# AlphacatPlus/VmambaIR

Hardware: AMD Instinct MI355X
Metric: images/sec, x4 SR 64->256 training step (fwd+bwd+Adam+EMA), full VmambaIR UNet (higher is better)
Workload: dtype bf16; 1 GPU; BASELINE.json configs[1]: x4 SR 64x64 LQ, MambaSISR6 dim48 [15,1,1,1]+15, bf16 autocast (scan arithmetic f32), batch 8 per GPU; global_batch=8, per_gpu_batch=8, parallelism=dp1, step_launch=hipGraph replay, vendor_conv_solver_search=True, vendor_conv_solver_records=bench_data/miopen, optimizer=Adam 2e-4 (0.9,0.99) + EMA 0.999, loss=L1, rccl_ranks=1, allreduce_overlapped=False, allreduce_buckets=1, allreduce_bytes=0

## Files before the change

### include/vmambair_oss.h

```cpp
#ifndef VMAMBAIR_OSS_H
#define VMAMBAIR_OSS_H

#include <stddef.h>
#include <stdint.h>

#ifdef __cplusplus
extern "C" {
#endif

#define OSS_OK 0
#define OSS_ERR_NULL (-1)
#define OSS_ERR_SHAPE (-2)
#define OSS_ERR_DSTATE (-3)
#define OSS_ERR_WORKSPACE (-4)

#define OSS_MAX_DSTATE 256

typedef enum {
    OSS_F32 = 0, OSS_F16 = 1, OSS_BF16 = 2,
    OSS_F32_BF16X3 = 3
} oss_dtype;

typedef void *oss_stream_t;

typedef struct {
    int batch, dim, seqlen, dstate, n_groups;
    int delta_softplus;
    int rev_group_start, u_row_mod;
    int a_log_form, reserved0_;
    int64_t u_batch_stride, u_d_stride;
    int64_t delta_batch_stride, delta_d_stride;
    int64_t out_batch_stride, out_d_stride;
    int64_t A_d_stride;
    int64_t B_batch_stride, B_group_stride, B_dstate_stride;
    int64_t C_batch_stride, C_group_stride, C_dstate_stride;
    const void *u, *delta;
    const float *A;
    const void *B, *C;
    const float *D;
    const float *delta_bias;
    void *out;
    float *x;
    const float *dt_weight;
    int dt_rank, reserved1_;
    int64_t dt_group_stride, dt_rank_stride;
    void *workspace;
    size_t workspace_bytes;
    float *hs;
    int tune_variant, tune_segments, tune_carry_split, reserved2_;
} oss_scan_fwd_params;

typedef struct {
    oss_scan_fwd_params f;
    int64_t dout_batch_stride, dout_d_stride;
    int64_t du_batch_stride, du_d_stride;
    int64_t ddelta_batch_stride, ddelta_d_stride;
    const void *dout;
    void *du, *ddelta;
    float *dA;
    void *dB, *dC;
    float *dD;
    float *ddelta_bias;
    void *workspace;
    size_t workspace_bytes;
    int dout_row_mod;
    int reserved_;
    int64_t dBC_group_stride;
    void *ddt;
    float *ddt_weight;
    int64_t ddt_batch_stride, ddt_group_stride, ddt_rank_stride;
    int tune_variant, tune_segments;
    int tune_partials, reserved3_;
    const float *finish_dt_weight;
    int finish_dt_rank, reserved4_;
} oss_scan_bwd_params;

int oss_scan_chunk(void);
int oss_scan_num_chunks(int seqlen);

size_t oss_scan_fwd_workspace_bytes(int batch, int dim, int seqlen, int dstate, int n_groups);
size_t oss_scan_lane_state_floats(int batch, int dim, int seqlen, int dstate);
int oss_scan_fwd(const oss_scan_fwd_params *p, oss_dtype io, oss_stream_t stream);

size_t oss_scan_bwd_workspace_bytes(int batch, int dim, int seqlen, int dstate, int n_groups);
int oss_scan_bwd(const oss_scan_bwd_params *p, oss_dtype io, oss_stream_t stream);

int oss_scan_bwd_finish_dt_ok(int seqlen, int dt_rank);

int oss_scan_fused_dt_ok(oss_dtype io, int batch, int D, int C, int R, int dstate, int seqlen);

void oss_scan_set_variant(int fwd_variant, int bwd_variant);
int oss_scan_last_variant(int which );
void oss_scan_set_segments(int fwd_segments, int bwd_segments);
int oss_scan_last_segments(int which );
void oss_scan_set_carry_split(int split);
int oss_scan_last_lane_states(void);

int oss_dwconv3x3_fwd(oss_dtype io, const void *x, const float *weight, const float *bias, void *y, void *pre_silu, int batch,
                      int channels, int height, int width, int64_t x_batch_stride, int64_t x_channel_stride,
                      int64_t y_batch_stride, int64_t y_channel_stride, int flip, oss_stream_t stream);
int oss_dwconv3x3_wgrad(oss_dtype io, const void *x, const void *dy, float *dweight, float *dbias, float *partials,
                        const void *pre_silu, void *dpre, int batch, int channels, int height, int width,
                        int64_t x_batch_stride, int64_t x_channel_stride, int64_t dy_batch_stride, int64_t dy_channel_stride,
                        oss_stream_t stream);

int oss_dwconv3x3_fused_ok(oss_dtype io, int height, int width, int channels_per_workgroup);
int oss_dwconv3x3_silu_fwd(oss_dtype io, const void *x, const float *weight, const float *bias, void *y, int batch, int channels,
                           int height, int width, int64_t x_batch_stride, int64_t x_channel_stride, int64_t y_batch_stride,
                           int64_t y_channel_stride, oss_stream_t stream);
int oss_dwconv3x3_silu_bwd(oss_dtype io, const void *x, const float *weight, const float *bias, const void *dy, void *dx,
                           float *dweight, float *dbias, float *partials, int batch, int channels, int height, int width,
                           int64_t x_batch_stride, int64_t x_channel_stride, int64_t dy_batch_stride, int64_t dy_channel_stride,
                           int64_t dx_batch_stride, int64_t dx_channel_stride, oss_stream_t stream);
int oss_dwgate_fwd_ok(oss_dtype io, int height, int width);

int oss_effn_fwd_ok(oss_dtype io, int channels, int hidden, int height, int width);
int oss_effn_round_weights(oss_dtype io, const float *project_in, const float *dwconv, const float *project_out, void *w_in, float *w_dw,
                           void *w_out, int channels, int hidden, oss_stream_t stream);
int oss_effn_fwd(oss_dtype io, const void *x, const float *norm_weight, const float *norm_bias, const void *w_in, const float *w_dw,
                 const void *w_out, void *out, int batch, int channels, int hidden, int height, int width, int64_t x_batch_stride,
                 int64_t x_channel_stride, int64_t out_batch_stride, int64_t out_channel_stride, float eps, oss_stream_t stream);
int oss_dwgate_fwd(oss_dtype io, const void *t, const float *weight, const float *bias, void *out, int batch, int hidden,
                   int height, int width, int64_t t_batch_stride, int64_t t_channel_stride, int64_t out_batch_stride,
                   int64_t out_channel_stride, oss_stream_t stream);
int oss_dwgate_bwd(oss_dtype io, const void *t, const float *weight, const float *bias, const void *dout, void *dt,
                   float *dweight, float *dbias, float *partials, int batch, int hidden, int height, int width,
                   int64_t t_batch_stride, int64_t t_channel_stride, int64_t dout_batch_stride, int64_t dout_channel_stride,
                   int64_t dt_batch_stride, int64_t dt_channel_stride, oss_stream_t stream);

int oss_dwconv3x3_flat2_ok(oss_dtype io, int height, int width);
int oss_dwconv3x3_silu_flat2_fwd(oss_dtype io, const void *x, const float *weight, const float *bias, void *x2, int batch, int channels,
                                 int height, int width, int64_t x_batch_stride, int64_t x_channel_stride, oss_stream_t stream);
int oss_dwconv3x3_silu_flat2_bwd(oss_dtype io, const void *x, const float *weight, const float *bias, const void *g2, void *dx,
                                 float *dweight, float *dbias, float *partials, int batch, int channels, int height, int width,
                                 int64_t x_batch_stride, int64_t x_channel_stride, int64_t dx_batch_stride, int64_t dx_channel_stride,
                                 oss_stream_t stream);

int oss_conv1x1_fwd(oss_dtype io, const void *x, const float *weight, const float *bias, const void *residual, void *y,
                    int batch, int cout, int cin, int pixels, int64_t x_batch_stride, int64_t x_channel_stride,
                    oss_stream_t stream);
int oss_conv1x1_dgrad(oss_dtype io, const void *dy, const float *weight, void *dx, int batch, int cout, int cin, int pixels,
                      int64_t dy_batch_stride, int64_t dy_channel_stride, oss_stream_t stream);
size_t oss_conv1x1_wgrad_partial_floats(int batch, int cout, int cin, int pixels);
size_t oss_conv1x1_fwd_image_bytes(int cout, int cin);
size_t oss_conv1x1_dgrad_image_bytes(int cout, int cin);
size_t oss_conv1x1_pack_row_bytes(void);
int oss_conv1x1_pack_rows(int cout, int cin);
int oss_conv1x1_pack_fill(void *rows, const float *weight, void *fwd_image, void *dgrad_image, int cout, int cin);
int oss_conv1x1_pack_weights(oss_dtype io, const void *table, int n_rows, oss_stream_t stream);
int oss_conv1x1_fwd_packed(oss_dtype io, const void *x, const float *weight, const void *fwd_image, const float *bias,
                           const void *residual, void *y, int batch, int cout, int cin, int pixels, int64_t x_batch_stride,
                           int64_t x_channel_stride, oss_stream_t stream);
int oss_conv1x1_dgrad_packed(oss_dtype io, const void *dy, const float *weight, const void *dgrad_image, void *dx, int batch,
                             int cout, int cin, int pixels, int64_t dy_batch_stride, int64_t dy_channel_stride,
                             oss_stream_t stream);
int oss_ln_conv1x1_fwd_packed(oss_dtype io, const void *x, const float *ln_weight, const float *ln_bias, float eps, void *n, float *mean,
                              float *rstd, const float *weight, const void *fwd_image, const float *bias, void *y, int batch, int cout,
                              int cin, int pixels, int64_t x_batch_stride, int64_t x_channel_stride, oss_stream_t stream);
int oss_conv1x1_wg(oss_dtype io, const void *x, const float *weight, const float *bias, void *y, int batch, int cout, int cin,
                   int pixels, int64_t x_batch_stride, int64_t x_channel_stride, int transposed_weight, oss_stream_t stream);
int oss_ln_conv1x1_ok(oss_dtype io, int cout, int cin, int pixels);
int oss_ln_conv1x1_fwd(oss_dtype io, const void *x, const float *ln_weight, const float *ln_bias, float eps, void *n, float *mean,
                       float *rstd, const float *weight, const float *bias, void *y, int batch, int cout, int cin, int pixels,
                       int64_t x_batch_stride, int64_t x_channel_stride, oss_stream_t stream);
int oss_conv1x1_dgrad_ln_bwd_ok(oss_dtype io, int cout, int cin, int pixels, int batch);
size_t oss_conv1x1_dgrad_ln_bwd_partial_floats(int batch, int cin, int pixels);
int oss_conv1x1_dgrad_ln_bwd(oss_dtype io, const void *dy, const float *weight, const void *x, const float *ln_weight, int ln_has_bias,
                             const float *mean, const float *rstd, const void *skip_grad, void *dx, float *dln_weight, float *dln_bias,
                             float *partials, int batch, int cout, int cin, int pixels, int64_t dy_batch_stride,
                             int64_t dy_channel_stride, oss_stream_t stream);
void oss_conv1x1_set_wg(int on, int pixels);
void oss_conv1x1_wgrad_set_tile(int mode);
void oss_conv1x1_wgrad_set_span(int mult);
int oss_conv1x1_wgrad(oss_dtype io, const void *dy, const void *x, float *dweight, float *dbias, float *partials, int batch,
                      int cout, int cin, int pixels, int64_t dy_batch_stride, int64_t dy_channel_stride,
                      int64_t x_batch_stride, int64_t x_channel_stride, oss_stream_t stream);

int oss_cross_scan2(oss_dtype in_type, oss_dtype out_type, const void *x, void *x2, int batch, int D, int height, int width,
                    int64_t x_batch_stride, int64_t x_channel_stride, oss_stream_t stream);
int oss_cross_merge2(oss_dtype io, const void *g2, void *dx, int batch, int D, int height, int width, oss_stream_t stream);
int oss_proj_fwd(oss_dtype io, const void *x2, const float *x_proj_weight, const float *dt_projs_weight, void *xdbl, void *dts,
                 int batch, int D, int C, int R, int seqlen, oss_stream_t stream);
int oss_proj_dgrad(oss_dtype io, const void *ddts, void *dxdbl, const void *du, const float *x_proj_weight,
                   const float *dt_projs_weight, void *dx2, int batch, int D, int C, int R, int seqlen, oss_stream_t stream);
size_t oss_proj_wgrad_partial_floats(int batch, int D, int C, int R, int seqlen);
void oss_proj_set_path(int force_vector_alu);
int oss_proj_rows_optional_ok(oss_dtype io, int batch, int D, int C, int R, int seqlen);
int oss_proj_wgrad(oss_dtype io, const void *x2, const void *xdbl, const void *dxdbl, const void *ddts, float *dx_proj_weight,
                   float *ddt_projs_weight, float *partials, int batch, int D, int C, int R, int seqlen, oss_stream_t stream);

typedef struct {
    int B, L, dc, Rc, Cc, reserved_;
    const float *pooled;
    const float *cin_w, *cin_b;
    const float *Wxc;
    const float *Wdtc;
    const float *dt_bias;
    const float *A_logs;
    const float *Dsc;
    const float *cout_w, *cout_b;
    const float *cn_w, *cn_b;
    float *zt;
    float *dts;
    float *hs;
    float *y;
    float *yc;
    float *stat;
    float *c;
    const float *pool_part;
    int n_part;
    float pool_scale;
} oss_chan_params;
int oss_chan_fwd(const oss_chan_params *p, oss_stream_t stream);
size_t oss_chan_grad_floats(int L, int dc, int Rc, int Cc);
size_t oss_chan_bwd_scratch_floats(int B, int L, int dc, int Rc, int Cc);
int oss_chan_bwd(const oss_chan_params *p, const float *gc, float *dpooled, float *grads, float *scratch, oss_stream_t stream);
int oss_rowsum(oss_dtype io, const void *a, const void *bmul, float *out, int batch, int channels, int pixels,
               int64_t a_batch_stride, int64_t a_channel_stride, int64_t b_batch_stride, int64_t b_channel_stride, float alpha,
               oss_stream_t stream);
int oss_row_affine(oss_dtype io, const void *x, const float *mul, const float *add, void *y, int batch, int channels,
                   int pixels, int64_t x_batch_stride, int64_t x_channel_stride, float alpha, oss_stream_t stream);

int oss_gelu_gate_fwd(oss_dtype io, const void *h, void *out, int batch, size_t half_elems, int64_t h_batch_stride,
                      oss_stream_t stream);
int oss_gelu_gate_bwd(oss_dtype io, const void *h, const void *dout, void *dh, int batch, size_t half_elems,
                      int64_t h_batch_stride, int64_t dout_batch_stride, oss_stream_t stream);

typedef struct {
    const void *src;
    void *dst;
    int64_t stride;
    int j0, n, K, reserved_;
} oss_sum_chunk;
void oss_set_defer_finish(int on);
size_t oss_deferred_chunks(void);
int oss_flush_finishes(void *host_table, void *device_table, size_t capacity_chunks, oss_stream_t stream);
int oss_flush_finishes_n(void *host_table, void *device_table, size_t capacity_chunks, size_t max_chunks, oss_stream_t stream);

void oss_set_defer_wgrad(int on);
size_t oss_deferred_wgrads(void);
size_t oss_deferred_wgrad_table_bytes(void);
int oss_flush_wgrads(void *host_table, void *device_table, size_t capacity_bytes, oss_stream_t stream);
int oss_flush_wgrads_n(void *host_table, void *device_table, size_t capacity_bytes, size_t max_products, oss_stream_t stream);

#define OSS_ADAM_CHUNK 2048
typedef struct {
    void *param;
    const void *grad;
    void *exp_avg, *exp_avg_sq, *ema;
    int n, reserved_;
} oss_adam_chunk;
int oss_adam_ema_step(const oss_adam_chunk *chunks, int n_chunks, float *state, float lr, float beta1, float beta2, float eps,
                      float ema_decay, oss_stream_t stream);
int oss_adamw_ema_step(const oss_adam_chunk *chunks, int n_chunks, float *state, float lr, float beta1, float beta2, float eps,
                       float weight_decay, float ema_decay, const float *grad_scale, oss_stream_t stream);

int oss_merge4(oss_dtype io, const void *out, float *y, int batch, int D, int height, int width, oss_stream_t stream);

size_t oss_ln_nchw_bwd_partial_floats(int batch, int channels, int pixels);
int oss_ln_nchw_fwd(oss_dtype x_type, oss_dtype y_type, const void *x, const float *weight, const float *bias,
                    const void *gate, void *y, float *mean, float *rstd, int batch, int channels, int pixels,
                    int64_t x_batch_stride, int64_t x_channel_stride, int64_t gate_batch_stride,
                    int64_t gate_channel_stride, float eps, oss_stream_t stream);
int oss_ln_nchw_fwd_pool_tiles(int channels, int pixels, int64_t x_batch_stride, int64_t x_channel_stride, int64_t gate_batch_stride,
                               int64_t gate_channel_stride);
int oss_ln_nchw_fwd_pool(oss_dtype x_type, oss_dtype y_type, const void *x, const float *weight, const float *bias,
                         const void *gate, void *y, float *mean, float *rstd, float *pool_part, int batch, int channels, int pixels,
                         int64_t x_batch_stride, int64_t x_channel_stride, int64_t gate_batch_stride,
                         int64_t gate_channel_stride, float eps, oss_stream_t stream);
int oss_ln_nchw_bwd(oss_dtype x_type, oss_dtype y_type, const void *x, const float *weight, const float *bias,
                    const void *gate, const void *dy, const float *mean, const float *rstd, void *dx, void *dgate,
                    float *dweight, float *dbias, float *partials, const void *skip_grad, int batch, int channels, int pixels,
                    int64_t x_batch_stride, int64_t x_channel_stride, int64_t gate_batch_stride,
                    int64_t gate_channel_stride, int64_t dgate_batch_stride, oss_stream_t stream);
int oss_ln_nchw_bwd_affine(oss_dtype x_type, oss_dtype y_type, const void *x, const float *weight, const float *bias,
                           const void *gate, const void *dy, const float *dy_mul, const float *dy_add, float add_scale,
                           const float *mean, const float *rstd, void *dx, void *dgate, float *dweight, float *dbias, float *partials,
                           const void *skip_grad, int batch, int channels, int pixels, int64_t x_batch_stride,
                           int64_t x_channel_stride, int64_t gate_batch_stride, int64_t gate_channel_stride,
                           int64_t dgate_batch_stride, oss_stream_t stream);

void oss_prof_enable(int on);
void oss_prof_reset(void);
int oss_prof_collect(int which, int variant, oss_dtype io, double *total_ms, long long *launches,
                     double *algorithmic_bytes);
int oss_prof_collect2(int which, int variant, oss_dtype io, double *total_ms, long long *launches, double *algorithmic_bytes,
                      double *own_bytes);

int oss_hbm_copy(const void *src, void *dst, size_t n_bytes, oss_stream_t stream);

int oss_prof_marker(int which, oss_stream_t stream);

const char *oss_scan_build_id(void);

const char *oss_version(void);

int oss_conv3x3_thin_ok(oss_dtype io, int cin, int cout, int height, int width);
int oss_conv3x3_thin_fwd(oss_dtype io, const void *x, const float *weight, const float *bias, void *y, int batch, int cin, int cout,
                         int height, int width, int64_t x_batch_stride, int64_t x_channel_stride, int64_t y_batch_stride,
                         int64_t y_channel_stride, oss_stream_t stream);
int oss_conv3x3_thin_dgrad(oss_dtype io, const void *dy, const float *weight, void *dx, int batch, int cin, int cout, int height,
                           int width, int64_t dy_batch_stride, int64_t dy_channel_stride, int64_t dx_batch_stride,
                           int64_t dx_channel_stride, oss_stream_t stream);
size_t oss_conv3x3_thin_wgrad_partial_floats(int batch, int cin, int cout);
int oss_conv3x3_thin_wgrad(oss_dtype io, const void *x, const void *dy, float *dweight, float *dbias, float *partial, int batch, int cin,
                           int cout, int height, int width, int64_t x_batch_stride, int64_t x_channel_stride, int64_t dy_batch_stride,
                           int64_t dy_channel_stride, oss_stream_t stream);

int oss_conv3x3_dense_ok(oss_dtype io, int cin, int cout, int height, int width);
int oss_conv3x3_dense_fwd(oss_dtype io, const void *x, const float *weight, const float *bias, void *y, int batch, int cin, int cout,
                          int height, int width, int64_t x_batch_stride, int64_t x_channel_stride, int64_t y_batch_stride,
                          int64_t y_channel_stride, oss_stream_t stream);
int oss_conv3x3_dense_dgrad(oss_dtype io, const void *dy, const float *weight, void *dx, int batch, int cin, int cout, int height,
                            int width, int64_t dy_batch_stride, int64_t dy_channel_stride, int64_t dx_batch_stride,
                            int64_t dx_channel_stride, oss_stream_t stream);
size_t oss_conv3x3_dense_wgrad_partial_floats(int batch, int cin, int cout, int height, int width);
int oss_conv3x3_dense_wgrad(oss_dtype io, const void *x, const void *dy, float *dweight, float *dbias, float *partial, int batch, int cin,
                            int cout, int height, int width, int64_t x_batch_stride, int64_t x_channel_stride, int64_t dy_batch_stride,
                            int64_t dy_channel_stride, oss_stream_t stream);

#define OSS_METRIC_QUANTISE 1
#define OSS_METRIC_Y 2
#define OSS_METRIC_REPLICATE 4
int oss_image_metrics_ok(oss_dtype io, int channels, int height, int width, int crop_border, int flags);
size_t oss_image_metrics_partial_doubles(int batch, int channels, int height, int width, int crop_border);
int oss_image_metrics(oss_dtype io, const void *a, const void *b, double *out, double *partials, int batch, int channels,
                      int height, int width, int64_t a_batch_stride, int64_t a_channel_stride, int64_t a_row_stride,
                      int64_t b_batch_stride, int64_t b_channel_stride, int64_t b_row_stride, int crop_border, int flags,
                      oss_stream_t stream);

#define OSS_PAIRS_HFLIP 1
#define OSS_PAIRS_ROT 2
int oss_pairs_philox(const uint32_t *counter, const uint32_t *key, uint32_t *out);
int oss_pairs_ok(int channels, int scale, int patch_h, int patch_w, int batch);
int oss_pairs_draw(const int64_t *table, int n_pairs, int64_t *counter, int *samples, int batch, int patch, int64_t seed, int rank,
                   int world, int flags, oss_stream_t stream);
int oss_pairs_gather(const void *pool, int64_t pool_bytes, const int64_t *table, int n_pairs, const int *samples, float *lq, float *gt,
                     int *clamped, int batch, int channels, int patch_h, int patch_w, int scale, int swap_rb, oss_stream_t stream);

void oss_prof_family_enable(int on);
int oss_prof_family_count(void);
int oss_prof_family(int family, const char **name, const char **kernel_patterns, double *algorithmic_bytes, long long *calls);

#define OSS_FEATURE_FUSED_DT 1
#define OSS_FEATURE_LANE_STATES 2
int oss_scan_features(void);

int oss_f32_matmul_modes(void);

#define OSS_ABI_VERSION 9
int oss_abi_version(void);
size_t oss_abi_struct_bytes(int which);

#ifdef __cplusplus
}
#endif
#endif
```

### vmambair_amd/csrc/oss_capi.hip

```cpp
#include <atomic>
#include <mutex>
#include <vector>
#include <cstring>
#include <algorithm>
#include "oss_device.h"
#include "oss_host.h"

namespace oss {

static std::atomic<int> g_force_fwd{-1}, g_force_bwd{-1};
static std::atomic<int> g_last_fwd{-1}, g_last_bwd{-1};
static std::atomic<int> g_force_fwd_seg{-1}, g_force_bwd_seg{-1};
std::atomic<int> g_last_fwd_segments{1}, g_last_bwd_segments{1}, g_last_bwd_lane_states{0};

int scan_pick_segments(long wgs, int n_chunks, int seg_req, double ovh) {
    if (seg_req == 0 || seg_req == 1 || n_chunks < 2 || wgs <= 0) return 1;
    if (seg_req > 1) return std::min(std::min(seg_req, n_chunks), kMaxSegments);
    if (wgs >= 256) return 1;
    int best = 1;
    double best_cost = (double)n_chunks;
    for (int s = 2; s <= std::min(n_chunks, 16); ++s) {
        const int cps = (n_chunks + s - 1) / s;
        if ((n_chunks + cps - 1) / cps != s) continue;
        const double rounds = (double)((wgs * s + 255) / 256);
        const double cost = rounds * cps * (1.0 + ovh);
        if (cost < 0.95 * best_cost) { best = s; best_cost = cost; }
    }
    return best;
}

static std::atomic<int> g_carry_split{0};
int scan_carry_split(long wgs, int n_seg, int cps, int n_chunks, int per_call) {
    if (n_seg <= 1) return 1;
    const int forced = per_call > 0 ? per_call : g_carry_split.load();
    const int max_slots = std::min(n_chunks, kMaxSegments);
    int csub = 1;
    for (int c = 2; c <= cps; ++c) {
        const int ccps = (cps + c - 1) / c, pieces = (cps + ccps - 1) / ccps;
        if (n_seg * pieces > max_slots) break;
        if (forced > 0 ? pieces <= forced : wgs * (n_seg - 1) * pieces <= 512) csub = pieces;
    }
    return csub;
}

static std::atomic<int> g_defer_finish{0};
static std::mutex g_defer_mu;
static std::vector<oss_sum_chunk> g_defer_chunks;
bool defer_finish() { return g_defer_finish.load() != 0; }
void defer_sum(const float *src, int K, size_t stride, size_t V, float *dst0, size_t n0, float *dst1) {
    std::lock_guard<std::mutex> lk(g_defer_mu);
    for (size_t j = 0; j < V;) {
        const size_t lim = j < n0 ? n0 : V;
        const size_t n = std::min<size_t>(1024, lim - j);
        oss_sum_chunk c;
        c.src = src;
        c.dst = j < n0 ? dst0 + j : dst1 + (j - n0);
        c.stride = (int64_t)stride;
        c.j0 = (int)j; c.n = (int)n; c.K = K; c.reserved_ = 0;
        g_defer_chunks.push_back(c);
        j += n;
    }
}
static std::atomic<int> g_defer_wgrad{0};
static std::vector<unsigned char> g_wgrad_descs;
static std::vector<unsigned> g_wgrad_blocks;
bool defer_wgrad() { return g_defer_wgrad.load() != 0; }
void defer_wgrad_push(const void *desc, size_t bytes, unsigned blocks) {
    std::lock_guard<std::mutex> lk(g_defer_mu);
    const unsigned char *p = reinterpret_cast<const unsigned char *>(desc);
    g_wgrad_descs.insert(g_wgrad_descs.end(), p, p + bytes);
    g_wgrad_blocks.push_back(blocks);
}

int scan_fwd_pick_variant(int batch, int dim, int seqlen, int dstate, int n_groups, int elem_bytes) {
    (void)dstate; (void)elem_bytes;
    const int rows_per_group = dim / n_groups;
    const long rows = (long)batch * dim;
    if (seqlen <= 256 || rows_per_group < 8) return (rows_per_group >= 16 && rows >= 4096) ? 2 : 4;
    if (rows_per_group % 16 == 0 && rows / 4 >= 2048) return 2;
    if (rows_per_group % 16 == 0 && rows / 2 >= 2048) return 1;
    if (seqlen >= 4096 && rows_per_group % 12 == 0 && (long)batch * n_groups * (rows_per_group / 12) <= 128) return 6;
    if (seqlen >= 1024 && (long)batch * n_groups * ((rows_per_group + 7) / 8) <= 256) return 3;
    if (seqlen >= 1024 && rows_per_group >= 12 && (long)batch * n_groups * ((rows_per_group + 11) / 12) <= 256) return 6;
    return 0;
}

int scan_bwd_pick_variant(int batch, int dim, int seqlen, int dstate, int n_groups) {
    const int rows_per_group = dim / n_groups;
    if (seqlen <= 256 || rows_per_group < 8 || dstate > 64) return 1;
    const long wgs = (long)batch * n_groups * ((rows_per_group + 7) / 8);
    if (seqlen >= 2048 && rows_per_group % 12 == 0 && (long)batch * n_groups * (rows_per_group / 12) < 192) return 10;
    if (wgs <= 128 && rows_per_group % 4 == 0) return 13;
    if (wgs <= 256) return 11;
    return rows_per_group >= 12 ? 10 : 11;
}

constexpr int kProfVariants = 32;
struct ProfBucket {
    std::vector<std::pair<hipEvent_t, hipEvent_t>> pending;
    double ms = 0.0, bytes = 0.0, own = 0.0;
    long long launches = 0;
};
static std::mutex g_prof_mu;
static std::atomic<int> g_prof_on{0};
static ProfBucket g_prof[3][kProfVariants][3];
static std::vector<hipEvent_t> g_event_pool;

static hipEvent_t prof_event() {
    if (!g_event_pool.empty()) { hipEvent_t e = g_event_pool.back(); g_event_pool.pop_back(); return e; }
    hipEvent_t e; (void)hipEventCreate(&e); return e;
}

struct ProfTimer : LaunchTimer {
    bool on; int which, variant, io; double bytes, own; hipEvent_t e0{}, e1{};
    ProfTimer(int which_, int variant_, int io_, double bytes_, double own_ = 0.0)
        : on(g_prof_on.load() != 0 && variant_ >= 0 && variant_ < 16), which(which_), variant(variant_),
          io(io_), bytes(bytes_), own(own_) {}
    void segmented() override { if (variant < 16) variant += 16; }
    void begin(hipStream_t s) override {
        if (!on) return;
        {
            std::lock_guard<std::mutex> lk(g_prof_mu);
            e0 = prof_event(); e1 = prof_event();
        }
        (void)hipEventRecord(e0, s);
    }
    void end(hipStream_t s) override {
        if (!on) return;
        (void)hipEventRecord(e1, s);
        std::lock_guard<std::mutex> lk(g_prof_mu);
        ProfBucket &b = g_prof[which][variant][io];
        b.pending.emplace_back(e0, e1);
        b.bytes += bytes;
        b.own += own;
        b.launches += 1;
    }
};


enum Fam { FAM_CONV1X1 = 0, FAM_WGRAD, FAM_DWCONV, FAM_PROJ, FAM_LN, FAM_CHAN, FAM_MERGE, FAM_GATE, FAM_CONV3X3, FAM_FINISH, FAM_OPTIM, FAM_N };
static const char *const kFamName[FAM_N] = {"conv1x1 forward / input gradient (+ fused LayerNorm)", "1x1 / projection weight gradients",
                                            "depth-wise 3x3 (+ silu / gelu gate / flattenings)", "x_proj / dt_proj forward + input gradient",
                                            "LayerNorm (+ silu gate, pooled sums)", "channel branch (+ rowsum / row_affine)",
                                            "cross-scan / cross-merge / merge4", "gelu gate (unfused)", "thin 3x3 convolutions",
                                            "deferred partial-sum finishing", "Adam(W) + EMA"};
static const char *const kFamKernels[FAM_N] = {"oss_conv1x1_pair_kernel|oss_conv1x1_pairk_kernel|oss_conv1x1_pairw_kernel|oss_conv1x1_wg_kernel|"
                                               "oss_conv1x1_dgrad_lnbwd_kernel|oss_conv1x1_f32_kernel|oss_conv1x1_pack_kernel",
                                               "oss_conv1x1_wgrad|oss_rows_f32_wgrad|oss_proj_wgrad",
                                               "oss_dwconv3x3|oss_dwgate|oss_effn",
                                               "oss_proj_fwd|oss_proj_dgrad|oss_dt_fwd|oss_dt_dgrad|oss_proj_valu",
                                               "oss_ln_nchw",
                                               "oss_chan_|oss_rowsum|oss_row_affine",
                                               "oss_merge4|oss_cross_scan2|oss_cross_merge2",
                                               "oss_gelu_gate",
                                               "oss_conv3x3_",
                                               "oss_sum_partials",
                                               "oss_adam"};
static std::atomic<int> g_fam_on{0};
static double g_fam_bytes[FAM_N];
static long long g_fam_calls[FAM_N];
static inline bool is_f32_split(oss_dtype io) { return io == OSS_F32_BF16X3; }
static inline int take_f32_split(oss_dtype &io) {
    if (!is_f32_split(io)) return 0;
    io = OSS_F32;
    return 1;
}
static inline void fam_count(int fam, double bytes) {
    if (!g_fam_on.load(std::memory_order_relaxed)) return;
    std::lock_guard<std::mutex> lk(g_prof_mu);
    g_fam_bytes[fam] += bytes;
    g_fam_calls[fam] += 1;
}

static double fwd_alg_bytes(const oss_scan_fwd_params &p, int s) {
    const double BKL = (double)p.batch * p.dim * p.seqlen, BGNL = (double)p.batch * p.n_groups * p.dstate * p.seqlen;
    const double xb = 4.0 * p.batch * p.dim * oss_scan_num_chunks(p.seqlen) * 2 * p.dstate;
    return s * (3.0 * BKL + 2.0 * BGNL) + 4.0 * ((double)p.dim * p.dstate + 2.0 * p.dim) + xb;
}
static double bwd_alg_bytes(const oss_scan_fwd_params &p, int s) {
    const double BKL = (double)p.batch * p.dim * p.seqlen, BGNL = (double)p.batch * p.n_groups * p.dstate * p.seqlen;
    const double xb = 4.0 * p.batch * p.dim * oss_scan_num_chunks(p.seqlen) * 2 * p.dstate;
    return s * (5.0 * BKL + 4.0 * BGNL) + 4.0 * (2.0 * p.dim * p.dstate + 4.0 * p.dim) + xb;
}

static double fwd_own_bytes(const oss_scan_fwd_params &p, int s) {
    const double full = fwd_alg_bytes(p, s);
    if (p.u_row_mod <= 0) return full;
    return full - (double)s * p.batch * (p.dim - p.u_row_mod) * p.seqlen;
}
static double bwd_own_bytes(const oss_scan_bwd_params &q, int s) {
    const oss_scan_fwd_params &p = q.f;
    double v = bwd_alg_bytes(p, s);
    if (p.u_row_mod > 0) v -= (double)s * p.batch * (p.dim - p.u_row_mod) * p.seqlen;
    if (q.dout_row_mod > 0) v -= (double)s * p.batch * (p.dim - q.dout_row_mod) * p.seqlen;
    return v;
}

static int check_fwd(const oss_scan_fwd_params *p) {
    if (!p || !p->u || !p->delta || !p->A || !p->B || !p->C) return OSS_ERR_NULL;
    if (p->dt_weight && (p->dt_rank < 1 || p->dt_rank > kMaxDtRank)) return OSS_ERR_SHAPE;
    if (p->batch < 0 || p->dim <= 0 || p->seqlen < 0 || p->dstate <= 0 || p->n_groups <= 0) return OSS_ERR_SHAPE;
    if (p->dim % p->n_groups != 0) return OSS_ERR_SHAPE;
    if (p->dstate > OSS_MAX_DSTATE) return OSS_ERR_DSTATE;
    if (p->rev_group_start < 0 || p->u_row_mod < 0 || (p->u_row_mod > 0 && p->dim % p->u_row_mod != 0)) return OSS_ERR_SHAPE;
    return OSS_OK;
}

}

using namespace oss;

extern "C" {

int oss_scan_chunk(void) { return kScanChunk; }
int oss_scan_num_chunks(int seqlen) { return seqlen <= 0 ? 0 : (seqlen + kScanChunk - 1) / kScanChunk; }

int oss_scan_fwd(const oss_scan_fwd_params *p, oss_dtype io, oss_stream_t stream) {
    const int eb = io_bytes(io);
    if (!eb) return OSS_ERR_SHAPE;
    int rc = check_fwd(p);
    if (rc != OSS_OK) return rc;
    if (!p->out || !p->x) return OSS_ERR_NULL;
    if (p->batch == 0 || p->seqlen == 0) return OSS_OK;
    int v = p->tune_variant > 0 ? p->tune_variant - 1 : g_force_fwd.load();
    if (v < 0) v = scan_fwd_pick_variant(p->batch, p->dim, p->seqlen, p->dstate, p->n_groups, eb);
    g_last_fwd.store(v);
    g_last_fwd_segments.store(1);
    const int sr = p->tune_segments > 0 ? p->tune_segments : g_force_fwd_seg.load();
    hipStream_t s = reinterpret_cast<hipStream_t>(stream);
    ProfTimer prof(0, v, (int)io, fwd_alg_bytes(*p, eb), fwd_own_bytes(*p, eb));
    prof.begin(s);
    rc = io_dispatch(io, [&](auto tag) { return scan_fwd_dispatch<typename decltype(tag)::type>(*p, v, sr, s); });
    if (g_last_fwd_segments.load() > 1) prof.segmented();
    prof.end(s);
    return rc;
}

static int bwd_variant_for(int batch, int dim, int seqlen, int dstate, int n_groups, int per_call = 0) {
    int v = per_call > 0 ? per_call - 1 : g_force_bwd.load();
    if (v < 0) v = scan_bwd_pick_variant(batch, dim, seqlen, dstate, n_groups);
    return v;
}

size_t oss_scan_bwd_workspace_bytes(int batch, int dim, int seqlen, int dstate, int n_groups) {
    if (batch <= 0 || dim <= 0 || seqlen <= 0 || dstate <= 0 || n_groups <= 0 || dim % n_groups) return 0;
    const int rows_per_group = dim / n_groups;
    const int rows = scan_bwd_rows_per_wg(1);
    const size_t tiles = (size_t)(rows_per_group + rows - 1) / rows;
    const size_t segs = (size_t)std::min(kMaxSegments, std::max(1, (seqlen + 511) / 512));
    const size_t floats = (size_t)batch * n_groups * tiles * (2 * dstate + kMaxDtRank) * seqlen +
                          (size_t)batch * segs * dim * (dstate + 2 + kMaxDtRank) +
                          (segs > 1 ? 2 * (size_t)batch * dim * dstate * segs : 0);
    return floats * sizeof(float);
}

size_t oss_scan_lane_state_floats(int batch, int dim, int seqlen, int dstate) {
    if (batch <= 0 || dim <= 0 || seqlen <= 0 || dstate <= 0) return 0;
    return (size_t)batch * dim * dstate * lane_state_stride(seqlen);
}

size_t oss_scan_fwd_workspace_bytes(int batch, int dim, int seqlen, int dstate, int n_groups) {
    if (batch <= 0 || dim <= 0 || seqlen <= 0 || dstate <= 0 || n_groups <= 0 || dim % n_groups) return 0;
    const int segs = std::min(kMaxSegments, (seqlen + kScanChunk - 1) / kScanChunk);
    return segs > 1 ? scan_carry_bytes(batch, dim, dstate, segs) : 0;
}

int oss_scan_bwd_finish_dt_ok(int seqlen, int dt_rank) { return scan_finish_dt_ok(seqlen, dt_rank) ? 1 : 0; }

int oss_scan_bwd(const oss_scan_bwd_params *p, oss_dtype io, oss_stream_t stream) {
    const int eb = io_bytes(io);
    if (!eb) return OSS_ERR_SHAPE;
    if (!p) return OSS_ERR_NULL;
    int rc = check_fwd(&p->f);
    if (rc != OSS_OK) return rc;
    if (!p->dout || !p->du || !p->dA || !p->dB || !p->dC) return OSS_ERR_NULL;
    if (!p->f.dt_weight && !p->ddelta) return OSS_ERR_NULL;
    if (p->f.dt_weight && (!p->ddt || !p->ddt_weight)) return OSS_ERR_NULL;
    const oss_scan_fwd_params &f = p->f;
    if (f.batch == 0 || f.seqlen == 0) return OSS_OK;
    if (!f.x && oss_scan_num_chunks(f.seqlen) > 1) return OSS_ERR_NULL;
    if (p->dout_row_mod < 0 || (p->dout_row_mod > 0 && f.dim % p->dout_row_mod != 0)) return OSS_ERR_SHAPE;
    const int v = bwd_variant_for(f.batch, f.dim, f.seqlen, f.dstate, f.n_groups, p->tune_variant);
    g_last_bwd.store(v);
    hipStream_t s = reinterpret_cast<hipStream_t>(stream);
    ProfTimer prof(1, v, (int)io, bwd_alg_bytes(f, eb), bwd_own_bytes(*p, eb));
    ProfTimer fprof(2, v, (int)io, 0.0);
    const int sr = p->tune_segments > 0 ? p->tune_segments : g_force_bwd_seg.load();
    g_last_bwd_lane_states.store(0);
    return io_dispatch(io, [&](auto tag) { return scan_bwd_dispatch<typename decltype(tag)::type>(*p, v, sr, s, &prof, &fprof); });
}

int oss_dwconv3x3_fwd(oss_dtype io, const void *x, const float *weight, const float *bias, void *y, void *pre_silu, int batch,
                      int channels, int height, int width, int64_t xsb, int64_t xsc, int64_t ysb, int64_t ysc, int flip,
                      oss_stream_t stream) {
    if (is_f32_split(io)) return OSS_ERR_SHAPE;
    fam_count(FAM_DWCONV, (double)batch * channels * height * width * io_bytes(io) * (pre_silu ? 3.0 : 2.0) + 40.0 * channels);
    if (!x || !weight || !y) return OSS_ERR_NULL;
    if (batch <= 0 || channels <= 0 || height <= 0 || width <= 0 || channels > 65535 || batch > 65535) return OSS_ERR_SHAPE;
    return dwconv3x3(io, x, weight, bias, y, batch, channels, height, width, xsb, xsc, ysb, ysc, flip,
                     reinterpret_cast<hipStream_t>(stream), pre_silu, pre_silu != nullptr);
}

int oss_dwconv3x3_fused_ok(oss_dtype io, int height, int width, int channels_per_workgroup) {
    return dwconv3x3_fused_ok(io, height, width, channels_per_workgroup);
}

int oss_dwconv3x3_silu_fwd(oss_dtype io, const void *x, const float *weight, const float *bias, void *y, int batch, int channels,
                           int height, int width, int64_t xsb, int64_t xsc, int64_t ysb, int64_t ysc, oss_stream_t stream) {
    if (is_f32_split(io)) return OSS_ERR_SHAPE;
    fam_count(FAM_DWCONV, (double)batch * channels * height * width * io_bytes(io) * 2.0 + 40.0 * channels);
    if (!x || !weight || !y) return OSS_ERR_NULL;
    if (batch <= 0 || channels <= 0 || height <= 0 || width <= 0 || channels > 65535 || batch > 65535) return OSS_ERR_SHAPE;
    return dwconv3x3(io, x, weight, bias, y, batch, channels, height, width, xsb, xsc, ysb, ysc, 0,
                     reinterpret_cast<hipStream_t>(stream), nullptr, 1);
}

int oss_dwconv3x3_silu_bwd(oss_dtype io, const void *x, const float *weight, const float *bias, const void *dy, void *dx,
                           float *dweight, float *dbias, float *partials, int batch, int channels, int height, int width,
                           int64_t xsb, int64_t xsc, int64_t gsb, int64_t gsc, int64_t dsb, int64_t dsc, oss_stream_t stream) {
    if (is_f32_split(io)) return OSS_ERR_SHAPE;
    fam_count(FAM_DWCONV, (double)batch * channels * height * width * io_bytes(io) * 3.0 + 80.0 * channels);
    if (!x || !weight || !dy || !dx || !dweight || !partials) return OSS_ERR_NULL;
    if (batch <= 0 || channels <= 0 || height <= 0 || width <= 0 || channels > 65535 || batch > 65535) return OSS_ERR_SHAPE;
    return dwconv3x3_bwd_fused(io, 0, x, weight, bias, dy, dx, dweight, dbias, partials, batch, channels, height, width, xsb, xsc,
                               gsb, gsc, dsb, dsc, reinterpret_cast<hipStream_t>(stream));
}

int oss_dwconv3x3_flat2_ok(oss_dtype io, int height, int width) {
    return dwconv3x3_flat2_ok(io, height, width);
}

int oss_dwconv3x3_silu_flat2_fwd(oss_dtype io, const void *x, const float *weight, const float *bias, void *x2, int batch, int channels,
                                 int height, int width, int64_t xsb, int64_t xsc, oss_stream_t stream) {
    if (is_f32_split(io)) return OSS_ERR_SHAPE;
    fam_count(FAM_DWCONV, (double)batch * channels * height * width * io_bytes(io) * 3.0 + 40.0 * channels);
    if (!x || !weight || !x2) return OSS_ERR_NULL;
    if (batch <= 0 || channels <= 0 || height <= 0 || width <= 0 || channels > 65535 || batch > 65535) return OSS_ERR_SHAPE;
    return dwconv3x3_silu_flat2_fwd(io, x, weight, bias, x2, batch, channels, height, width, xsb, xsc, reinterpret_cast<hipStream_t>(stream));
}

int oss_dwconv3x3_silu_flat2_bwd(oss_dtype io, const void *x, const float *weight, const float *bias, const void *g2, void *dx,
                                 float *dweight, float *dbias, float *partials, int batch, int channels, int height, int width,
                                 int64_t xsb, int64_t xsc, int64_t dsb, int64_t dsc, oss_stream_t stream) {
    if (is_f32_split(io)) return OSS_ERR_SHAPE;
    fam_count(FAM_DWCONV, (double)batch * channels * height * width * io_bytes(io) * 4.0 + 80.0 * channels);
    if (!x || !weight || !g2 || !dx || !dweight || !partials) return OSS_ERR_NULL;
    if (batch <= 0 || channels <= 0 || height <= 0 || width <= 0 || channels > 65535 || batch > 65535) return OSS_ERR_SHAPE;
    return dwconv3x3_silu_flat2_bwd(io, x, weight, bias, g2, dx, dweight, dbias, partials, batch, channels, height, width, xsb, xsc, dsb,
                                    dsc, reinterpret_cast<hipStream_t>(stream));
}

int oss_effn_fwd_ok(oss_dtype io, int channels, int hidden, int height, int width) {
    return effn_fwd_ok(io, channels, hidden, height, width);
}

int oss_effn_round_weights(oss_dtype io, const float *project_in, const float *dwconv, const float *project_out, void *w_in, float *w_dw,
                           void *w_out, int channels, int hidden, oss_stream_t stream) {
    if (is_f32_split(io)) return OSS_ERR_SHAPE;
    if (!project_in || !dwconv || !project_out || !w_in || !w_dw || !w_out) return OSS_ERR_NULL;
    return effn_round_weights(io, project_in, dwconv, project_out, w_in, w_dw, w_out, channels, hidden, reinterpret_cast<hipStream_t>(stream));
}

int oss_effn_fwd(oss_dtype io, const void *x, const float *norm_weight, const float *norm_bias, const void *w_in, const float *w_dw,
                 const void *w_out, void *out, int batch, int channels, int hidden, int height, int width, int64_t xsb, int64_t xsc,
                 int64_t osb, int64_t osc, float eps, oss_stream_t stream) {
    if (is_f32_split(io)) return OSS_ERR_SHAPE;
    fam_count(FAM_DWCONV, (double)batch * channels * height * width * io_bytes(io) * 3.0 + (double)hidden * (3.0 * channels * io_bytes(io) + 72.0));
    if (!x || !norm_weight || !w_in || !w_dw || !w_out || !out) return OSS_ERR_NULL;
    if (batch <= 0 || channels <= 0 || hidden <= 0 || height <= 0 || width <= 0) return OSS_ERR_SHAPE;
    return effn_fwd(io, x, norm_weight, norm_bias, w_in, w_dw, w_out, out, batch, channels, hidden, height, width, xsb, xsc, osb, osc, eps,
                    reinterpret_cast<hipStream_t>(stream));
}

int oss_dwgate_fwd_ok(oss_dtype io, int height, int width) {
    return dwgate_fwd_ok(io, height, width);
}

int oss_dwgate_fwd(oss_dtype io, const void *t, const float *weight, const float *bias, void *out, int batch, int hidden,
                   int height, int width, int64_t tsb, int64_t tsc, int64_t osb, int64_t osc, oss_stream_t stream) {
    if (is_f32_split(io)) return OSS_ERR_SHAPE;
    fam_count(FAM_DWCONV, (double)batch * hidden * height * width * io_bytes(io) * 3.0 + 80.0 * hidden);
    if (!t || !weight || !out) return OSS_ERR_NULL;
    if (batch <= 0 || hidden <= 0 || height <= 0 || width <= 0 || hidden > 32767 || batch > 65535) return OSS_ERR_SHAPE;
    return dwgate_fwd(io, t, weight, bias, out, batch, hidden, height, width, tsb, tsc, osb, osc, reinterpret_cast<hipStream_t>(stream));
}

int oss_dwgate_bwd(oss_dtype io, const void *t, const float *weight, const float *bias, const void *dout, void *dt,
                   float *dweight, float *dbias, float *partials, int batch, int hidden, int height, int width, int64_t tsb,
                   int64_t tsc, int64_t gsb, int64_t gsc, int64_t dsb, int64_t dsc, oss_stream_t stream) {
    if (is_f32_split(io)) return OSS_ERR_SHAPE;
    fam_count(FAM_DWCONV, (double)batch * hidden * height * width * io_bytes(io) * 5.0 + 160.0 * hidden);
    if (!t || !weight || !dout || !dt || !dweight || !partials) return OSS_ERR_NULL;
    if (batch <= 0 || hidden <= 0 || height <= 0 || width <= 0 || hidden > 32767 || batch > 65535) return OSS_ERR_SHAPE;
    return dwconv3x3_bwd_fused(io, 1, t, weight, bias, dout, dt, dweight, dbias, partials, batch, 2 * hidden, height, width, tsb,
                               tsc, gsb, gsc, dsb, dsc, reinterpret_cast<hipStream_t>(stream));
}

int oss_dwconv3x3_wgrad(oss_dtype io, const void *x, const void *dy, float *dweight, float *dbias, float *partials,
                        const void *pre_silu, void *dpre, int batch, int channels, int height, int width, int64_t xsb,
                        int64_t xsc, int64_t gsb, int64_t gsc, oss_stream_t stream) {
    if (is_f32_split(io)) return OSS_ERR_SHAPE;
    fam_count(FAM_DWCONV, (double)batch * channels * height * width * io_bytes(io) * (pre_silu ? 4.0 : 2.0));
    if (!x || !dy || !dweight || !partials) return OSS_ERR_NULL;
    if (batch <= 0 || channels <= 0 || height <= 0 || width <= 0 || batch > 65535) return OSS_ERR_SHAPE;
    return dwconv3x3_wgrad(io, x, dy, dweight, dbias, partials, batch, channels, height, width, xsb, xsc, gsb, gsc,
                           reinterpret_cast<hipStream_t>(stream), pre_silu, dpre);
}

int oss_conv1x1_fwd(oss_dtype io, const void *x, const float *weight, const float *bias, const void *residual, void *y,
                    int batch, int cout, int cin, int pixels, int64_t xsb, int64_t xsc, oss_stream_t stream) {
    const int x3 = take_f32_split(io);
    fam_count(FAM_CONV1X1, (double)batch * pixels * io_bytes(io) * ((double)cin + cout + (residual ? cout : 0)) + 4.0 * cin * cout);
    if (!x || !weight || !y) return OSS_ERR_NULL;
    if (batch <= 0 || cout <= 0 || cin <= 0 || pixels <= 0 || batch > 65535 || cout > 32 * 65535) return OSS_ERR_SHAPE;
    return conv1x1(io, x, weight, bias, y, batch, cout, cin, pixels, xsb, xsc, cin, 1, reinterpret_cast<hipStream_t>(stream),
                   residual, x3);
}

int oss_conv1x1_dgrad(oss_dtype io, const void *dy, const float *weight, void *dx, int batch, int cout, int cin, int pixels,
                      int64_t gsb, int64_t gsc, oss_stream_t stream) {
    const int x3 = take_f32_split(io);
    fam_count(FAM_CONV1X1, (double)batch * pixels * io_bytes(io) * ((double)cin + cout) + 4.0 * cin * cout);
    if (!dy || !weight || !dx) return OSS_ERR_NULL;
    if (batch <= 0 || cout <= 0 || cin <= 0 || pixels <= 0 || batch > 65535) return OSS_ERR_SHAPE;
    return conv1x1(io, dy, weight, nullptr, dx, batch, cin, cout, pixels, gsb, gsc, 1, cin, reinterpret_cast<hipStream_t>(stream), nullptr, x3);
}

size_t oss_conv1x1_fwd_image_bytes(int cout, int cin) { return cout > 0 && cin > 0 ? conv1x1_image_bytes(cout, cin) : 0; }
size_t oss_conv1x1_dgrad_image_bytes(int cout, int cin) { return cout > 0 && cin > 0 ? conv1x1_image_bytes(cin, cout) : 0; }
size_t oss_conv1x1_pack_row_bytes(void) { return conv1x1_pack_row_bytes(); }
int oss_conv1x1_pack_rows(int cout, int cin) { return cout > 0 && cin > 0 ? conv1x1_pack_rows(cout, cin) : 0; }
int oss_conv1x1_pack_fill(void *rows, const float *weight, void *fwd_image, void *dgrad_image, int cout, int cin) {
    if (!rows || !weight || !fwd_image || !dgrad_image) return OSS_ERR_NULL;
    if (cout <= 0 || cin <= 0 || (size_t)cout * cin >= (1u << 30)) return OSS_ERR_SHAPE;
    if ((reinterpret_cast<uintptr_t>(fwd_image) | reinterpret_cast<uintptr_t>(dgrad_image)) & 15u) return OSS_ERR_SHAPE;
    return conv1x1_pack_fill(rows, weight, fwd_image, dgrad_image, cout, cin);
}
int oss_conv1x1_pack_weights(oss_dtype io, const void *table, int n_rows, oss_stream_t stream) {
    if (is_f32_split(io)) return OSS_ERR_SHAPE;
    fam_count(FAM_CONV1X1, (double)n_rows * 256.0 * 16.0 * 3.0);
    if (!table) return OSS_ERR_NULL;
    if (n_rows <= 0) return OSS_ERR_SHAPE;
    return conv1x1_pack(io, table, n_rows, reinterpret_cast<hipStream_t>(stream));
}
int oss_conv1x1_fwd_packed(oss_dtype io, const void *x, const float *weight, const void *fwd_image, const float *bias,
                           const void *residual, void *y, int batch, int cout, int cin, int pixels, int64_t xsb, int64_t xsc,
                           oss_stream_t stream) {
    if (!fwd_image || !io_ok<IO_16>(io)) return oss_conv1x1_fwd(io, x, weight, bias, residual, y, batch, cout, cin, pixels, xsb, xsc, stream);
    fam_count(FAM_CONV1X1, (double)batch * pixels * io_bytes(io) * ((double)cin + cout + (residual ? cout : 0)) + 2.0 * cin * cout);
    if (!x || !weight || !y) return OSS_ERR_NULL;
    if (batch <= 0 || cout <= 0 || cin <= 0 || pixels <= 0 || batch > 65535 || cout > 32 * 65535) return OSS_ERR_SHAPE;
    if (reinterpret_cast<uintptr_t>(fwd_image) & 15u) return OSS_ERR_SHAPE;
    return conv1x1(io, x, weight, bias, y, batch, cout, cin, pixels, xsb, xsc, cin, 1, reinterpret_cast<hipStream_t>(stream),
                   residual, 0, fwd_image);
}
int oss_conv1x1_dgrad_packed(oss_dtype io, const void *dy, const float *weight, const void *dgrad_image, void *dx, int batch,
                             int cout, int cin, int pixels, int64_t gsb, int64_t gsc, oss_stream_t stream) {
    if (!dgrad_image || !io_ok<IO_16>(io)) return oss_conv1x1_dgrad(io, dy, weight, dx, batch, cout, cin, pixels, gsb, gsc, stream);
    fam_count(FAM_CONV1X1, (double)batch * pixels * io_bytes(io) * ((double)cin + cout) + 2.0 * cin * cout);
    if (!dy || !weight || !dx) return OSS_ERR_NULL;
    if (batch <= 0 || cout <= 0 || cin <= 0 || pixels <= 0 || batch > 65535) return OSS_ERR_SHAPE;
    if (reinterpret_cast<uintptr_t>(dgrad_image) & 15u) return OSS_ERR_SHAPE;
    return conv1x1(io, dy, weight, nullptr, dx, batch, cin, cout, pixels, gsb, gsc, 1, cin, reinterpret_cast<hipStream_t>(stream), nullptr, 0,
                   dgrad_image);
}

size_t oss_conv1x1_wgrad_partial_floats(int batch, int cout, int cin, int pixels) {
    if (batch <= 0 || cout <= 0 || cin <= 0 || pixels <= 0) return 0;
    return (size_t)batch * conv1x1_wgrad_slabs(pixels) * cout * (cin + 1);
}

int oss_conv1x1_wgrad(oss_dtype io, const void *dy, const void *x, float *dweight, float *dbias, float *partials, int batch,
                      int cout, int cin, int pixels, int64_t gsb, int64_t gsc, int64_t xsb, int64_t xsc, oss_stream_t stream) {
    const int x3 = take_f32_split(io);
    fam_count(FAM_WGRAD, (double)batch * pixels * io_bytes(io) * ((double)cin + cout) + 4.0 * cin * cout);
    if (!dy || !x || !dweight || !partials) return OSS_ERR_NULL;
    if (batch <= 0 || cout <= 0 || cin <= 0 || pixels <= 0 || batch > 65535) return OSS_ERR_SHAPE;
    return conv1x1_wgrad(io, dy, x, dweight, partials, batch, cout, cin, pixels, gsb, gsc, xsb, xsc,
                         reinterpret_cast<hipStream_t>(stream), 1, 0, 0, 0, 0, dbias, x3);
}

size_t oss_proj_wgrad_partial_floats(int batch, int D, int C, int R, int seqlen) {
    if (batch <= 0 || D <= 0 || C <= 0 || R <= 0 || seqlen <= 0) return 0;
    const size_t slabs = (size_t)batch * conv1x1_wgrad_slabs(seqlen);
    const size_t a = slabs * 2 * (2 * (size_t)C) * D, b = slabs * 4 * (size_t)D * R;
    return a + b;
}

int oss_proj_fwd(oss_dtype io, const void *x2, const float *x_proj_weight, const float *dt_projs_weight, void *xdbl, void *dts,
                 int batch, int D, int C, int R, int seqlen, oss_stream_t stream) {
    const int x3 = take_f32_split(io);
    fam_count(FAM_PROJ, (double)batch * seqlen * io_bytes(io) * (2.0 * D + 4.0 * C + (dts ? 4.0 * R + 4.0 * D : 0.0)) + 16.0 * C * D + 16.0 * D * R);
    if (!x2 || !x_proj_weight || !dt_projs_weight || !xdbl) return OSS_ERR_NULL;
    if (batch <= 0 || D <= 0 || seqlen <= 0 || R <= 0 || C <= R) return OSS_ERR_SHAPE;
    return proj_fwd(io, x2, x_proj_weight, dt_projs_weight, xdbl, dts, batch, D, C, R, seqlen, reinterpret_cast<hipStream_t>(stream), x3);
}

int oss_proj_dgrad(oss_dtype io, const void *ddts, void *dxdbl, const void *du, const float *x_proj_weight,
                   const float *dt_projs_weight, void *dx2, int batch, int D, int C, int R, int seqlen, oss_stream_t stream) {
    const int x3 = take_f32_split(io);
    fam_count(FAM_PROJ, (double)batch * seqlen * io_bytes(io) * ((ddts ? 4.0 * D + 4.0 * R : 0.0) + 4.0 * C + (du ? 4.0 * D : 0.0) + 2.0 * D) + 16.0 * C * D);
    if (!dxdbl || !x_proj_weight || !dt_projs_weight || !dx2) return OSS_ERR_NULL;
    if (batch <= 0 || D <= 0 || seqlen <= 0 || R <= 0 || C <= R) return OSS_ERR_SHAPE;
    return proj_dgrad(io, ddts, dxdbl, du, x_proj_weight, dt_projs_weight, dx2, batch, D, C, R, seqlen,
                      reinterpret_cast<hipStream_t>(stream), x3);
}

void oss_proj_set_path(int force_vector_alu) { proj_force_valu(force_vector_alu); }
int oss_proj_rows_optional_ok(oss_dtype io, int batch, int D, int C, int R, int seqlen) {
    return proj_mfma_ok(io, batch, D, C, R, seqlen) ? 1 : 0;
}
int oss_scan_fused_dt_ok(oss_dtype io, int batch, int D, int C, int R, int dstate, int seqlen) {
    return proj_mfma_ok(io, batch, D, C, R, seqlen) && R >= 1 && R <= kMaxDtRank && dstate <= 64 && seqlen >= 512;
}
int oss_conv1x1_wg(oss_dtype io, const void *x, const float *weight, const float *bias, void *y, int batch, int cout, int cin,
                   int pixels, int64_t xsb, int64_t xsc, int transposed_weight, oss_stream_t stream) {
    if (is_f32_split(io)) return OSS_ERR_SHAPE;
    fam_count(FAM_CONV1X1, (double)batch * pixels * io_bytes(io) * ((double)cin + cout) + 4.0 * cin * cout);
    if (!x || !weight || !y) return OSS_ERR_NULL;
    if (batch <= 0 || batch > 65535) return OSS_ERR_SHAPE;
    return conv1x1_wg(io, x, weight, bias, y, batch, cout, cin, pixels, xsb, xsc, transposed_weight, reinterpret_cast<hipStream_t>(stream));
}

int oss_ln_conv1x1_ok(oss_dtype io, int cout, int cin, int pixels) {
    const void *a = reinterpret_cast<const void *>(uintptr_t(256));
    return conv1x1_wg_ok(io, cout, cin, pixels, (int64_t)cin * pixels, pixels, a, a, reinterpret_cast<const float *>(a), nullptr);
}

int oss_ln_conv1x1_fwd(oss_dtype io, const void *x, const float *ln_weight, const float *ln_bias, float eps, void *n, float *mean,
                       float *rstd, const float *weight, const float *bias, void *y, int batch, int cout, int cin, int pixels,
                       int64_t xsb, int64_t xsc, oss_stream_t stream) {
    if (is_f32_split(io)) return OSS_ERR_SHAPE;
    fam_count(FAM_CONV1X1, (double)batch * pixels * (io_bytes(io) * (2.0 * cin + cout) + 8.0) + 4.0 * cin * cout);
    if (!x || !ln_weight || !n || !mean || !rstd || !weight || !y) return OSS_ERR_NULL;
    if (batch <= 0 || batch > 65535) return OSS_ERR_SHAPE;
    return ln_conv1x1_wg(io, x, ln_weight, ln_bias, eps, n, mean, rstd, weight, bias, y, batch, cout, cin, pixels, xsb, xsc,
                         reinterpret_cast<hipStream_t>(stream));
}

int oss_ln_conv1x1_fwd_packed(oss_dtype io, const void *x, const float *ln_weight, const float *ln_bias, float eps, void *n, float *mean,
                              float *rstd, const float *weight, const void *fwd_image, const float *bias, void *y, int batch, int cout,
                              int cin, int pixels, int64_t xsb, int64_t xsc, oss_stream_t stream) {
    if (!fwd_image)
        return oss_ln_conv1x1_fwd(io, x, ln_weight, ln_bias, eps, n, mean, rstd, weight, bias, y, batch, cout, cin, pixels, xsb, xsc, stream);
    if (is_f32_split(io)) return OSS_ERR_SHAPE;
    fam_count(FAM_CONV1X1, (double)batch * pixels * (io_bytes(io) * (2.0 * cin + cout) + 8.0) + 2.0 * cin * cout);
    if (!x || !ln_weight || !n || !mean || !rstd || !weight || !y) return OSS_ERR_NULL;
    if (batch <= 0 || batch > 65535) return OSS_ERR_SHAPE;
    return ln_conv1x1_wg(io, x, ln_weight, ln_bias, eps, n, mean, rstd, weight, bias, y, batch, cout, cin, pixels, xsb, xsc,
                         reinterpret_cast<hipStream_t>(stream), fwd_image);
}

int oss_conv1x1_dgrad_ln_bwd_ok(oss_dtype io, int cout, int cin, int pixels, int batch) {
    return conv1x1_dgrad_lnbwd_ok(io, cin, cout, pixels, batch);
}
size_t oss_conv1x1_dgrad_ln_bwd_partial_floats(int batch, int cin, int pixels) {
    if (batch <= 0 || cin <= 0 || pixels <= 0) return 0;
    return conv1x1_dgrad_lnbwd_partial_floats(batch, cin, pixels);
}
int oss_conv1x1_dgrad_ln_bwd(oss_dtype io, const void *dy, const float *weight, const void *x, const float *ln_weight, int ln_has_bias,
                             const float *mean, const float *rstd, const void *skip_grad, void *dx, float *dln_weight, float *dln_bias,
                             float *partials, int batch, int cout, int cin, int pixels, int64_t gsb, int64_t gsc, oss_stream_t stream) {
    if (is_f32_split(io)) return OSS_ERR_SHAPE;
    fam_count(FAM_CONV1X1, (double)batch * pixels * (io_bytes(io) * ((double)cout + 2.0 * cin + (skip_grad ? cin : 0)) + 8.0) + 4.0 * cin * cout);
    if (!dy || !weight || !x || !ln_weight || !mean || !rstd || !dx || !dln_weight || !partials) return OSS_ERR_NULL;
    if (batch <= 0 || batch > 65535) return OSS_ERR_SHAPE;
    return conv1x1_dgrad_lnbwd(io, dy, weight, x, ln_weight, ln_has_bias, mean, rstd, skip_grad, dx, dln_weight, dln_bias, partials, batch,
                               cin, cout, pixels, gsb, gsc, reinterpret_cast<hipStream_t>(stream));
}

void oss_conv1x1_set_wg(int on, int pixels) { conv1x1_set_wg(on); conv1x1_wg_set_pixels(pixels); }
void oss_conv1x1_wgrad_set_tile(int mode) { conv1x1_wgrad_set_tile(mode); }
void oss_conv1x1_wgrad_set_span(int mult) { conv1x1_wgrad_set_span(mult); }

int oss_proj_wgrad(oss_dtype io, const void *x2, const void *xdbl, const void *dxdbl, const void *ddts, float *dx_proj_weight,
                   float *ddt_projs_weight, float *partials, int batch, int D, int C, int R, int seqlen, oss_stream_t stream) {
    const int x3 = take_f32_split(io);
    fam_count(FAM_WGRAD, (double)batch * seqlen * io_bytes(io) * (2.0 * D + 8.0 * C + (ddts ? 4.0 * D : 0.0)));
    if (!x2 || !xdbl || !dxdbl || !dx_proj_weight || !partials) return OSS_ERR_NULL;
    if (ddts && !ddt_projs_weight) return OSS_ERR_NULL;
    if (batch <= 0 || D <= 0 || seqlen <= 0 || R <= 0 || C <= R) return OSS_ERR_SHAPE;
    hipStream_t s = reinterpret_cast<hipStream_t>(stream);
    const int64_t L = seqlen;
    if (io == OSS_F32) {
        int e = rows_f32_wgrad(reinterpret_cast<const float *>(dxdbl), reinterpret_cast<const float *>(x2), dx_proj_weight, partials, batch,
                               4, 2, C, D, seqlen, 4 * C * L, C * L, L, 2 * D * L, D * L, L, s, nullptr, x3);
        if (e || !ddts) return e;
        float *part2 = partials + (size_t)batch * conv1x1_wgrad_slabs(seqlen) * 2 * (2 * (size_t)C) * D;
        return rows_f32_wgrad(reinterpret_cast<const float *>(ddts), reinterpret_cast<const float *>(xdbl), ddt_projs_weight, part2, batch, 4,
                              4, D, R, seqlen, 4 * D * L, D * L, L, 4 * C * L, C * L, L, s, nullptr, x3);
    }
    int e = conv1x1_wgrad(io, dxdbl, x2, dx_proj_weight, partials, batch, 2 * C, D, seqlen, 4 * C * L, L, 2 * D * L, L, s,
                           2,  C * L,  D * L,  C,  2 * C * L);
    if (e || !ddts) return e;
    float *part2 = partials + (size_t)batch * conv1x1_wgrad_slabs(seqlen) * 2 * (2 * (size_t)C) * D;
    return conv1x1_wgrad(io, ddts, xdbl, ddt_projs_weight, part2, batch, D, R, seqlen, 4 * D * L, L, 4 * C * L, L, s,
                          4,  D * L,  C * L,  D, 0);
}

int oss_cross_scan2(oss_dtype in_type, oss_dtype out_type, const void *x, void *x2, int batch, int D, int height, int width,
                    int64_t x_batch_stride, int64_t x_channel_stride, oss_stream_t stream) {
    if (is_f32_split(in_type) || is_f32_split(out_type)) return OSS_ERR_SHAPE;
    fam_count(FAM_MERGE, (double)batch * D * height * width * (io_bytes(in_type) + 2.0 * io_bytes(out_type)));
    if (!x || !x2) return OSS_ERR_NULL;
    if (batch <= 0 || D <= 0 || height <= 0 || width <= 0) return OSS_ERR_SHAPE;
    return cross_scan2(in_type, out_type, x, x2, batch, D, height, width, x_batch_stride, x_channel_stride,
                       reinterpret_cast<hipStream_t>(stream));
}

int oss_cross_merge2(oss_dtype io, const void *g2, void *dx, int batch, int D, int height, int width, oss_stream_t stream) {
    if (is_f32_split(io)) return OSS_ERR_SHAPE;
    fam_count(FAM_MERGE, (double)batch * D * height * width * io_bytes(io) * 3.0);
    if (!g2 || !dx) return OSS_ERR_NULL;
    if (batch <= 0 || D <= 0 || height <= 0 || width <= 0) return OSS_ERR_SHAPE;
    return cross_merge2(io, g2, dx, batch, D, height, width, reinterpret_cast<hipStream_t>(stream));
}

int oss_chan_fwd(const oss_chan_params *p, oss_stream_t stream) {
    fam_count(FAM_CHAN, p ? 4.0 * p->B * ((double)p->L * (2.0 * p->Cc + 2.0 * p->dc * 18.0 + 3.0) + (p->pool_part ? (double)p->n_part * p->L : p->L)) : 0.0);
    if (!p) return OSS_ERR_NULL;
    return chan_fwd(*p, reinterpret_cast<hipStream_t>(stream));
}

size_t oss_chan_grad_floats(int L, int dc, int Rc, int Cc) { return chan_grad_floats(L, dc, Rc, Cc); }
size_t oss_chan_bwd_scratch_floats(int B, int L, int dc, int Rc, int Cc) { return chan_bwd_scratch_floats(B, L, dc, Rc, Cc); }

int oss_chan_bwd(const oss_chan_params *p, const float *gc, float *dpooled, float *grads, float *scratch, oss_stream_t stream) {
    fam_count(FAM_CHAN, p ? 4.0 * p->B * ((double)p->L * (2.0 * p->Cc + 2.0 * p->dc * 18.0 + 5.0)) : 0.0);
    if (!p) return OSS_ERR_NULL;
    return chan_bwd(*p, gc, dpooled, grads, scratch, reinterpret_cast<hipStream_t>(stream));
}

int oss_rowsum(oss_dtype io, const void *a, const void *bmul, float *out, int batch, int channels, int pixels, int64_t asb,
               int64_t asc, int64_t bsb, int64_t bsc, float alpha, oss_stream_t stream) {
    if (is_f32_split(io)) return OSS_ERR_SHAPE;
    fam_count(FAM_CHAN, (double)batch * channels * pixels * io_bytes(io) * (bmul ? 2.0 : 1.0));
    if (!a || !out) return OSS_ERR_NULL;
    if (batch <= 0 || channels <= 0 || pixels <= 0) return OSS_ERR_SHAPE;
    return rowsum(io, a, bmul, out, batch, channels, pixels, asb, asc, bsb, bsc, alpha, reinterpret_cast<hipStream_t>(stream));
}

int oss_row_affine(oss_dtype io, const void *x, const float *mul, const float *add, void *y, int batch, int channels, int pixels,
                   int64_t xsb, int64_t xsc, float alpha, oss_stream_t stream) {
    if (is_f32_split(io)) return OSS_ERR_SHAPE;
    fam_count(FAM_CHAN, (double)batch * channels * pixels * io_bytes(io) * 2.0);
    if (!x || !y) return OSS_ERR_NULL;
    if (batch <= 0 || channels <= 0 || pixels <= 0) return OSS_ERR_SHAPE;
    return row_affine(io, x, mul, add, y, batch, channels, pixels, xsb, xsc, alpha, reinterpret_cast<hipStream_t>(stream));
}

int oss_gelu_gate_fwd(oss_dtype io, const void *h, void *out, int batch, size_t half_elems, int64_t h_batch_stride,
                      oss_stream_t stream) {
    if (is_f32_split(io)) return OSS_ERR_SHAPE;
    fam_count(FAM_GATE, (double)batch * half_elems * io_bytes(io) * 3.0);
    if (!h || !out) return OSS_ERR_NULL;
    if (batch <= 0 || half_elems == 0) return OSS_ERR_SHAPE;
    return gelu_gate_fwd(io, h, out, batch, half_elems, h_batch_stride, reinterpret_cast<hipStream_t>(stream));
}

int oss_gelu_gate_bwd(oss_dtype io, const void *h, const void *dout, void *dh, int batch, size_t half_elems,
                      int64_t h_batch_stride, int64_t dout_batch_stride, oss_stream_t stream) {
    if (is_f32_split(io)) return OSS_ERR_SHAPE;
    fam_count(FAM_GATE, (double)batch * half_elems * io_bytes(io) * 5.0);
    if (!h || !dout || !dh) return OSS_ERR_NULL;
    if (batch <= 0 || half_elems == 0) return OSS_ERR_SHAPE;
    return gelu_gate_bwd(io, h, dout, dh, batch, half_elems, h_batch_stride, dout_batch_stride, reinterpret_cast<hipStream_t>(stream));
}

int oss_conv3x3_thin_ok(oss_dtype io, int cin, int cout, int height, int width) {
    return conv3x3_thin_ok(io, cin, cout, height, width);
}
int oss_conv3x3_thin_fwd(oss_dtype io, const void *x, const float *weight, const float *bias, void *y, int batch, int cin, int cout,
                         int height, int width, int64_t xsb, int64_t xsc, int64_t ysb, int64_t ysc, oss_stream_t stream) {
    if (is_f32_split(io)) return OSS_ERR_SHAPE;
    fam_count(FAM_CONV3X3, (double)batch * height * width * io_bytes(io) * ((double)cin + cout));
    if (!x || !weight || !y) return OSS_ERR_NULL;
    return conv3x3_thin_fwd(io, x, weight, bias, y, batch, cin, cout, height, width, xsb, xsc, ysb, ysc, reinterpret_cast<hipStream_t>(stream));
}
int oss_conv3x3_thin_dgrad(oss_dtype io, const void *dy, const float *weight, void *dx, int batch, int cin, int cout, int height,
                           int width, int64_t gsb, int64_t gsc, int64_t dsb, int64_t dsc, oss_stream_t stream) {
    if (is_f32_split(io)) return OSS_ERR_SHAPE;
    fam_count(FAM_CONV3X3, (double)batch * height * width * io_bytes(io) * ((double)cin + cout));
    if (!dy || !weight || !dx) return OSS_ERR_NULL;
    return conv3x3_thin_dgrad(io, dy, weight, dx, batch, cin, cout, height, width, gsb, gsc, dsb, dsc, reinterpret_cast<hipStream_t>(stream));
}
size_t oss_conv3x3_thin_wgrad_partial_floats(int batch, int cin, int cout) {
    return (batch <= 0 || cin <= 0 || cout <= 0) ? 0 : conv3x3_thin_wgrad_partial_floats(batch, cin, cout);
}
int oss_conv3x3_thin_wgrad(oss_dtype io, const void *x, const void *dy, float *dweight, float *dbias, float *partial, int batch, int cin,
                           int cout, int height, int width, int64_t xsb, int64_t xsc, int64_t gsb, int64_t gsc, oss_stream_t stream) {
    if (is_f32_split(io)) return OSS_ERR_SHAPE;
    fam_count(FAM_CONV3X3, (double)batch * height * width * io_bytes(io) * ((double)cin + cout));
    if (!x || !dy || !dweight || !partial) return OSS_ERR_NULL;
    return conv3x3_thin_wgrad(io, x, dy, dweight, dbias, partial, batch, cin, cout, height, width, xsb, xsc, gsb, gsc,
                              reinterpret_cast<hipStream_t>(stream));
}

int oss_conv3x3_dense_ok(oss_dtype io, int cin, int cout, int height, int width) {
    return conv3x3_dense_ok(io, cin, cout, height, width);
}
static double dense_bytes(oss_dtype io, int batch, int cin, int cout, int height, int width) {
    return (double)batch * height * width * io_bytes(io) * ((double)cin + cout) + 36.0 * cin * cout;
}
int oss_conv3x3_dense_fwd(oss_dtype io, const void *x, const float *weight, const float *bias, void *y, int batch, int cin, int cout,
                          int height, int width, int64_t xsb, int64_t xsc, int64_t ysb, int64_t ysc, oss_stream_t stream) {
    if (is_f32_split(io)) return OSS_ERR_SHAPE;
    fam_count(FAM_CONV3X3, dense_bytes(io, batch, cin, cout, height, width));
    if (!x || !weight || !y) return OSS_ERR_NULL;
    return conv3x3_dense_fwd(io, x, weight, bias, y, batch, cin, cout, height, width, xsb, xsc, ysb, ysc, reinterpret_cast<hipStream_t>(stream));
}
int oss_conv3x3_dense_dgrad(oss_dtype io, const void *dy, const float *weight, void *dx, int batch, int cin, int cout, int height,
                            int width, int64_t gsb, int64_t gsc, int64_t dsb, int64_t dsc, oss_stream_t stream) {
    if (is_f32_split(io)) return OSS_ERR_SHAPE;
    fam_count(FAM_CONV3X3, dense_bytes(io, batch, cin, cout, height, width));
    if (!dy || !weight || !dx) return OSS_ERR_NULL;
    return conv3x3_dense_dgrad(io, dy, weight, dx, batch, cin, cout, height, width, gsb, gsc, dsb, dsc, reinterpret_cast<hipStream_t>(stream));
}
size_t oss_conv3x3_dense_wgrad_partial_floats(int batch, int cin, int cout, int height, int width) {
    if (batch <= 0 || batch > 65535 || cin < 16 || cin % 16 != 0 || cin > 16384 || cout < 5 || cout > 16384 || height < 1 ||
        height > 32768 || width < 1 || width > 32768)
        return 0;
    return conv3x3_dense_wgrad_partial_floats(batch, cin, cout, height, width);
}
int oss_conv3x3_dense_wgrad(oss_dtype io, const void *x, const void *dy, float *dweight, float *dbias, float *partial, int batch, int cin,
                            int cout, int height, int width, int64_t xsb, int64_t xsc, int64_t gsb, int64_t gsc, oss_stream_t stream) {
    if (is_f32_split(io)) return OSS_ERR_SHAPE;
    fam_count(FAM_CONV3X3, dense_bytes(io, batch, cin, cout, height, width));
    if (!x || !dy || !dweight || !partial) return OSS_ERR_NULL;
    return conv3x3_dense_wgrad(io, x, dy, dweight, dbias, partial, batch, cin, cout, height, width, xsb, xsc, gsb, gsc,
                               reinterpret_cast<hipStream_t>(stream));
}

int oss_image_metrics_ok(oss_dtype io, int channels, int height, int width, int crop_border, int flags) {
    return image_metrics_ok(io, channels, height, width, crop_border, flags);
}
size_t oss_image_metrics_partial_doubles(int batch, int channels, int height, int width, int crop_border) {
    return image_metrics_partial_doubles(batch, channels, height, width, crop_border);
}
int oss_image_metrics(oss_dtype io, const void *a, const void *b, double *out, double *partials, int batch, int channels, int height,
                      int width, int64_t asb, int64_t asc, int64_t ars, int64_t bsb, int64_t bsc, int64_t brs, int crop_border, int flags,
                      oss_stream_t stream) {
    if (is_f32_split(io)) return OSS_ERR_SHAPE;
    if (!a || !b || !out || !partials) return OSS_ERR_NULL;
    return image_metrics(io, a, b, out, partials, batch, channels, height, width, asb, asc, ars, bsb, bsc, brs, crop_border, flags,
                         reinterpret_cast<hipStream_t>(stream));
}

void oss_set_defer_wgrad(int on) {
    std::lock_guard<std::mutex> lk(g_defer_mu);
    g_defer_wgrad.store(on ? 1 : 0);
    g_wgrad_descs.clear();
    g_wgrad_blocks.clear();
}
size_t oss_deferred_wgrads(void) {
    std::lock_guard<std::mutex> lk(g_defer_mu);
    return g_wgrad_blocks.size();
}
size_t oss_deferred_wgrad_table_bytes(void) {
    std::lock_guard<std::mutex> lk(g_defer_mu);
    size_t blocks = 0;
    for (unsigned b : g_wgrad_blocks) blocks += b;
    return ((g_wgrad_descs.size() + 255) & ~(size_t)255) + 2 * blocks;
}
int oss_flush_wgrads_n(void *host_table, void *device_table, size_t capacity_bytes, size_t max_products, oss_stream_t stream) {
    std::lock_guard<std::mutex> lk(g_defer_mu);
    const size_t n_all = g_wgrad_blocks.size();
    const size_t n = max_products > 0 ? std::min(n_all, max_products) : n_all;
    if (n == 0) return 0;
    if (!host_table || !device_table) return OSS_ERR_NULL;
    if (n > 65535) return OSS_ERR_SHAPE;
    const size_t db = wgrad_desc_bytes();
    const size_t desc_bytes = (n * db + 255) & ~(size_t)255;
    size_t total = 0;
    for (size_t i = 0; i < n; ++i) total += g_wgrad_blocks[i];
    if (desc_bytes + 2 * total > capacity_bytes) return OSS_ERR_WORKSPACE;
    if (total > 0x7fffffffu) return OSS_ERR_SHAPE;
    const int io = wgrad_desc_io(g_wgrad_descs.data());
    unsigned first = 0;
    uint16_t *map = reinterpret_cast<uint16_t *>(reinterpret_cast<unsigned char *>(host_table) + desc_bytes);
    for (size_t i = 0; i < n; ++i) {
        if (wgrad_desc_io(g_wgrad_descs.data() + i * db) != io) return OSS_ERR_SHAPE;
        wgrad_desc_set_first_block(g_wgrad_descs.data() + i * db, first);
        for (unsigned k = 0; k < g_wgrad_blocks[i]; ++k) map[first + k] = (uint16_t)i;
        first += g_wgrad_blocks[i];
    }
    std::memcpy(host_table, g_wgrad_descs.data(), n * db);
    hipStream_t s = reinterpret_cast<hipStream_t>(stream);
    const hipError_t e = hipMemcpyAsync(device_table, host_table, desc_bytes + 2 * total, hipMemcpyHostToDevice, s);
    if (e != hipSuccess) return (int)e;
    g_wgrad_descs.erase(g_wgrad_descs.begin(), g_wgrad_descs.begin() + n * db);
    g_wgrad_blocks.erase(g_wgrad_blocks.begin(), g_wgrad_blocks.begin() + n);
    return wgrad_grouped_launch(io, device_table, reinterpret_cast<unsigned char *>(device_table) + desc_bytes, (unsigned)total, s);
}
int oss_flush_wgrads(void *host_table, void *device_table, size_t capacity_bytes, oss_stream_t stream) {
    return oss_flush_wgrads_n(host_table, device_table, capacity_bytes, 0, stream);
}

void oss_set_defer_finish(int on) {
    std::lock_guard<std::mutex> lk(g_defer_mu);
    g_defer_finish.store(on ? 1 : 0);
    g_defer_chunks.clear();
}
size_t oss_deferred_chunks(void) {
    std::lock_guard<std::mutex> lk(g_defer_mu);
    return g_defer_chunks.size();
}
int oss_flush_finishes_n(void *host_table, void *device_table, size_t capacity_chunks, size_t max_chunks, oss_stream_t stream) {
    std::lock_guard<std::mutex> lk(g_defer_mu);
    const size_t n_all = g_defer_chunks.size();
    const size_t n = max_chunks > 0 ? std::min(n_all, max_chunks) : n_all;
    if (n == 0) return 0;
    if (!host_table || !device_table) return OSS_ERR_NULL;
    if (n > capacity_chunks) return OSS_ERR_WORKSPACE;
    hipStream_t s = reinterpret_cast<hipStream_t>(stream);
    if (g_fam_on.load(std::memory_order_relaxed)) {
        double by = 0.0;
        for (size_t i = 0; i < n; ++i) by += 4.0 * g_defer_chunks[i].n * (g_defer_chunks[i].K + 1.0);
        fam_count(FAM_FINISH, by);
    }
    std::memcpy(host_table, g_defer_chunks.data(), n * sizeof(oss_sum_chunk));
    hipError_t e = hipMemcpyAsync(device_table, host_table, n * sizeof(oss_sum_chunk), hipMemcpyHostToDevice, s);
    if (e != hipSuccess) return (int)e;
    g_defer_chunks.erase(g_defer_chunks.begin(), g_defer_chunks.begin() + n);
    return sum_partials_multi(reinterpret_cast<const oss_sum_chunk *>(device_table), (int)n, s);
}
int oss_flush_finishes(void *host_table, void *device_table, size_t capacity_chunks, oss_stream_t stream) {
    return oss_flush_finishes_n(host_table, device_table, capacity_chunks, 0, stream);
}

int oss_adam_ema_step(const oss_adam_chunk *chunks, int n_chunks, float *state, float lr, float beta1, float beta2, float eps,
                      float ema_decay, oss_stream_t stream) {
    fam_count(FAM_OPTIM, 36.0 * n_chunks * 2048.0);
    if (!chunks || !state) return OSS_ERR_NULL;
    if (n_chunks <= 0) return OSS_ERR_SHAPE;
    return adam_ema_step(chunks, n_chunks, state, lr, beta1, beta2, eps, ema_decay, reinterpret_cast<hipStream_t>(stream));
}

int oss_adamw_ema_step(const oss_adam_chunk *chunks, int n_chunks, float *state, float lr, float beta1, float beta2, float eps,
                       float weight_decay, float ema_decay, const float *grad_scale, oss_stream_t stream) {
    fam_count(FAM_OPTIM, 36.0 * n_chunks * 2048.0);
    if (!chunks || !state) return OSS_ERR_NULL;
    if (n_chunks <= 0 || weight_decay < 0.f) return OSS_ERR_SHAPE;
    return adam_ema_step(chunks, n_chunks, state, lr, beta1, beta2, eps, ema_decay, reinterpret_cast<hipStream_t>(stream),
                         weight_decay, grad_scale);
}

int oss_merge4(oss_dtype io, const void *out, float *y, int batch, int D, int height, int width, oss_stream_t stream) {
    if (is_f32_split(io)) return OSS_ERR_SHAPE;
    fam_count(FAM_MERGE, (double)batch * D * height * width * (4.0 * io_bytes(io) + 4.0));
    if (!out || !y) return OSS_ERR_NULL;
    if (batch <= 0 || D <= 0 || height <= 0 || width <= 0 || (long)batch * D > 65535) return OSS_ERR_SHAPE;
    return merge4(io, out, y, batch, D, height, width, reinterpret_cast<hipStream_t>(stream));
}

int oss_ln_nchw_fwd(oss_dtype xt, oss_dtype yt, const void *x, const float *weight, const float *bias, const void *gate,
                    void *y, float *mean, float *rstd, int batch, int channels, int pixels, int64_t xsb, int64_t xsc,
                    int64_t gsb, int64_t gsc, float eps, oss_stream_t stream) {
    if (is_f32_split(xt) || is_f32_split(yt)) return OSS_ERR_SHAPE;
    fam_count(FAM_LN, (double)batch * channels * pixels * (io_bytes(xt) + io_bytes(yt) * (gate ? 2.0 : 1.0)) + 8.0 * batch * pixels);
    if (!x || !weight || !y || !mean || !rstd) return OSS_ERR_NULL;
    if (batch <= 0 || channels <= 0 || pixels <= 0 || batch > 65535) return OSS_ERR_SHAPE;
    return ln_nchw_fwd(xt, yt, x, weight, bias, gate, y, mean, rstd, batch, channels, pixels, xsb, xsc, gsb, gsc, eps,
                       reinterpret_cast<hipStream_t>(stream));
}

int oss_ln_nchw_fwd_pool_tiles(int channels, int pixels, int64_t xsb, int64_t xsc, int64_t gsb, int64_t gsc) {
    if (channels <= 0 || pixels <= 0) return 0;
    return ln_nchw_fwd_pool_tiles(channels, pixels, xsb, xsc, gsb, gsc);
}

int oss_ln_nchw_fwd_pool(oss_dtype xt, oss_dtype yt, const void *x, const float *weight, const float *bias, const void *gate, void *y,
                         float *mean, float *rstd, float *pool_part, int batch, int channels, int pixels, int64_t xsb, int64_t xsc,
                         int64_t gsb, int64_t gsc, float eps, oss_stream_t stream) {
    if (is_f32_split(xt) || is_f32_split(yt)) return OSS_ERR_SHAPE;
    fam_count(FAM_LN, (double)batch * channels * pixels * (io_bytes(xt) + io_bytes(yt) * (gate ? 2.0 : 1.0)) + 8.0 * batch * pixels);
    if (!x || !weight || !y || !mean || !rstd || !pool_part) return OSS_ERR_NULL;
    if (batch <= 0 || channels <= 0 || pixels <= 0 || batch > 65535 || channels > 4096) return OSS_ERR_SHAPE;
    return ln_nchw_fwd(xt, yt, x, weight, bias, gate, y, mean, rstd, batch, channels, pixels, xsb, xsc, gsb, gsc, eps,
                       reinterpret_cast<hipStream_t>(stream), pool_part);
}

int oss_ln_nchw_bwd(oss_dtype xt, oss_dtype yt, const void *x, const float *weight, const float *bias, const void *gate,
                    const void *dy, const float *mean, const float *rstd, void *dx, void *dgate, float *dweight,
                    float *dbias, float *partials, const void *skip_grad, int batch, int channels, int pixels, int64_t xsb,
                    int64_t xsc, int64_t gsb, int64_t gsc, int64_t dgate_batch_stride, oss_stream_t stream) {
    if (is_f32_split(xt) || is_f32_split(yt)) return OSS_ERR_SHAPE;
    fam_count(FAM_LN, (double)batch * channels * pixels * (2.0 * io_bytes(xt) + io_bytes(yt) * (1.0 + (gate ? 2.0 : 0.0) + (skip_grad ? 1.0 : 0.0))) + 8.0 * batch * pixels);
    if (!x || !weight || !dy || !mean || !rstd || !dx || !dweight || !partials) return OSS_ERR_NULL;
    if (gate && !dgate) return OSS_ERR_NULL;
    if (batch <= 0 || channels <= 0 || pixels <= 0 || batch > 65535 || channels > 4096) return OSS_ERR_SHAPE;
    return ln_nchw_bwd(xt, yt, x, weight, bias, gate, dy, mean, rstd, dx, dgate, dweight, dbias, partials, batch, channels,
                       pixels, xsb, xsc, gsb, gsc, reinterpret_cast<hipStream_t>(stream), skip_grad, dgate_batch_stride);
}

int oss_ln_nchw_bwd_affine(oss_dtype xt, oss_dtype yt, const void *x, const float *weight, const float *bias, const void *gate,
                           const void *dy, const float *dy_mul, const float *dy_add, float add_scale, const float *mean,
                           const float *rstd, void *dx,
                           void *dgate, float *dweight, float *dbias, float *partials, const void *skip_grad, int batch,
                           int channels, int pixels, int64_t xsb, int64_t xsc, int64_t gsb, int64_t gsc,
                           int64_t dgate_batch_stride, oss_stream_t stream) {
    if (is_f32_split(xt) || is_f32_split(yt)) return OSS_ERR_SHAPE;
    fam_count(FAM_LN, (double)batch * channels * pixels * (2.0 * io_bytes(xt) + io_bytes(yt) * (1.0 + (gate ? 2.0 : 0.0) + (skip_grad ? 1.0 : 0.0))) + 8.0 * batch * pixels);
    if (!x || !weight || !dy || !mean || !rstd || !dx || !dweight || !partials || !dy_add) return OSS_ERR_NULL;
    if (gate && !dgate) return OSS_ERR_NULL;
    if (batch <= 0 || channels <= 0 || pixels <= 0 || batch > 65535 || channels > 4096) return OSS_ERR_SHAPE;
    return ln_nchw_bwd(xt, yt, x, weight, bias, gate, dy, mean, rstd, dx, dgate, dweight, dbias, partials, batch, channels,
                       pixels, xsb, xsc, gsb, gsc, reinterpret_cast<hipStream_t>(stream), skip_grad, dgate_batch_stride, dy_mul,
                       dy_add, add_scale);
}

size_t oss_ln_nchw_bwd_partial_floats(int batch, int channels, int pixels) {
    if (batch <= 0 || channels <= 0 || pixels <= 0) return 0;
    return ln_nchw_bwd_partial_floats(batch, channels, pixels);
}

void oss_prof_enable(int on) { g_prof_on.store(on ? 1 : 0); }

void oss_prof_family_enable(int on) {
    std::lock_guard<std::mutex> lk(g_prof_mu);
    if (on) for (int f = 0; f < FAM_N; ++f) { g_fam_bytes[f] = 0.0; g_fam_calls[f] = 0; }
    g_fam_on.store(on ? 1 : 0);
}
int oss_prof_family_count(void) { return FAM_N; }
int oss_prof_family(int family, const char **name, const char **kernel_patterns, double *algorithmic_bytes, long long *calls) {
    if (family < 0 || family >= FAM_N) return OSS_ERR_SHAPE;
    std::lock_guard<std::mutex> lk(g_prof_mu);
    if (name) *name = kFamName[family];
    if (kernel_patterns) *kernel_patterns = kFamKernels[family];
    if (algorithmic_bytes) *algorithmic_bytes = g_fam_bytes[family];
    if (calls) *calls = g_fam_calls[family];
    return OSS_OK;
}

void oss_prof_reset(void) {
    std::lock_guard<std::mutex> lk(g_prof_mu);
    for (auto &k : g_prof) for (auto &v : k) for (auto &b : v) {
        for (auto &pr : b.pending) { (void)hipEventSynchronize(pr.second); g_event_pool.push_back(pr.first); g_event_pool.push_back(pr.second); }
        b.pending.clear(); b.ms = 0.0; b.bytes = 0.0; b.own = 0.0; b.launches = 0;
    }
}

int oss_prof_collect2(int which, int variant, oss_dtype io, double *total_ms, long long *launches, double *algorithmic_bytes,
                      double *own_bytes) {
    const int rc = oss_prof_collect(which, variant, io, total_ms, launches, algorithmic_bytes);
    if (rc == OSS_OK && own_bytes) {
        std::lock_guard<std::mutex> lk(g_prof_mu);
        *own_bytes = g_prof[which][variant][(int)io].own;
    }
    return rc;
}

int oss_prof_collect(int which, int variant, oss_dtype io, double *total_ms, long long *launches, double *algorithmic_bytes) {
    if (which < 0 || which > 2 || variant < 0 || variant >= kProfVariants || !io_ok(io)) return OSS_ERR_SHAPE;
    std::lock_guard<std::mutex> lk(g_prof_mu);
    ProfBucket &b = g_prof[which][variant][(int)io];
    for (auto &pr : b.pending) {
        (void)hipEventSynchronize(pr.second);
        float ms = 0.f;
        if (hipEventElapsedTime(&ms, pr.first, pr.second) == hipSuccess) b.ms += ms;
        g_event_pool.push_back(pr.first); g_event_pool.push_back(pr.second);
    }
    b.pending.clear();
    if (total_ms) *total_ms = b.ms;
    if (launches) *launches = b.launches;
    if (algorithmic_bytes) *algorithmic_bytes = b.bytes;
    return OSS_OK;
}

void oss_scan_set_variant(int fwd_variant, int bwd_variant) {
    g_force_fwd.store(fwd_variant);
    g_force_bwd.store(bwd_variant);
}
int oss_scan_last_variant(int which) { return which == 0 ? g_last_fwd.load() : g_last_bwd.load(); }
void oss_scan_set_segments(int fwd_segments, int bwd_segments) {
    g_force_fwd_seg.store(fwd_segments);
    g_force_bwd_seg.store(bwd_segments);
}
int oss_scan_last_segments(int which) { return which == 0 ? g_last_fwd_segments.load() : g_last_bwd_segments.load(); }
void oss_scan_set_carry_split(int split) { g_carry_split.store(split < 0 ? 0 : split); }
int oss_scan_last_lane_states(void) { return g_last_bwd_lane_states.load(); }
int oss_f32_matmul_modes(void) { return 1 | 2; }
int oss_scan_features(void) { return OSS_FEATURE_FUSED_DT | OSS_FEATURE_LANE_STATES; }

__global__ void __launch_bounds__(256) oss_copy_flat_kernel(const f32x4 *src, f32x4 *dst, size_t n) {
    const size_t i = (size_t)blockIdx.x * 256 + threadIdx.x;
    if (i < n) dst[i] = src[i];
}

int oss_hbm_copy(const void *src, void *dst, size_t n_bytes, oss_stream_t stream) {
    if (!src || !dst) return OSS_ERR_NULL;
    const size_t n = n_bytes / 16;
    if (n == 0) return OSS_OK;
    if ((n + 255) / 256 > 0x7fffffffu) return OSS_ERR_SHAPE;
    hipLaunchKernelGGL(oss_copy_flat_kernel, dim3((unsigned)((n + 255) / 256)), dim3(256), 0, reinterpret_cast<hipStream_t>(stream),
                       reinterpret_cast<const f32x4 *>(src), reinterpret_cast<f32x4 *>(dst), n);
    return (int)hipGetLastError();
}

__global__ void oss_prof_marker_begin() {}
__global__ void oss_prof_marker_end() {}
int oss_prof_marker(int which, oss_stream_t stream) {
    hipStream_t s = reinterpret_cast<hipStream_t>(stream);
    if (which == 1) hipLaunchKernelGGL(oss_prof_marker_begin, dim3(1), dim3(1), 0, s);
    else hipLaunchKernelGGL(oss_prof_marker_end, dim3(1), dim3(1), 0, s);
    return (int)hipGetLastError();
}

#ifndef OSS_SCAN_BUILD_ID
#define OSS_SCAN_BUILD_ID "unknown"
#endif
const char *oss_scan_build_id(void) { return OSS_SCAN_BUILD_ID; }

const char *oss_version(void) { return "vmambair_oss 0.4 (gfx950)"; }

int oss_abi_version(void) { return OSS_ABI_VERSION; }
size_t oss_abi_struct_bytes(int which) {
    switch (which) {
        case 0: return sizeof(oss_scan_fwd_params);
        case 1: return sizeof(oss_scan_bwd_params);
        case 2: return sizeof(oss_chan_params);
        default: return 0;
    }
}

}
```

### vmambair_amd/csrc/oss_channel.hip

```cpp
#include "oss_device.h"
#include "oss_host.h"

namespace oss {

constexpr int kChN = 16;
constexpr int kChU = 8;
constexpr int kChNT = 512;
constexpr int kChRed = 8;

template <int NT>
__device__ __forceinline__ float block_sum(float v, float *red , int tid) {
    static_assert(NT == 256 || NT == 512, "block_sum: 4 or 8 waves");
    const float w = segment_sum_to_last<64>(v);
    __syncthreads();
    if ((tid & 63) == 63) red[tid >> 6] = w;
    __syncthreads();
    float t = (red[0] + red[1]) + (red[2] + red[3]);
    if constexpr (NT == 512) t += (red[4] + red[5]) + (red[6] + red[7]);
    return t;
}

__device__ __forceinline__ float sum_over_rows(float v, int lane) {
    v += __int_as_float(__builtin_amdgcn_ds_bpermute((lane ^ 16) << 2, __float_as_int(v)));
    v += __int_as_float(__builtin_amdgcn_ds_bpermute((lane ^ 32) << 2, __float_as_int(v)));
    return v;
}

template <bool use_lds, int NT>
__global__ void __launch_bounds__(NT)
oss_chan_fwd_kernel(oss_chan_params p) {
    extern __shared__ float sm[];
    const int b = blockIdx.x, tid = threadIdx.x, L = p.L, dc = p.dc, Cc = p.Cc, Rc = p.Rc;
    const bool lift = p.cin_w != nullptr;
    float *seq = sm;
    float *ybuf = seq + dc * L;
    float *ycs = ybuf + 2 * dc * L;
    float *red = ycs + L;
    float *ypart = red + kChRed;
    const bool pool_runs = p.pool_part && p.n_part >= 64;
    if (pool_runs) {
        const int ns = max(1, min(8, NT / L)), per = (p.n_part + ns - 1) / ns;
        float *run = ypart;
        for (int idx = tid; idx < ns * L; idx += NT) {
            const int sub = idx / L, l = idx - sub * L;
            const int k0 = sub * per, k1 = min(p.n_part, k0 + per);
            const float *pp = p.pool_part + (size_t)b * p.n_part * L + l;
            float sum = 0.f;
            int k = k0;
            for (; k + 16 <= k1; k += 16) {
                float v[16];
#pragma unroll
                for (int q = 0; q < 16; ++q) v[q] = pp[(size_t)(k + q) * L];
#pragma unroll
                for (int q = 0; q < 16; ++q) sum += v[q];
            }
            for (; k < k1; ++k) sum += pp[(size_t)k * L];
            run[idx] = sum;
        }
        __syncthreads();
        for (int l = tid; l < L; l += NT) {
            float sum = run[l];
            for (int sub = 1; sub < ns; ++sub) sum += run[sub * L + l];
            ycs[l] = sum * p.pool_scale;
        }
        __syncthreads();
    }
    for (int l = tid; l < L; l += NT) {
        float pl;
        if (pool_runs) {
            pl = ycs[l];
            const_cast<float *>(p.pooled)[(size_t)b * L + l] = pl;
        } else if (p.pool_part) {
            const float *pp = p.pool_part + (size_t)b * p.n_part * L + l;
            float sum = 0.f;
            int k = 0;
            for (; k + 8 <= p.n_part; k += 8) {
                float v[8];
#pragma unroll
                for (int q = 0; q < 8; ++q) v[q] = pp[(size_t)(k + q) * L];
#pragma unroll
                for (int q = 0; q < 8; ++q) sum += v[q];
            }
            for (; k < p.n_part; ++k) sum += pp[(size_t)k * L];
            pl = sum * p.pool_scale;
            const_cast<float *>(p.pooled)[(size_t)b * L + l] = pl;
        } else {
            pl = p.pooled[(size_t)b * L + l];
        }
        for (int i = 0; i < dc; ++i) seq[i * L + l] = lift ? __builtin_fmaf(p.cin_w[i], pl, p.cin_b[i]) : pl;
    }
    __syncthreads();
    float *zg = p.zt + (size_t)b * 2 * L * Cc;
    float *dg = p.dts + (size_t)b * 2 * dc * L;
    float *zb, *db, *dlsF = nullptr;
    if constexpr (use_lds) { zb = ypart + 4 * 2 * dc * L; db = zb + 2 * L * Cc; dlsF = db + 2 * dc * L; } else { zb = zg; db = dg; }
    {
        const int ncol = 2 * Cc;
        const int tpc = ncol >= NT ? 1 : NT / ncol;
        for (int col = tid % (ncol < NT ? ncol : NT); col < ncol; col += NT) {
            const int sub = ncol < NT ? tid / ncol : 0;
            if (sub >= tpc) break;
            float wv[4];
#pragma unroll
            for (int i = 0; i < 4; ++i) wv[i] = i < dc ? p.Wxc[col * dc + i] : 0.f;
            const int k = col / Cc, c = col - k * Cc;
#pragma unroll 4
            for (int l = sub; l < L; l += tpc) {
                float s = 0.f;
#pragma unroll
                for (int i = 0; i < 4; ++i)
                    if (i < dc) s = __builtin_fmaf(wv[i], seq[i * L + l], s);
                zb[(k * L + l) * Cc + c] = s;
                if (use_lds) zg[(k * L + l) * Cc + c] = s;
            }
        }
    }
    __syncthreads();
    {
        const int nrow = 2 * dc, tpr = NT / nrow;
        const int row = tid / tpr, sub = tid - row * tpr;
        if (row < nrow) {
            const int k = row / dc;
            const float brow = p.dt_bias[row];
            float wr[8];
#pragma unroll
            for (int r = 0; r < 8; ++r) wr[r] = r < Rc ? p.Wdtc[row * Rc + r] : 0.f;
#pragma unroll 2
            for (int l = sub; l < L; l += tpr) {
                const float *zr = zb + (k * L + l) * Cc;
                float s = 0.f;
#pragma unroll
                for (int r = 0; r < 8; ++r)
                    if (r < Rc) s = __builtin_fmaf(wr[r], zr[r], s);
                for (int r = 8; r < Rc; ++r) s = __builtin_fmaf(p.Wdtc[row * Rc + r], zr[r], s);
                db[row * L + l] = s;
                if constexpr (use_lds) {
                    dg[row * L + l] = s;
                    float e;
                    dlsF[row * L + l] = softplus_thr(s + brow, e);
                }
            }
        }
    }
    __syncthreads();
    static_assert(NT == 512, "wave = (direction, one of four state groups)");
    constexpr int GPD = NT / 128, NPG = kChN / GPD;
    const int wave = __builtin_amdgcn_readfirstlane(tid >> 6), lane = tid & 63;
    {
        const int k = wave / GPD, ng = wave - k * GPD, n0 = ng * NPG;
        float A2[4][NPG], carry[4][NPG], Dv[4];
#pragma unroll
        for (int i = 0; i < 4; ++i) {
            const int row = k * dc + min(i, dc - 1);
            Dv[i] = p.Dsc[row];
#pragma unroll
            for (int nn = 0; nn < NPG; ++nn) { A2[i][nn] = -__expf(p.A_logs[row * kChN + n0 + nn]) * kLog2e; carry[i][nn] = 0.f; }
        }
        const int nchunk = (L + 127) >> 7;
        for (int c = 0; c < nchunk; ++c) {
            const int t0 = c * 128 + 2 * lane;
            const bool v0 = t0 < L, v1 = t0 + 1 < L;
            const int tc0 = min(t0, L - 1), tc1 = min(t0 + 1, L - 1);
            const int l0 = k ? L - 1 - tc0 : tc0, l1 = k ? L - 1 - tc1 : tc1;
            const float *z0 = zb + (k * L + l0) * Cc + Rc + n0, *z1 = zb + (k * L + l1) * Cc + Rc + n0;
            float B0[NPG], B1[NPG], C0[NPG], C1[NPG];
#pragma unroll
            for (int nn = 0; nn < NPG; ++nn) { B0[nn] = z0[nn]; B1[nn] = z1[nn]; C0[nn] = z0[kChN + nn]; C1[nn] = z1[kChN + nn]; }
            float yv0[4], yv1[4];
#pragma unroll
            for (int i = 0; i < 4; ++i) {
                yv0[i] = 0.f; yv1[i] = 0.f;
                if (i < dc) {
                    const int row = k * dc + i;
                    float dl0, dl1;
                    if constexpr (use_lds) { dl0 = dlsF[row * L + l0]; dl1 = dlsF[row * L + l1]; }
                    else {
                        float e;
                        const float bias = p.dt_bias[row];
                        dl0 = softplus_thr(db[row * L + l0] + bias, e);
                        dl1 = softplus_thr(db[row * L + l1] + bias, e);
                    }
                    dl0 = v0 ? dl0 : 0.f;
                    dl1 = v1 ? dl1 : 0.f;
                    const float u0 = seq[i * L + l0], u1 = seq[i * L + l1];
                    float hv0[NPG], hv1[NPG], a0[NPG], a1[NPG], b0[NPG], b1[NPG], P[NPG], h[NPG];
#pragma unroll
                    for (int nn = 0; nn < NPG; ++nn) {
                        a0[nn] = exp2_hw(dl0 * A2[i][nn]); a1[nn] = exp2_hw(dl1 * A2[i][nn]);
                        b0[nn] = dl0 * B0[nn] * u0; b1[nn] = dl1 * B1[nn] * u1;
                        P[nn] = a0[nn] * a1[nn]; h[nn] = __builtin_fmaf(a1[nn], b0[nn], b1[nn]);
                    }
                    segment_scan4_64(P, h);
#pragma unroll
                    for (int nn = 0; nn < NPG; ++nn) {
                        const float hp = shift_from_prev_lane(h[nn], 0.f, false), Pp = shift_from_prev_lane(P[nn], 1.f, false);
                        const float hin = __builtin_fmaf(Pp, carry[i][nn], hp);
                        const float h0 = __builtin_fmaf(a0[nn], hin, b0[nn]), h1 = __builtin_fmaf(a1[nn], h0, b1[nn]);
                        hv0[nn] = h0; hv1[nn] = h1;
                        yv0[i] = __builtin_fmaf(C0[nn], h0, yv0[i]);
                        yv1[i] = __builtin_fmaf(C1[nn], h1, yv1[i]);
                        carry[i][nn] = __int_as_float(__builtin_amdgcn_readlane(__float_as_int(h1), 63));
                    }
                    float *hr = p.hs + (((size_t)b * 2 * dc + row) * L) * kChN + n0;
                    static_assert(NPG == 4, "one 16-byte store per (row, step)");
                    if (v0) *reinterpret_cast<f32x4 *>(hr + (size_t)l0 * kChN) = f32x4{hv0[0], hv0[1], hv0[2], hv0[3]};
                    if (v1) *reinterpret_cast<f32x4 *>(hr + (size_t)l1 * kChN) = f32x4{hv1[0], hv1[1], hv1[2], hv1[3]};
                    if (ng == 0) { yv0[i] = __builtin_fmaf(Dv[i], u0, yv0[i]); yv1[i] = __builtin_fmaf(Dv[i], u1, yv1[i]); }
                }
            }
#pragma unroll
            for (int i = 0; i < 4; ++i) {
                if (i < dc) {
                    float *yr = ypart + (ng * 2 * dc + k * dc + i) * L;
                    if (v0) yr[l0] = yv0[i];
                    if (v1) yr[l1] = yv1[i];
                }
            }
        }
    }
    __syncthreads();
    for (int idx = tid; idx < 2 * dc * L; idx += NT)
        ybuf[idx] = ((ypart[idx] + ypart[2 * dc * L + idx]) + ypart[2 * 2 * dc * L + idx]) + ypart[3 * 2 * dc * L + idx];
    __syncthreads();
    float part = 0.f;
    for (int l = tid; l < L; l += NT) {
        float s = lift ? p.cout_b[0] : 0.f;
        for (int i = 0; i < dc; ++i) s = __builtin_fmaf(lift ? p.cout_w[i] : 1.f, ybuf[i * L + l] + ybuf[(dc + i) * L + l], s);
        ycs[l] = s;
        part += s;
    }
    for (int idx = tid; idx < 2 * dc * L; idx += NT) p.y[(size_t)b * 2 * dc * L + idx] = ybuf[idx];
    const float mu = block_sum<NT>(part, red, tid) / (float)L;
    float q = 0.f;
    for (int l = tid; l < L; l += NT) { const float d = ycs[l] - mu; q = __builtin_fmaf(d, d, q); }
    const float rstd = 1.0f / sqrtf(block_sum<NT>(q, red, tid) / (float)L + 1e-5f);
    for (int l = tid; l < L; l += NT) {
        p.yc[(size_t)b * L + l] = ycs[l];
        p.c[(size_t)b * L + l] = __builtin_fmaf((ycs[l] - mu) * rstd, p.cn_w[l], p.cn_b[l]);
    }
    if (tid == 0) { p.stat[b * 2] = mu; p.stat[b * 2 + 1] = rstd; }
}

struct ChanSlots {
    int cnw, cnb, coutw, coutb, dA, dD, dbias, wdtc, wxc, cinw, cinb, total;
    __host__ __device__ ChanSlots(int L, int dc, int Rc, int Cc) {
        cnw = 0; cnb = L; coutw = 2 * L; coutb = coutw + dc; dA = coutb + 1; dD = dA + 2 * dc * kChN; dbias = dD + 2 * dc;
        wdtc = dbias + 2 * dc; wxc = wdtc + 2 * dc * Rc; cinw = wxc + 2 * Cc * dc; cinb = cinw + dc; total = cinb + dc;
    }
};

template <bool use_lds , int NT>
__global__ void __launch_bounds__(NT)
oss_chan_bwd_kernel(oss_chan_params p, const float *__restrict__ gc , float *__restrict__ dpool,
                    float *__restrict__ gpart, float *__restrict__ dzt, float *__restrict__ ddts, float *__restrict__ dug,
                    int stage_zdt ) {
    extern __shared__ float sm[];
    const int b = blockIdx.x, tid = threadIdx.x, L = p.L, dc = p.dc, Cc = p.Cc, Rc = p.Rc;
    const bool lift = p.cin_w != nullptr;
    const ChanSlots sl(L, dc, Rc, Cc);
    static_assert(NT == 512, "wave = (direction, one of four state groups)");
    constexpr int GPD = NT / 128, NPG = kChN / GPD;
    static_assert(NPG == 4, "16-byte accesses of a group's states");
    const int wave = __builtin_amdgcn_readfirstlane(tid >> 6), lane = tid & 63;
    const int sk = wave / GPD, sng = wave - sk * GPD, sn0 = sng * NPG;
    struct ScanOps { float B0[NPG], B1[NPG], C0[NPG], C1[NPG]; f32x4 hq0[4], hq1[4], hq2[4]; };
    auto fetch_ops = [&](int c, ScanOps &o) {
        const int u0 = c * 128 + 2 * lane;
        const int c0 = min(u0, L - 1), c1 = min(u0 + 1, L - 1), c2 = min(u0 + 2, L - 1);
        const int l0 = sk ? c0 : L - 1 - c0, l1 = sk ? c1 : L - 1 - c1, l2 = sk ? c2 : L - 1 - c2;
        const float *zsrc = p.zt + (size_t)b * 2 * L * Cc;
        const float *z0 = zsrc + (sk * L + l0) * Cc + Rc + sn0, *z1 = zsrc + (sk * L + l1) * Cc + Rc + sn0;
#pragma unroll
        for (int nn = 0; nn < NPG; ++nn) { o.B0[nn] = z0[nn]; o.B1[nn] = z1[nn]; o.C0[nn] = z0[kChN + nn]; o.C1[nn] = z1[kChN + nn]; }
#pragma unroll
        for (int i = 0; i < 4; ++i) {
            const float *hr = p.hs + (((size_t)b * 2 * dc + sk * dc + min(i, dc - 1)) * L) * kChN + sn0;
            o.hq0[i] = *reinterpret_cast<const f32x4 *>(hr + (size_t)l0 * kChN);
            o.hq1[i] = *reinterpret_cast<const f32x4 *>(hr + (size_t)l1 * kChN);
            o.hq2[i] = *reinterpret_cast<const f32x4 *>(hr + (size_t)l2 * kChN);
        }
    };
    ScanOps cur;
    fetch_ops(0, cur);
    float *seq = sm;
    float *dys = seq + dc * L;
    float *dsq = dys + L;
    float *red = dsq + dc * L;
    float *dpl = red + kChRed;
    float *dpu = dpl + 4 * 2 * dc * L;
    float *sWx = dpu + 4 * 2 * dc * L;
    float *zdt = sWx + 2 * Cc * dc;
    float *lds_end = zdt + (stage_zdt ? 2 * L * Rc : 0);
    float *gp = gpart + (size_t)b * sl.total;
    for (int idx = tid; idx < 2 * Cc * dc; idx += NT) sWx[idx] = p.Wxc[idx];
    if (stage_zdt) {
        const float *zsrc = p.zt + (size_t)b * 2 * L * Cc;
        for (int kl = tid; kl < 2 * L; kl += NT)
            for (int r = 0; r < Rc; ++r) zdt[kl * Rc + r] = zsrc[kl * Cc + r];
    }
    const float *db = p.dts + (size_t)b * 2 * dc * L;
    float *dzb, *ddb, *dub, *dlsL = nullptr, *sgsL = nullptr;
    if constexpr (use_lds) {
        dzb = lds_end; ddb = dzb + 2 * L * Cc; dub = ddb + 2 * dc * L;
        dlsL = dub + 2 * dc * L; sgsL = dlsL + 2 * dc * L;
#pragma unroll 4
        for (int idx = tid; idx < 2 * dc * L; idx += NT) {
            const float x = db[idx] + p.dt_bias[idx / L];
            float e;
            dlsL[idx] = softplus_thr(x, e);
            sgsL[idx] = (x <= 20.f) ? e * __builtin_amdgcn_rcpf(1.f + e) : 1.f;
        }
    } else {
        dzb = dzt + (size_t)b * 2 * L * Cc; ddb = ddts + (size_t)b * 2 * dc * L; dub = dug + (size_t)b * 2 * dc * L;
    }
    const float mu = p.stat[b * 2], rstd = p.stat[b * 2 + 1];
    float s1 = 0.f, s2 = 0.f;
    for (int l = tid; l < L; l += NT) {
        const float pl = p.pooled[(size_t)b * L + l];
        for (int i = 0; i < dc; ++i) seq[i * L + l] = lift ? __builtin_fmaf(p.cin_w[i], pl, p.cin_b[i]) : pl;
        const float g0 = gc[(size_t)b * L + l], xh = (p.yc[(size_t)b * L + l] - mu) * rstd, g = g0 * p.cn_w[l];
        gp[sl.cnw + l] = g0 * xh;
        gp[sl.cnb + l] = g0;
        s1 += g;
        s2 = __builtin_fmaf(g, xh, s2);
    }
    const float m1 = block_sum<NT>(s1, red, tid) / (float)L;
    const float m2 = block_sum<NT>(s2, red, tid) / (float)L;
    for (int l = tid; l < L; l += NT) {
        const float xh = (p.yc[(size_t)b * L + l] - mu) * rstd, g = gc[(size_t)b * L + l] * p.cn_w[l];
        dys[l] = rstd * (g - m1 - xh * m2);
    }
    __syncthreads();
    const float *yb = p.y + (size_t)b * 2 * dc * L;
    const float *zb = p.zt + (size_t)b * 2 * L * Cc;
    {
        const int k = sk, ng = sng, n0 = sn0;
        float Av[4][NPG], carry[4][NPG], carry_a[4][NPG], accA[4][NPG], cwv[4];
#pragma unroll
        for (int i = 0; i < 4; ++i) {
            const int row = k * dc + min(i, dc - 1);
            cwv[i] = i < dc ? (lift ? p.cout_w[i] : 1.f) : 0.f;
#pragma unroll
            for (int nn = 0; nn < NPG; ++nn) {
                Av[i][nn] = -__expf(p.A_logs[row * kChN + n0 + nn]);
                carry[i][nn] = 0.f; carry_a[i][nn] = 1.f; accA[i][nn] = 0.f;
            }
        }
        const int nchunk = (L + 127) >> 7;
        for (int c = 0; c < nchunk; ++c) {
            const int u0 = c * 128 + 2 * lane;
            const bool v0 = u0 < L, v1 = u0 + 1 < L, v2 = u0 + 2 < L;
            const int c0 = min(u0, L - 1), c1 = min(u0 + 1, L - 1), c2 = min(u0 + 2, L - 1);
            const int l0 = k ? c0 : L - 1 - c0, l1 = k ? c1 : L - 1 - c1, l2 = k ? c2 : L - 1 - c2;
            ScanOps nxt;
            if (c + 1 < nchunk) fetch_ops(c + 1, nxt);
            float (&B0)[NPG] = cur.B0, (&B1)[NPG] = cur.B1, (&C0)[NPG] = cur.C0, (&C1)[NPG] = cur.C1;
            f32x4 (&hq0)[4] = cur.hq0, (&hq1)[4] = cur.hq1, (&hq2)[4] = cur.hq2;
            const float dys0 = v0 ? dys[l0] : 0.f, dys1 = v1 ? dys[l1] : 0.f;
            float dB0[NPG], dB1[NPG], dC0[NPG], dC1[NPG], ddl0[4], ddl1[4], du0[4], du1[4];
#pragma unroll
            for (int nn = 0; nn < NPG; ++nn) { dB0[nn] = 0.f; dB1[nn] = 0.f; dC0[nn] = 0.f; dC1[nn] = 0.f; }
#pragma unroll
            for (int i = 0; i < 4; ++i) {
                ddl0[i] = 0.f; ddl1[i] = 0.f; du0[i] = 0.f; du1[i] = 0.f;
                if (i < dc) {
                    const int row = k * dc + i;
                    float dl0, dl1;
                    if constexpr (use_lds) { dl0 = dlsL[row * L + l0]; dl1 = dlsL[row * L + l1]; }
                    else {
                        float e;
                        const float bias = p.dt_bias[row];
                        dl0 = softplus_thr(db[row * L + l0] + bias, e);
                        dl1 = softplus_thr(db[row * L + l1] + bias, e);
                    }
                    dl0 = v0 ? dl0 : 0.f;
                    dl1 = v1 ? dl1 : 0.f;
                    const float us0 = seq[i * L + l0], us1 = seq[i * L + l1];
                    const float dy0 = cwv[i] * dys0, dy1 = cwv[i] * dys1;
                    float a0[NPG], a1[NPG], al0[NPG], g0[NPG], g1[NPG], P[NPG], h[NPG];
#pragma unroll
                    for (int nn = 0; nn < NPG; ++nn) {
                        a0[nn] = exp2_hw(dl0 * Av[i][nn] * kLog2e); a1[nn] = exp2_hw(dl1 * Av[i][nn] * kLog2e);
                        al0[nn] = shift_from_prev_lane(a1[nn], carry_a[i][nn], false);
                        g0[nn] = dy0 * C0[nn]; g1[nn] = dy1 * C1[nn];
                        P[nn] = al0[nn] * a0[nn]; h[nn] = __builtin_fmaf(a0[nn], g0[nn], g1[nn]);
                    }
                    segment_scan4_64(P, h);
#pragma unroll
                    for (int nn = 0; nn < NPG; ++nn) {
                        const float A = Av[i][nn];
                        const float hp = shift_from_prev_lane(h[nn], 0.f, false), Pp = shift_from_prev_lane(P[nn], 1.f, false);
                        const float din = __builtin_fmaf(Pp, carry[i][nn], hp);
                        const float dh0 = __builtin_fmaf(al0[nn], din, g0[nn]), dh1 = __builtin_fmaf(a0[nn], dh0, g1[nn]);
                        carry[i][nn] = __int_as_float(__builtin_amdgcn_readlane(__float_as_int(dh1), 63));
                        carry_a[i][nn] = __int_as_float(__builtin_amdgcn_readlane(__float_as_int(a1[nn]), 63));
                        const float h0 = hq0[i][nn], h1 = hq1[i][nn];
                        const float hp0 = v1 ? h1 : 0.f, hp1 = v2 ? hq2[i][nn] : 0.f;
                        dC0[nn] = __builtin_fmaf(dy0, h0, dC0[nn]);
                        dC1[nn] = __builtin_fmaf(dy1, h1, dC1[nn]);
                        dB0[nn] = __builtin_fmaf(dh0 * dl0, us0, dB0[nn]);
                        dB1[nn] = __builtin_fmaf(dh1 * dl1, us1, dB1[nn]);
                        ddl0[i] = __builtin_fmaf(dh0, __builtin_fmaf(A * a0[nn], hp0, B0[nn] * us0), ddl0[i]);
                        ddl1[i] = __builtin_fmaf(dh1, __builtin_fmaf(A * a1[nn], hp1, B1[nn] * us1), ddl1[i]);
                        du0[i] = __builtin_fmaf(dh0 * dl0, B0[nn], du0[i]);
                        du1[i] = __builtin_fmaf(dh1 * dl1, B1[nn], du1[i]);
                        accA[i][nn] = __builtin_fmaf(dh0 * dl0 * a0[nn], hp0, __builtin_fmaf(dh1 * dl1 * a1[nn], hp1, accA[i][nn]));
                    }
                }
            }
            {
                float *dz0 = dzb + (k * L + l0) * Cc + Rc + n0, *dz1 = dzb + (k * L + l1) * Cc + Rc + n0;
#pragma unroll
                for (int nn = 0; nn < NPG; ++nn) {
                    if (v0) { dz0[nn] = dB0[nn]; dz0[kChN + nn] = dC0[nn]; }
                    if (v1) { dz1[nn] = dB1[nn]; dz1[kChN + nn] = dC1[nn]; }
                }
            }
#pragma unroll
            for (int i = 0; i < 4; ++i) {
                if (i < dc) {
                    const int o = (ng * 2 * dc + k * dc + i) * L;
                    if (v0) { dpl[o + l0] = ddl0[i]; dpu[o + l0] = du0[i]; }
                    if (v1) { dpl[o + l1] = ddl1[i]; dpu[o + l1] = du1[i]; }
                }
            }
            if (c + 1 < nchunk) cur = nxt;
        }
#pragma unroll
        for (int i = 0; i < 4; ++i) {
            if (i < dc) {
#pragma unroll
                for (int nn = 0; nn < NPG; ++nn) {
                    const float tA = segment_sum_to_last<64>(accA[i][nn]);
                    if (lane == 63) gp[sl.dA + (k * dc + i) * kChN + n0 + nn] = tA * Av[i][nn];
                }
            }
        }
        __syncthreads();
        if (wave < 2 * dc) {
            const int row = wave, i = row % dc;
            const float Dr = p.Dsc[row], cw = lift ? p.cout_w[i] : 1.f, bias = p.dt_bias[row];
            float sB = 0.f, sD = 0.f;
            for (int l = lane; l < L; l += 64) {
                const int o = row * L + l, st = 2 * dc * L;
                const float tl = ((dpl[o] + dpl[st + o]) + dpl[2 * st + o]) + dpl[3 * st + o];
                const float tu = ((dpu[o] + dpu[st + o]) + dpu[2 * st + o]) + dpu[3 * st + o];
                float sg;
                if constexpr (use_lds) { sg = sgsL[o]; }
                else {
                    const float x = db[o] + bias, e = exp2_hw(x * kLog2e);
                    sg = (x <= 20.f) ? e * __builtin_amdgcn_rcpf(1.f + e) : 1.f;
                }
                const float dy = cw * dys[l], ddt = tl * sg;
                ddb[o] = ddt;
                dub[o] = __builtin_fmaf(dy, Dr, tu);
                sB += ddt;
                sD = __builtin_fmaf(dy, seq[i * L + l], sD);
            }
            const float tB = segment_sum_to_last<64>(sB), tD = segment_sum_to_last<64>(sD);
            if (lane == 63) { gp[sl.dbias + row] = tB; gp[sl.dD + row] = tD; }
        }
        if (wave <= dc) {
            const int o = wave;
            float a = 0.f;
            if (lift) {
                for (int l = lane; l < L; l += 64)
                    a = o < dc ? __builtin_fmaf(dys[l], yb[o * L + l] + yb[(dc + o) * L + l], a) : a + dys[l];
            }
            const float t = segment_sum_to_last<64>(a);
            if (lane == 63) gp[sl.coutw + o] = t;
        }
    }
    __syncthreads();
    {
        const int ncol = 2 * Rc;
        const int tpc = ncol >= NT ? 1 : NT / ncol;
        for (int col = tid % (ncol < NT ? ncol : NT); col < ncol; col += NT) {
            const int sub = ncol < NT ? tid / ncol : 0;
            if (sub >= tpc) break;
            const int k = col / Rc, r = col - k * Rc;
            float wv[4];
#pragma unroll
            for (int i = 0; i < 4; ++i) wv[i] = i < dc ? p.Wdtc[(k * dc + i) * Rc + r] : 0.f;
#pragma unroll 4
            for (int l = sub; l < L; l += tpc) {
                float s = 0.f;
#pragma unroll
                for (int i = 0; i < 4; ++i)
                    if (i < dc) s = __builtin_fmaf(wv[i], ddb[(k * dc + i) * L + l], s);
                dzb[(k * L + l) * Cc + r] = s;
            }
        }
    }
    __syncthreads();
    for (int idx = tid; idx < dc * L; idx += NT) {
        const int i = idx / L, l = idx - i * L;
        float s = dub[i * L + l] + dub[(dc + i) * L + l];
        for (int k = 0; k < 2; ++k) {
            const float *dz = dzb + (k * L + l) * Cc;
            const float *wx = sWx + k * Cc * dc + i;
#pragma unroll 8
            for (int c = 0; c < Cc; ++c) s = __builtin_fmaf(wx[c * dc], dz[c], s);
        }
        dsq[idx] = s;
    }
    __syncthreads();
    for (int l = tid; l < L; l += NT) {
        float s = 0.f;
        for (int i = 0; i < dc; ++i) s = lift ? __builtin_fmaf(p.cin_w[i], dsq[i * L + l], s) : s + dsq[i * L + l];
        dpool[(size_t)b * L + l] = s;
    }
    const int n_wdtc = 2 * dc * Rc, n_wxc = 2 * Cc * dc;
    for (int o = tid; o < n_wdtc + n_wxc + 2 * dc; o += NT) {
        float s = 0.f;
        if (o < n_wdtc) {
            const int row = o / Rc, r = o - row * Rc, k = row / dc;
            if (stage_zdt) {
#pragma unroll 8
                for (int l = 0; l < L; ++l) s = __builtin_fmaf(ddb[row * L + l], zdt[(k * L + l) * Rc + r], s);
            } else {
#pragma unroll 8
                for (int l = 0; l < L; ++l) s = __builtin_fmaf(ddb[row * L + l], zb[(k * L + l) * Cc + r], s);
            }
            gp[sl.wdtc + o] = s;
        } else if (o < n_wdtc + n_wxc) {
            const int q = o - n_wdtc, i = q % dc, kc = q / dc, k = kc / Cc, c = kc - k * Cc;
#pragma unroll 8
            for (int l = 0; l < L; ++l) s = __builtin_fmaf(dzb[(k * L + l) * Cc + c], seq[i * L + l], s);
            gp[sl.wxc + q] = s;
        } else {
            const int q = o - n_wdtc - n_wxc, i = q % dc;
            if (lift) {
                if (q < dc) { for (int l = 0; l < L; ++l) s = __builtin_fmaf(dsq[i * L + l], p.pooled[(size_t)b * L + l], s); }
                else        { for (int l = 0; l < L; ++l) s += dsq[i * L + l]; }
            }
            gp[sl.cinw + q] = s;
        }
    }
}

__global__ void __launch_bounds__(256)
oss_chan_grad_finish(const float *__restrict__ gpart, float *__restrict__ gsum, int B, int NP) {
    const int j = blockIdx.x * 256 + threadIdx.x;
    if (j >= NP) return;
    float s = 0.f;
    for (int b = 0; b < B; ++b) s += gpart[(size_t)b * NP + j];
    gsum[j] = s;
}

template <typename T>
__global__ void __launch_bounds__(256)
oss_rowsum_kernel(const T *__restrict__ a, const T *__restrict__ bmul, float *__restrict__ out, int C, int P, int64_t asb,
                  int64_t asc, int64_t bsb, int64_t bsc, float alpha) {
    __shared__ float red[4];
    const int row = blockIdx.x, b = row / C, c = row - b * C, tid = threadIdx.x;
    const T *ap = a + b * asb + c * asc;
    const T *bp = bmul ? bmul + b * bsb + c * bsc : nullptr;
    float s = 0.f;
    const bool vec = (P % 8 == 0) && ((reinterpret_cast<uintptr_t>(ap) | reinterpret_cast<uintptr_t>(bp)) & 15u) == 0;
    if (vec) {
        const T *bq = bp ? bp : ap;
        for (int p = tid * 8; p < P; p += 4096) {
            const bool two = p + 2048 < P;
            const int p2 = two ? p + 2048 : p;
            float a0[8], b0[8], a1[8], b1[8];
            load_items<8>(ap + p, 8, true, a0);
            load_items<8>(bq + p, 8, true, b0);
            load_items<8>(ap + p2, 8, true, a1);
            load_items<8>(bq + p2, 8, true, b1);
#pragma unroll
            for (int i = 0; i < 8; ++i) s = bp ? __builtin_fmaf(a0[i], b0[i], s) : s + a0[i];
            if (two) {
#pragma unroll
                for (int i = 0; i < 8; ++i) s = bp ? __builtin_fmaf(a1[i], b1[i], s) : s + a1[i];
            }
        }
    } else {
        for (int p = tid; p < P; p += 256) s = bp ? __builtin_fmaf(to_f32(ap[p]), to_f32(bp[p]), s) : s + to_f32(ap[p]);
    }
    const float t = block_sum<256>(s, red, tid);
    if (tid == 0) out[row] = t * alpha;
}

template <typename T>
__global__ void __launch_bounds__(256)
oss_row_affine_kernel(const T *__restrict__ x, const float *__restrict__ mul, const float *__restrict__ add, T *__restrict__ y,
                      int C, int P, int64_t xsb, int64_t xsc, float alpha) {
    const int row = blockIdx.y, b = row / C, c = row - b * C;
    const T *xp = x + b * xsb + c * xsc;
    T *yp = y + (size_t)row * P;
    const float *mp = mul ? mul + row : reinterpret_cast<const float *>(x), *ap = add ? add + row : mp;
    const float mv = *mp, av = *ap;
    const int p = (blockIdx.x * 256 + threadIdx.x) * 8;
    if (p >= P) return;
    const bool vec = (P % 8 == 0) && ((reinterpret_cast<uintptr_t>(xp) | reinterpret_cast<uintptr_t>(yp)) & 15u) == 0;
    float v[8];
    const int valid = min(8, P - p);
    load_items<8>(xp + p, valid, vec, v);
    const float sc = mul ? 1.f + mv : 1.f, sh = add ? alpha * av : 0.f;
#pragma unroll
    for (int i = 0; i < 8; ++i) v[i] = __builtin_fmaf(v[i], sc, sh);
    store_items<8>(yp + p, valid, vec, v);
}

size_t chan_grad_floats(int L, int dc, int Rc, int Cc) { return (size_t)ChanSlots(L, dc, Rc, Cc).total; }

constexpr size_t kChanLdsMax = 160 * 1024;
static int chan_enable_lds(const void *kern, size_t bytes) {
    if (bytes <= 48 * 1024) return 0;
    return (int)hipFuncSetAttribute(kern, hipFuncAttributeMaxDynamicSharedMemorySize, (int)kChanLdsMax);
}

static int chan_check(const oss_chan_params &p) {
    if (p.B <= 0 || p.L <= 0 || p.dc < 1 || p.dc > 4 || p.Rc < 1 || p.Cc != p.Rc + 2 * kChN) return OSS_ERR_SHAPE;
    if (!p.pooled || !p.Wxc || !p.Wdtc || !p.dt_bias || !p.A_logs || !p.Dsc || !p.cn_w || !p.cn_b || !p.zt || !p.dts || !p.hs ||
        !p.y || !p.yc || !p.stat || !p.c)
        return OSS_ERR_NULL;
    if ((p.cin_w != nullptr) != (p.cout_w != nullptr)) return OSS_ERR_NULL;
    if (p.cin_w && (!p.cin_b || !p.cout_b)) return OSS_ERR_NULL;
    return 0;
}

int chan_fwd(const oss_chan_params &p, hipStream_t s) {
    if (int e = chan_check(p)) return e;
    size_t smem = sizeof(float) * ((size_t)(3 * p.dc + 1) * p.L + kChRed + 4 * 2 * (size_t)p.dc * p.L);
    if (smem > kChanLdsMax) return OSS_ERR_SHAPE;
    const size_t extra = sizeof(float) * (2 * (size_t)p.L * p.Cc + 4 * (size_t)p.dc * p.L);
    const int use_lds = smem + extra <= kChanLdsMax ? 1 : 0;
    if (use_lds) smem += extra;
    if (use_lds) {
        if (int e = chan_enable_lds(reinterpret_cast<const void *>(oss_chan_fwd_kernel<true, kChNT>), smem)) return e;
        hipLaunchKernelGGL((oss_chan_fwd_kernel<true, kChNT>), dim3(p.B), dim3(kChNT), smem, s, p);
    } else {
        if (int e = chan_enable_lds(reinterpret_cast<const void *>(oss_chan_fwd_kernel<false, kChNT>), smem)) return e;
        hipLaunchKernelGGL((oss_chan_fwd_kernel<false, kChNT>), dim3(p.B), dim3(kChNT), smem, s, p);
    }
    return (int)hipGetLastError();
}

int chan_bwd(const oss_chan_params &p, const float *gc, float *dpool, float *gsum, float *scratch, hipStream_t s) {
    if (int e = chan_check(p)) return e;
    if (!gc || !dpool || !gsum || !scratch) return OSS_ERR_NULL;
    size_t smem = sizeof(float) * ((size_t)(2 * p.dc + 1) * p.L + kChRed + 2 * 4 * 2 * (size_t)p.dc * p.L + 2 * (size_t)p.Cc * p.dc);
    if (smem > kChanLdsMax) return OSS_ERR_SHAPE;
    const size_t zdt_bytes = sizeof(float) * 2 * (size_t)p.L * p.Rc;
    const int stage_zdt = smem + zdt_bytes <= kChanLdsMax ? 1 : 0;
    if (stage_zdt) smem += zdt_bytes;
    const size_t extra = sizeof(float) * (2 * (size_t)p.L * p.Cc + 8 * (size_t)p.dc * p.L);
    const int use_lds = smem + extra <= kChanLdsMax ? 1 : 0;
    if (use_lds) smem += extra;
    if (use_lds) {
        if (int e = chan_enable_lds(reinterpret_cast<const void *>(oss_chan_bwd_kernel<true, kChNT>), smem)) return e;
    } else {
        if (int e = chan_enable_lds(reinterpret_cast<const void *>(oss_chan_bwd_kernel<false, kChNT>), smem)) return e;
    }
    const size_t np = chan_grad_floats(p.L, p.dc, p.Rc, p.Cc);
    float *gpart = scratch;
    float *dzt = gpart + (size_t)p.B * np;
    float *ddts = dzt + (size_t)p.B * 2 * p.L * p.Cc;
    float *dug = ddts + (size_t)p.B * 2 * p.dc * p.L;
    if (use_lds) hipLaunchKernelGGL((oss_chan_bwd_kernel<true, kChNT>), dim3(p.B), dim3(kChNT), smem, s, p, gc, dpool, gpart, dzt, ddts, dug, stage_zdt);
    else         hipLaunchKernelGGL((oss_chan_bwd_kernel<false, kChNT>), dim3(p.B), dim3(kChNT), smem, s, p, gc, dpool, gpart, dzt, ddts, dug, stage_zdt);
    if (defer_finish())
        defer_sum(gpart, p.B, np, np, gsum, np, nullptr);
    else
        hipLaunchKernelGGL(oss_chan_grad_finish, dim3((unsigned)((np + 255) / 256)), dim3(256), 0, s, gpart, gsum, p.B, (int)np);
    return (int)hipGetLastError();
}

size_t chan_bwd_scratch_floats(int B, int L, int dc, int Rc, int Cc) {
    return (size_t)B * (chan_grad_floats(L, dc, Rc, Cc) + 2 * (size_t)L * Cc + 4 * (size_t)dc * L);
}

int rowsum(oss_dtype io, const void *a, const void *bmul, float *out, int B, int C, int P, int64_t asb, int64_t asc, int64_t bsb,
           int64_t bsc, float alpha, hipStream_t s) {
    return io_dispatch(io, [&](auto tag) {
        using T = typename decltype(tag)::type;
        hipLaunchKernelGGL(oss_rowsum_kernel<T>, dim3(B * C), dim3(256), 0, s, reinterpret_cast<const T *>(a), reinterpret_cast<const T *>(bmul),
                           out, C, P, asb, asc, bsb, bsc, alpha);
        return (int)hipGetLastError();
    });
}

int row_affine(oss_dtype io, const void *x, const float *mul, const float *add, void *y, int B, int C, int P, int64_t xsb,
               int64_t xsc, float alpha, hipStream_t s) {
    return io_dispatch(io, [&](auto tag) {
        using T = typename decltype(tag)::type;
        if ((long)B * C > 65535) return OSS_ERR_SHAPE;
        hipLaunchKernelGGL(oss_row_affine_kernel<T>, dim3((P + 2047) / 2048, B * C), dim3(256), 0, s, reinterpret_cast<const T *>(x), mul, add,
                           reinterpret_cast<T *>(y), C, P, xsb, xsc, alpha);
        return (int)hipGetLastError();
    });
}

}
```

### vmambair_amd/ops/channel.py

```python
from __future__ import annotations

import contextlib
import os
from typing import List, Optional

import torch

from .. import _capi
from ._common import (_DT, _LIB, _check, _f32c, _fork_for_wgrad, _keep, _keep_views, _planes, _ptr)


def chan_supported(dc: int, n_state: int, d_inner: int) -> bool:
    lds_bwd = 4 * ((18 * dc + 1) * d_inner + 2 * dc * (dc + 32 + 8) + 8)
    return n_state == 16 and 1 <= dc <= 4 and lds_bwd <= 160 * 1024


def _chan_params(B, L, pooled, prm, saved, c):
    cin_w, cin_b, Wxc, Wdtc, dt_bias, A_logs, Dsc, cout_w, cout_b, cn_w, cn_b = prm
    zt, dts, hs, y, yc, stat = saved
    P = _capi.ChanParams()
    P.B, P.L, P.dc, P.Rc, P.Cc = B, L, Wdtc.shape[1], Wdtc.shape[2], Wxc.shape[1]
    for name, t in (("pooled", pooled), ("cin_w", cin_w), ("cin_b", cin_b), ("Wxc", Wxc), ("Wdtc", Wdtc), ("dt_bias", dt_bias),
                    ("A_logs", A_logs), ("Dsc", Dsc), ("cout_w", cout_w), ("cout_b", cout_b), ("cn_w", cn_w), ("cn_b", cn_b),
                    ("zt", zt), ("dts", dts), ("hs", hs), ("y", y), ("yc", yc), ("stat", stat), ("c", c)):
        setattr(P, name, _ptr(t))
    P.pool_part, P.n_part, P.pool_scale = None, 0, 0.0
    return P


def chan_gate_fwd(y2: torch.Tensor, cin_w: Optional[torch.Tensor], cin_b: Optional[torch.Tensor], Wxc: torch.Tensor,
                  Wdtc: torch.Tensor, dt_bias: torch.Tensor, A_logs: torch.Tensor, Dsc: torch.Tensor,
                  cout_w: Optional[torch.Tensor], cout_b: Optional[torch.Tensor], cn_w: torch.Tensor, cn_b: torch.Tensor,
                  mul_mode: bool, pool_part: Optional[torch.Tensor] = None) -> List[torch.Tensor]:
    _check(y2.is_cuda and y2.dim() == 4 and y2.dtype in _DT, "chan_gate: y2 must be a (B, d, H, W) GPU tensor")
    B, d, H, W = y2.shape
    y2 = _planes(y2)
    prm = tuple(_f32c(t) for t in (cin_w, cin_b, Wxc, Wdtc, dt_bias, A_logs, Dsc, cout_w, cout_b, cn_w, cn_b))
    dc, Rc, Cc = Wdtc.shape[1], Wdtc.shape[2], Wxc.shape[1]
    _check(tuple(Wxc.shape) == (2, Cc, dc) and tuple(Wdtc.shape) == (2, dc, Rc) and Cc == Rc + 32 and
           tuple(A_logs.shape) == (2 * dc, 16) and cn_w.numel() == d, "chan_gate: parameter shapes do not match SS2D_1's")
    dev = y2.device
    f = dict(dtype=torch.float32, device=dev)
    pooled, c = torch.empty((B, d), **f), torch.empty((B, d), **f)
    saved = (torch.empty((B, 2, d, Cc), **f), torch.empty((B, 2 * dc, d), **f), torch.empty((B, 2 * dc, d, 16), **f),
             torch.empty((B, 2 * dc, d), **f), torch.empty((B, d), **f), torch.empty((B, 2), **f))
    out = torch.empty((B, d, H, W), dtype=y2.dtype, device=dev)
    if y2.numel() == 0:
        return [out, c, pooled, *saved]
    lib = _capi.load()
    with torch.cuda.device(dev):
        st = torch.cuda.current_stream().cuda_stream
        P = _chan_params(B, d, pooled, prm, saved, c)
        if pool_part is not None and pool_part.numel():
            _check(pool_part.dtype == torch.float32 and pool_part.is_contiguous() and pool_part.dim() == 3 and
                   pool_part.shape[0] == B and pool_part.shape[2] == d, "chan_gate: pool_part must be contiguous (B, tiles, d) float32")
            P.pool_part, P.n_part, P.pool_scale = pool_part.data_ptr(), pool_part.shape[1], 1.0 / (H * W)
        else:
            _capi.check(lib.oss_rowsum(_DT[y2.dtype], y2.data_ptr(), None, pooled.data_ptr(), B, d, H * W, y2.stride(0), y2.stride(1),
                                       0, 0, 1.0 / (H * W), st), "oss_rowsum")
        _capi.check(lib.oss_chan_fwd(P, st), "oss_chan_fwd")
        _capi.check(lib.oss_row_affine(_DT[y2.dtype], y2.data_ptr(), c.data_ptr() if mul_mode else None,
                                       None if mul_mode else c.data_ptr(), out.data_ptr(), B, d, H * W, y2.stride(0),
                                       y2.stride(1), 1.0, st), "oss_row_affine")
    return [out, c, pooled, *saved]


def chan_gate_bwd(g: torch.Tensor, y2: torch.Tensor, c: torch.Tensor, pooled: torch.Tensor, zt: torch.Tensor, dts: torch.Tensor,
                  hs: torch.Tensor, y: torch.Tensor, yc: torch.Tensor, stat: torch.Tensor, cin_w: Optional[torch.Tensor],
                  cin_b: Optional[torch.Tensor], Wxc: torch.Tensor, Wdtc: torch.Tensor, dt_bias: torch.Tensor,
                  A_logs: torch.Tensor, Dsc: torch.Tensor, cout_w: Optional[torch.Tensor], cout_b: Optional[torch.Tensor],
                  cn_w: torch.Tensor, cn_b: torch.Tensor, mul_mode: bool, fold: bool = False) -> List[torch.Tensor]:
    B, d, H, W = y2.shape
    y2, g = _planes(y2), _planes(g)
    if g.dtype != y2.dtype:
        g = g.to(y2.dtype)
    prm = tuple(_f32c(t) for t in (cin_w, cin_b, Wxc, Wdtc, dt_bias, A_logs, Dsc, cout_w, cout_b, cn_w, cn_b))
    dc, Rc, Cc = Wdtc.shape[1], Wdtc.shape[2], Wxc.shape[1]
    dev = y2.device
    lib = _capi.load()
    f = dict(dtype=torch.float32, device=dev)
    gc, dpool = torch.empty((B, d), **f), torch.empty((B, d), **f)
    grads = torch.empty((int(lib.oss_chan_grad_floats(d, dc, Rc, Cc)),), **f)
    scratch = torch.empty((int(lib.oss_chan_bwd_scratch_floats(B, d, dc, Rc, Cc)),), **f)
    dy2 = None if fold else torch.empty((B, d, H, W), dtype=y2.dtype, device=dev)
    with torch.cuda.device(dev):
        st = torch.cuda.current_stream().cuda_stream
        _capi.check(lib.oss_rowsum(_DT[y2.dtype], g.data_ptr(), y2.data_ptr() if mul_mode else None, gc.data_ptr(), B, d, H * W,
                                   g.stride(0), g.stride(1), y2.stride(0), y2.stride(1), 1.0, st), "oss_rowsum")
        _capi.check(lib.oss_chan_bwd(_chan_params(B, d, pooled, prm, (zt, dts, hs, y, yc, stat), c), gc.data_ptr(),
                                     dpool.data_ptr(), grads.data_ptr(), scratch.data_ptr(), st), "oss_chan_bwd")
        _keep(scratch, grads)
        if fold:
            return [dpool, grads]
        _capi.check(lib.oss_row_affine(_DT[y2.dtype], g.data_ptr(), c.data_ptr() if mul_mode else None, dpool.data_ptr(),
                                       dy2.data_ptr(), B, d, H * W, g.stride(0), g.stride(1), 1.0 / (H * W), st), "oss_row_affine")
    return [dy2, grads]


_CH = "Tensor? cin_w, Tensor? cin_b, Tensor Wxc, Tensor Wdtc, Tensor dt_bias, Tensor A_logs, Tensor Dsc, Tensor? cout_w, " \
      "Tensor? cout_b, Tensor cn_w, Tensor cn_b, bool mul_mode"
_LIB.define(f"chan_gate_fwd(Tensor y2, {_CH}, Tensor? pool_part=None) -> Tensor[]")
_LIB.define(f"chan_gate_bwd(Tensor g, Tensor y2, Tensor c, Tensor pooled, Tensor zt, Tensor dts, Tensor hs, Tensor y, Tensor yc, "
            f"Tensor stat, {_CH}, bool fold=False) -> Tensor[]")
_LIB.impl("chan_gate_fwd", chan_gate_fwd, "CUDA")
_LIB.impl("chan_gate_bwd", chan_gate_bwd, "CUDA")


class ChannelGateFn(torch.autograd.Function):

    @staticmethod
    def forward(ctx, y2, cin_w, cin_b, Wxc, Wdtc, dt_bias, A_logs, Dsc, cout_w, cout_b, cn_w, cn_b, mul_mode):
        out, *saved = torch.ops.vmambair.chan_gate_fwd(y2, cin_w, cin_b, Wxc, Wdtc, dt_bias, A_logs, Dsc, cout_w, cout_b,
                                                       cn_w, cn_b, mul_mode)
        ctx.mul_mode = mul_mode
        ctx.save_for_backward(y2, *saved, cin_w, cin_b, Wxc, Wdtc, dt_bias, A_logs, Dsc, cout_w, cout_b, cn_w, cn_b)
        return out

    @staticmethod
    def backward(ctx, g):
        y2, c, pooled, zt, dts, hs, y, yc, stat, cin_w, cin_b, Wxc, Wdtc, dt_bias, A_logs, Dsc, cout_w, cout_b, cn_w, cn_b = \
            ctx.saved_tensors
        dy2, gr = torch.ops.vmambair.chan_gate_bwd(g, y2, c, pooled, zt, dts, hs, y, yc, stat, cin_w, cin_b, Wxc, Wdtc, dt_bias,
                                                   A_logs, Dsc, cout_w, cout_b, cn_w, cn_b, ctx.mul_mode)
        L, dc, Rc, Cc = cn_w.numel(), Wdtc.shape[1], Wdtc.shape[2], Wxc.shape[1]
        o = [0]

        def take(n, like):
            t = gr[o[0]:o[0] + n]
            o[0] += n
            return None if like is None else t.view(like.shape).to(like.dtype)

        d_cnw, d_cnb = take(L, cn_w), take(L, cn_b)
        d_coutw, d_coutb = take(dc, cout_w), take(1, cout_b)
        d_A, d_D, d_bias = take(2 * dc * 16, A_logs), take(2 * dc, Dsc), take(2 * dc, dt_bias)
        d_wdtc, d_wxc = take(2 * dc * Rc, Wdtc), take(2 * Cc * dc, Wxc)
        d_cinw, d_cinb = take(dc, cin_w), take(dc, cin_b)
        _keep_views(gr, (d_cnw, d_cnb, d_coutw, d_coutb, d_A, d_D, d_bias, d_wdtc, d_wxc, d_cinw, d_cinb))
        return dy2, d_cinw, d_cinb, d_wxc, d_wdtc, d_bias, d_A, d_D, d_coutw, d_coutb, d_cnw, d_cnb, None


POOL_FUSED = os.environ.get("VMAMBAIR_POOL_FUSED", "1") == "1"


class NormChannelGateFn(torch.autograd.Function):

    @staticmethod
    def forward(ctx, y, ln_w, ln_b, z, out_dtype, gate_grad_into, cin_w, cin_b, Wxc, Wdtc, dt_bias, A_logs, Dsc, cout_w, cout_b,
                cn_w, cn_b, mul_mode):
        from .layernorm import _DT_CODE
        res = torch.ops.vmambair.ln_nchw_fwd(y, ln_w, ln_b, z, _DT_CODE[out_dtype], POOL_FUSED)
        y2, mean, rstd = res[0], res[1], res[2]
        pool = res[3] if len(res) > 3 and res[3].numel() else None
        out, *saved = torch.ops.vmambair.chan_gate_fwd(y2, cin_w, cin_b, Wxc, Wdtc, dt_bias, A_logs, Dsc, cout_w, cout_b,
                                                       cn_w, cn_b, mul_mode, pool)
        ctx.mul_mode, ctx.gate_grad_into, ctx.has_lnb = mul_mode, gate_grad_into, ln_b is not None
        ctx.save_for_backward(y, ln_w, ln_b, z, mean, rstd, y2, *saved, cin_w, cin_b, Wxc, Wdtc, dt_bias, A_logs, Dsc, cout_w, cout_b,
                              cn_w, cn_b)
        return out

    @staticmethod
    def backward(ctx, g):
        (y, ln_w, ln_b, z, mean, rstd, y2, c, pooled, zt, dts, hs, ys, yc, stat, cin_w, cin_b, Wxc, Wdtc, dt_bias, A_logs, Dsc,
         cout_w, cout_b, cn_w, cn_b) = ctx.saved_tensors
        g = g.contiguous()
        if g.dtype != y2.dtype:
            g = g.to(y2.dtype)
        dpool, gr = torch.ops.vmambair.chan_gate_bwd(g, y2, c, pooled, zt, dts, hs, ys, yc, stat, cin_w, cin_b, Wxc, Wdtc, dt_bias,
                                                     A_logs, Dsc, cout_w, cout_b, cn_w, cn_b, ctx.mul_mode, True)
        into = None
        if ctx.gate_grad_into is not None and z.dtype == g.dtype:
            into = ctx.gate_grad_into[0].half(ctx.gate_grad_into[1], z)
        H, W = y2.shape[2], y2.shape[3]
        dy_, dz, dlw, dlb = torch.ops.vmambair.ln_nchw_bwd(y, ln_w, ln_b, z, g, mean, rstd, None, into,
                                                          c if ctx.mul_mode else None, dpool, 1.0 / (H * W))
        if into is not None and dz.numel() == 0 and z.numel() != 0:
            dz = into
        L, dc, Rc, Cc = cn_w.numel(), Wdtc.shape[1], Wdtc.shape[2], Wxc.shape[1]
        o = [0]

        def take(n, like):
            t = gr[o[0]:o[0] + n]
            o[0] += n
            return None if like is None else t.view(like.shape).to(like.dtype)

        d_cnw, d_cnb = take(L, cn_w), take(L, cn_b)
        d_coutw, d_coutb = take(dc, cout_w), take(1, cout_b)
        d_A, d_D, d_bias = take(2 * dc * 16, A_logs), take(2 * dc, Dsc), take(2 * dc, dt_bias)
        d_wdtc, d_wxc = take(2 * dc * Rc, Wdtc), take(2 * Cc * dc, Wxc)
        d_cinw, d_cinb = take(dc, cin_w), take(dc, cin_b)
        _keep_views(gr, (d_cnw, d_cnb, d_coutw, d_coutb, d_A, d_D, d_bias, d_wdtc, d_wxc, d_cinw, d_cinb))
        return (dy_, dlw.to(ln_w.dtype), dlb.to(ln_b.dtype) if ctx.has_lnb else None, dz.to(z.dtype), None, None,
                d_cinw, d_cinb, d_wxc, d_wdtc, d_bias, d_A, d_D, d_coutw, d_coutb, d_cnw, d_cnb, None)
```

Before: 251.2 images/s.

## Fold channel-scan projections into per-channel affine coefficients of pooled input

Because the channel-attention input is a rank-1 affine function of the pooled value, the x_proj and dt_proj outputs (B, C, delta pre-activation) are rewritten as a*pl+b with coefficient tables computed per block. The forward no longer materialises or saves zt/dts, and the backward recomputes B, C and delta on the fly and accumulates gradients into coefficient-level reductions instead of per-position dzt/ddts buffers. This removes global scratch traffic and LDS staging in exchange for some recomputation and a new reduction scheme. The channel kernel is small relative to the whole UNet step.

```diff
diff --git a/include/vmambair_oss.h b/include/vmambair_oss.h
--- a/include/vmambair_oss.h
+++ b/include/vmambair_oss.h
@@ -200,8 +200,6 @@
     const float *Dsc;
     const float *cout_w, *cout_b;
     const float *cn_w, *cn_b;
-    float *zt;
-    float *dts;
     float *hs;
     float *y;
     float *yc;
@@ -348,7 +346,7 @@
 
 int oss_f32_matmul_modes(void);
 
-#define OSS_ABI_VERSION 9
+#define OSS_ABI_VERSION 10
 int oss_abi_version(void);
 size_t oss_abi_struct_bytes(int which);
 
diff --git a/vmambair_amd/csrc/oss_capi.hip b/vmambair_amd/csrc/oss_capi.hip
--- a/vmambair_amd/csrc/oss_capi.hip
+++ b/vmambair_amd/csrc/oss_capi.hip
@@ -617,7 +617,7 @@
 }
 
 int oss_chan_fwd(const oss_chan_params *p, oss_stream_t stream) {
-    fam_count(FAM_CHAN, p ? 4.0 * p->B * ((double)p->L * (2.0 * p->Cc + 2.0 * p->dc * 18.0 + 3.0) + (p->pool_part ? (double)p->n_part * p->L : p->L)) : 0.0);
+    fam_count(FAM_CHAN, p ? 4.0 * p->B * ((double)p->L * (2.0 * p->dc * 17.0 + 3.0) + (p->pool_part ? (double)p->n_part * p->L : p->L)) : 0.0);
     if (!p) return OSS_ERR_NULL;
     return chan_fwd(*p, reinterpret_cast<hipStream_t>(stream));
 }
@@ -626,7 +626,7 @@
 size_t oss_chan_bwd_scratch_floats(int B, int L, int dc, int Rc, int Cc) { return chan_bwd_scratch_floats(B, L, dc, Rc, Cc); }
 
 int oss_chan_bwd(const oss_chan_params *p, const float *gc, float *dpooled, float *grads, float *scratch, oss_stream_t stream) {
-    fam_count(FAM_CHAN, p ? 4.0 * p->B * ((double)p->L * (2.0 * p->Cc + 2.0 * p->dc * 18.0 + 5.0)) : 0.0);
+    fam_count(FAM_CHAN, p ? 4.0 * p->B * ((double)p->L * (2.0 * p->dc * 17.0 + 5.0)) : 0.0);
     if (!p) return OSS_ERR_NULL;
     return chan_bwd(*p, gc, dpooled, grads, scratch, reinterpret_cast<hipStream_t>(stream));
 }
diff --git a/vmambair_amd/csrc/oss_channel.hip b/vmambair_amd/csrc/oss_channel.hip
--- a/vmambair_amd/csrc/oss_channel.hip
+++ b/vmambair_amd/csrc/oss_channel.hip
@@ -26,20 +26,77 @@
     return v;
 }
 
-template <bool use_lds, int NT>
+__host__ __device__ inline int chan_tab_floats(int dc, int Cc) { return 4 * Cc + 6 * dc; }
+struct ChanTab {
+    float *za, *zb, *ta, *tb, *cw, *cb;
+    __device__ ChanTab(float *t, int dc, int Cc) { za = t; zb = za + 2 * Cc; ta = zb + 2 * Cc; tb = ta + 2 * dc; cw = tb + 2 * dc; cb = cw + dc; }
+};
+
+__device__ __forceinline__ void chan_zcoef(const oss_chan_params &p, int col, float &a, float &b) {
+    const bool lift = p.cin_w != nullptr;
+    a = 0.f; b = 0.f;
+    for (int i = 0; i < p.dc; ++i) {
+        const float w = p.Wxc[col * p.dc + i];
+        a = __builtin_fmaf(w, lift ? p.cin_w[i] : 1.f, a);
+        b = __builtin_fmaf(w, lift ? p.cin_b[i] : 0.f, b);
+    }
+}
+
+template <int NT>
+__device__ __forceinline__ void chan_coef_table(const oss_chan_params &p, float *tab, int tid) {
+    const int dc = p.dc, Cc = p.Cc, Rc = p.Rc;
+    const ChanTab T(tab, dc, Cc);
+    for (int o = NT - 1 - tid; o < 2 * Cc + 3 * dc; o += NT) {
+        if (o < 2 * Cc) {
+            float a, b;
+            chan_zcoef(p, o, a, b);
+            T.za[o] = a; T.zb[o] = b;
+        } else if (o < 2 * Cc + 2 * dc) {
+            const int row = o - 2 * Cc, k = row / dc;
+            float a = 0.f, b = 0.f;
+            for (int r = 0; r < Rc; ++r) {
+                float za, zb;
+                chan_zcoef(p, k * Cc + r, za, zb);
+                const float w = p.Wdtc[row * Rc + r];
+                a = __builtin_fmaf(w, za, a);
+                b = __builtin_fmaf(w, zb, b);
+            }
+            T.ta[row] = a; T.tb[row] = b;
+        } else {
+            const int i = o - 2 * Cc - 2 * dc;
+            T.cw[i] = p.cin_w ? p.cin_w[i] : 1.f;
+            T.cb[i] = p.cin_w ? p.cin_b[i] : 0.f;
+        }
+    }
+}
+
+__device__ __forceinline__ float wave_uniform(float v) { return __int_as_float(__builtin_amdgcn_readfirstlane(__float_as_int(v))); }
+
+__device__ __forceinline__ float chan_delta(float ta, float tb, float bias, float pl, float &sg) {
+    const float x = __builtin_fmaf(ta, pl, tb) + bias;
+    float e;
+    const float d = softplus_thr(x, e);
+    sg = (x <= 20.f) ? e * __builtin_amdgcn_rcpf(1.f + e) : 1.f;
+    return d;
+}
+
+template <int NT>
 __global__ void __launch_bounds__(NT)
 oss_chan_fwd_kernel(oss_chan_params p) {
     extern __shared__ float sm[];
     const int b = blockIdx.x, tid = threadIdx.x, L = p.L, dc = p.dc, Cc = p.Cc, Rc = p.Rc;
     const bool lift = p.cin_w != nullptr;
-    float *seq = sm;
-    float *ybuf = seq + dc * L;
+    float *pls = sm;
+    float *ybuf = pls + L;
     float *ycs = ybuf + 2 * dc * L;
     float *red = ycs + L;
     float *ypart = red + kChRed;
+    float *tab = ypart + 4 * 2 * dc * L;
+    chan_coef_table<NT>(p, tab, tid);
     const bool pool_runs = p.pool_part && p.n_part >= 64;
+    const int ns = max(1, min(8, NT / L));
     if (pool_runs) {
-        const int ns = max(1, min(8, NT / L)), per = (p.n_part + ns - 1) / ns;
+        const int per = (p.n_part + ns - 1) / ns;
         float *run = ypart;
         for (int idx = tid; idx < ns * L; idx += NT) {
             const int sub = idx / L, l = idx - sub * L;
@@ -58,17 +115,13 @@
             run[idx] = sum;
         }
         __syncthreads();
-        for (int l = tid; l < L; l += NT) {
-            float sum = run[l];
-            for (int sub = 1; sub < ns; ++sub) sum += run[sub * L + l];
-            ycs[l] = sum * p.pool_scale;
-        }
-        __syncthreads();
     }
     for (int l = tid; l < L; l += NT) {
         float pl;
         if (pool_runs) {
-            pl = ycs[l];
+            float sum = ypart[l];
+            for (int sub = 1; sub < ns; ++sub) sum += ypart[sub * L + l];
+            pl = sum * p.pool_scale;
             const_cast<float *>(p.pooled)[(size_t)b * L + l] = pl;
         } else if (p.pool_part) {
             const float *pp = p.pool_part + (size_t)b * p.n_part * L + l;
@@ -87,60 +140,7 @@
         } else {
             pl = p.pooled[(size_t)b * L + l];
         }
-        for (int i = 0; i < dc; ++i) seq[i * L + l] = lift ? __builtin_fmaf(p.cin_w[i], pl, p.cin_b[i]) : pl;
-    }
-    __syncthreads();
-    float *zg = p.zt + (size_t)b * 2 * L * Cc;
-    float *dg = p.dts + (size_t)b * 2 * dc * L;
-    float *zb, *db, *dlsF = nullptr;
-    if constexpr (use_lds) { zb = ypart + 4 * 2 * dc * L; db = zb + 2 * L * Cc; dlsF = db + 2 * dc * L; } else { zb = zg; db = dg; }
-    {
-        const int ncol = 2 * Cc;
-        const int tpc = ncol >= NT ? 1 : NT / ncol;
-        for (int col = tid % (ncol < NT ? ncol : NT); col < ncol; col += NT) {
-            const int sub = ncol < NT ? tid / ncol : 0;
-            if (sub >= tpc) break;
-            float wv[4];
-#pragma unroll
-            for (int i = 0; i < 4; ++i) wv[i] = i < dc ? p.Wxc[col * dc + i] : 0.f;
-            const int k = col / Cc, c = col - k * Cc;
-#pragma unroll 4
-            for (int l = sub; l < L; l += tpc) {
-                float s = 0.f;
-#pragma unroll
-                for (int i = 0; i < 4; ++i)
-                    if (i < dc) s = __builtin_fmaf(wv[i], seq[i * L + l], s);
-                zb[(k * L + l) * Cc + c] = s;
-                if (use_lds) zg[(k * L + l) * Cc + c] = s;
-            }
-        }
-    }
-    __syncthreads();
-    {
-        const int nrow = 2 * dc, tpr = NT / nrow;
-        const int row = tid / tpr, sub = tid - row * tpr;
-        if (row < nrow) {
-            const int k = row / dc;
-            const float brow = p.dt_bias[row];
-            float wr[8];
-#pragma unroll
-            for (int r = 0; r < 8; ++r) wr[r] = r < Rc ? p.Wdtc[row * Rc + r] : 0.f;
-#pragma unroll 2
-            for (int l = sub; l < L; l += tpr) {
-                const float *zr = zb + (k * L + l) * Cc;
-                float s = 0.f;
-#pragma unroll
-                for (int r = 0; r < 8; ++r)
-                    if (r < Rc) s = __builtin_fmaf(wr[r], zr[r], s);
-                for (int r = 8; r < Rc; ++r) s = __builtin_fmaf(p.Wdtc[row * Rc + r], zr[r], s);
-                db[row * L + l] = s;
-                if constexpr (use_lds) {
-                    dg[row * L + l] = s;
-                    float e;
-                    dlsF[row * L + l] = softplus_thr(s + brow, e);
-                }
-            }
-        }
+        pls[l] = pl;
     }
     __syncthreads();
     static_assert(NT == 512, "wave = (direction, one of four state groups)");
@@ -148,11 +148,22 @@
     const int wave = __builtin_amdgcn_readfirstlane(tid >> 6), lane = tid & 63;
     {
         const int k = wave / GPD, ng = wave - k * GPD, n0 = ng * NPG;
-        float A2[4][NPG], carry[4][NPG], Dv[4];
+        const ChanTab T(tab, dc, Cc);
+        float A2[4][NPG], carry[4][NPG], Dv[4], ta[4], tb[4], bias[4], cw[4], cb[4];
+        float zaB[NPG], zbB[NPG], zaC[NPG], zbC[NPG];
+#pragma unroll
+        for (int nn = 0; nn < NPG; ++nn) {
+            const int cB = k * Cc + Rc + n0 + nn, cC = cB + kChN;
+            zaB[nn] = wave_uniform(T.za[cB]); zbB[nn] = wave_uniform(T.zb[cB]);
+            zaC[nn] = wave_uniform(T.za[cC]); zbC[nn] = wave_uniform(T.zb[cC]);
+        }
 #pragma unroll
         for (int i = 0; i < 4; ++i) {
-            const int row = k * dc + min(i, dc - 1);
+            const int ic = min(i, dc - 1), row = k * dc + ic;
             Dv[i] = p.Dsc[row];
+            bias[i] = p.dt_bias[row];
+            ta[i] = wave_uniform(T.ta[row]); tb[i] = wave_uniform(T.tb[row]);
+            cw[i] = wave_uniform(T.cw[ic]); cb[i] = wave_uniform(T.cb[ic]);
 #pragma unroll
             for (int nn = 0; nn < NPG; ++nn) { A2[i][nn] = -__expf(p.A_logs[row * kChN + n0 + nn]) * kLog2e; carry[i][nn] = 0.f; }
         }
@@ -162,27 +173,24 @@
             const bool v0 = t0 < L, v1 = t0 + 1 < L;
             const int tc0 = min(t0, L - 1), tc1 = min(t0 + 1, L - 1);
             const int l0 = k ? L - 1 - tc0 : tc0, l1 = k ? L - 1 - tc1 : tc1;
-            const float *z0 = zb + (k * L + l0) * Cc + Rc + n0, *z1 = zb + (k * L + l1) * Cc + Rc + n0;
+            const float p0 = pls[l0], p1 = pls[l1];
             float B0[NPG], B1[NPG], C0[NPG], C1[NPG];
 #pragma unroll
-            for (int nn = 0; nn < NPG; ++nn) { B0[nn] = z0[nn]; B1[nn] = z1[nn]; C0[nn] = z0[kChN + nn]; C1[nn] = z1[kChN + nn]; }
+            for (int nn = 0; nn < NPG; ++nn) {
+                B0[nn] = __builtin_fmaf(zaB[nn], p0, zbB[nn]); B1[nn] = __builtin_fmaf(zaB[nn], p1, zbB[nn]);
+                C0[nn] = __builtin_fmaf(zaC[nn], p0, zbC[nn]); C1[nn] = __builtin_fmaf(zaC[nn], p1, zbC[nn]);
+            }
             float yv0[4], yv1[4];
 #pragma unroll
             for (int i = 0; i < 4; ++i) {
                 yv0[i] = 0.f; yv1[i] = 0.f;
                 if (i < dc) {
                     const int row = k * dc + i;
-                    float dl0, dl1;
-                    if constexpr (use_lds) { dl0 = dlsF[row * L + l0]; dl1 = dlsF[row * L + l1]; }
-                    else {
-                        float e;
-                        const float bias = p.dt_bias[row];
-                        dl0 = softplus_thr(db[row * L + l0] + bias, e);
-                        dl1 = softplus_thr(db[row * L + l1] + bias, e);
-                    }
+                    float sg;
+                    float dl0 = chan_delta(ta[i], tb[i], bias[i], p0, sg), dl1 = chan_delta(ta[i], tb[i], bias[i], p1, sg);
                     dl0 = v0 ? dl0 : 0.f;
                     dl1 = v1 ? dl1 : 0.f;
-                    const float u0 = seq[i * L + l0], u1 = seq[i * L + l1];
+                    const float u0 = __builtin_fmaf(cw[i], p0, cb[i]), u1 = __builtin_fmaf(cw[i], p1, cb[i]);
                     float hv0[NPG], hv1[NPG], a0[NPG], a1[NPG], b0[NPG], b1[NPG], P[NPG], h[NPG];
 #pragma unroll
                     for (int nn = 0; nn < NPG; ++nn) {
@@ -249,75 +257,60 @@
     }
 };
 
-template <bool use_lds , int NT>
+constexpr int kChCg = 32;
+
+template <int NT>
 __global__ void __launch_bounds__(NT)
 oss_chan_bwd_kernel(oss_chan_params p, const float *__restrict__ gc , float *__restrict__ dpool,
-                    float *__restrict__ gpart, float *__restrict__ dzt, float *__restrict__ ddts, float *__restrict__ dug,
-                    int stage_zdt ) {
+                    float *__restrict__ gpart) {
     extern __shared__ float sm[];
     const int b = blockIdx.x, tid = threadIdx.x, L = p.L, dc = p.dc, Cc = p.Cc, Rc = p.Rc;
     const bool lift = p.cin_w != nullptr;
     const ChanSlots sl(L, dc, Rc, Cc);
     static_assert(NT == 512, "wave = (direction, one of four state groups)");
-    constexpr int GPD = NT / 128, NPG = kChN / GPD;
+    constexpr int GPD = NT / 128, NPG = kChN / GPD, NW = NT / 64;
     static_assert(NPG == 4, "16-byte accesses of a group's states");
     const int wave = __builtin_amdgcn_readfirstlane(tid >> 6), lane = tid & 63;
     const int sk = wave / GPD, sng = wave - sk * GPD, sn0 = sng * NPG;
-    struct ScanOps { float B0[NPG], B1[NPG], C0[NPG], C1[NPG]; f32x4 hq0[4], hq1[4], hq2[4]; };
-    auto fetch_ops = [&](int c, ScanOps &o) {
+    struct RowOps { f32x4 h0, h1, h2; };
+    auto chunk_pos = [&](int c, int &l0, int &l1, int &l2) {
         const int u0 = c * 128 + 2 * lane;
         const int c0 = min(u0, L - 1), c1 = min(u0 + 1, L - 1), c2 = min(u0 + 2, L - 1);
-        const int l0 = sk ? c0 : L - 1 - c0, l1 = sk ? c1 : L - 1 - c1, l2 = sk ? c2 : L - 1 - c2;
-        const float *zsrc = p.zt + (size_t)b * 2 * L * Cc;
-        const float *z0 = zsrc + (sk * L + l0) * Cc + Rc + sn0, *z1 = zsrc + (sk * L + l1) * Cc + Rc + sn0;
-#pragma unroll
-        for (int nn = 0; nn < NPG; ++nn) { o.B0[nn] = z0[nn]; o.B1[nn] = z1[nn]; o.C0[nn] = z0[kChN + nn]; o.C1[nn] = z1[kChN + nn]; }
-#pragma unroll
-        for (int i = 0; i < 4; ++i) {
-            const float *hr = p.hs + (((size_t)b * 2 * dc + sk * dc + min(i, dc - 1)) * L) * kChN + sn0;
-            o.hq0[i] = *reinterpret_cast<const f32x4 *>(hr + (size_t)l0 * kChN);
-            o.hq1[i] = *reinterpret_cast<const f32x4 *>(hr + (size_t)l1 * kChN);
-            o.hq2[i] = *reinterpret_cast<const f32x4 *>(hr + (size_t)l2 * kChN);
-        }
+        l0 = sk ? c0 : L - 1 - c0; l1 = sk ? c1 : L - 1 - c1; l2 = sk ? c2 : L - 1 - c2;
     };
-    ScanOps cur;
-    fetch_ops(0, cur);
-    float *seq = sm;
-    float *dys = seq + dc * L;
-    float *dsq = dys + L;
-    float *red = dsq + dc * L;
-    float *dpl = red + kChRed;
-    float *dpu = dpl + 4 * 2 * dc * L;
-    float *sWx = dpu + 4 * 2 * dc * L;
-    float *zdt = sWx + 2 * Cc * dc;
-    float *lds_end = zdt + (stage_zdt ? 2 * L * Rc : 0);
+    auto fetch_row = [&](int c, int i, RowOps &o) {
+        int l0, l1, l2;
+        chunk_pos(c, l0, l1, l2);
+        const float *hr = p.hs + (((size_t)b * 2 * dc + sk * dc + min(i, dc - 1)) * L) * kChN + sn0;
+        o.h0 = *reinterpret_cast<const f32x4 *>(hr + (size_t)l0 * kChN);
+        o.h1 = *reinterpret_cast<const f32x4 *>(hr + (size_t)l1 * kChN);
+        o.h2 = *reinterpret_cast<const f32x4 *>(hr + (size_t)l2 * kChN);
+    };
+    auto fetch_pooled = [&](int c, float &p0, float &p1) {
+        int l0, l1, l2;
+        chunk_pos(c, l0, l1, l2);
+        p0 = p.pooled[(size_t)b * L + l0];
+        p1 = p.pooled[(size_t)b * L + l1];
+    };
+    RowOps hq[2];
+    float pc0, pc1;
+    fetch_pooled(0, pc0, pc1);
+    fetch_row(0, 0, hq[0]);
+    float *dys = sm;
+    float *red = dys + L;
+    float *tab = red + kChRed;
+    float *dpp = tab + chan_tab_floats(dc, Cc);
+    float *cgw = dpp + NW * L;
+    float *dza = cgw + NW * kChCg;
+    float *dzb = dza + 2 * Cc;
+    float *dta = dzb + 2 * Cc;
+    float *dtb = dta + 2 * dc;
     float *gp = gpart + (size_t)b * sl.total;
-    for (int idx = tid; idx < 2 * Cc * dc; idx += NT) sWx[idx] = p.Wxc[idx];
-    if (stage_zdt) {
-        const float *zsrc = p.zt + (size_t)b * 2 * L * Cc;
-        for (int kl = tid; kl < 2 * L; kl += NT)
-            for (int r = 0; r < Rc; ++r) zdt[kl * Rc + r] = zsrc[kl * Cc + r];
-    }
-    const float *db = p.dts + (size_t)b * 2 * dc * L;
-    float *dzb, *ddb, *dub, *dlsL = nullptr, *sgsL = nullptr;
-    if constexpr (use_lds) {
-        dzb = lds_end; ddb = dzb + 2 * L * Cc; dub = ddb + 2 * dc * L;
-        dlsL = dub + 2 * dc * L; sgsL = dlsL + 2 * dc * L;
-#pragma unroll 4
-        for (int idx = tid; idx < 2 * dc * L; idx += NT) {
-            const float x = db[idx] + p.dt_bias[idx / L];
-            float e;
-            dlsL[idx] = softplus_thr(x, e);
-            sgsL[idx] = (x <= 20.f) ? e * __builtin_amdgcn_rcpf(1.f + e) : 1.f;
-        }
-    } else {
-        dzb = dzt + (size_t)b * 2 * L * Cc; ddb = ddts + (size_t)b * 2 * dc * L; dub = dug + (size_t)b * 2 * dc * L;
-    }
+    chan_coef_table<NT>(p, tab, tid);
     const float mu = p.stat[b * 2], rstd = p.stat[b * 2 + 1];
     float s1 = 0.f, s2 = 0.f;
     for (int l = tid; l < L; l += NT) {
-        const float pl = p.pooled[(size_t)b * L + l];
-        for (int i = 0; i < dc; ++i) seq[i * L + l] = lift ? __builtin_fmaf(p.cin_w[i], pl, p.cin_b[i]) : pl;
+#pragma clang fp contract(off)
         const float g0 = gc[(size_t)b * L + l], xh = (p.yc[(size_t)b * L + l] - mu) * rstd, g = g0 * p.cn_w[l];
         gp[sl.cnw + l] = g0 * xh;
         gp[sl.cnb + l] = g0;
@@ -327,19 +320,34 @@
     const float m1 = block_sum<NT>(s1, red, tid) / (float)L;
     const float m2 = block_sum<NT>(s2, red, tid) / (float)L;
     for (int l = tid; l < L; l += NT) {
+#pragma clang fp contract(off)
         const float xh = (p.yc[(size_t)b * L + l] - mu) * rstd, g = gc[(size_t)b * L + l] * p.cn_w[l];
         dys[l] = rstd * (g - m1 - xh * m2);
     }
     __syncthreads();
     const float *yb = p.y + (size_t)b * 2 * dc * L;
-    const float *zb = p.zt + (size_t)b * 2 * L * Cc;
+    const ChanTab T(tab, dc, Cc);
     {
         const int k = sk, ng = sng, n0 = sn0;
-        float Av[4][NPG], carry[4][NPG], carry_a[4][NPG], accA[4][NPG], cwv[4];
+        float Av[4][NPG], carry[4][NPG], carry_a[4][NPG], accA[4][NPG], cwv[4], Dv[4], ta[4], tb[4], bias[4], cw[4], cb[4];
+        float zaB[NPG], zbB[NPG], zaC[NPG], zbC[NPG];
+        float gzaB[NPG], gzbB[NPG], gzaC[NPG], gzbC[NPG], gta[4], gtb[4], gcw[4], gcb[4], accD[4];
+#pragma unroll
+        for (int nn = 0; nn < NPG; ++nn) {
+            const int cB = k * Cc + Rc + n0 + nn, cC = cB + kChN;
+            zaB[nn] = wave_uniform(T.za[cB]); zbB[nn] = wave_uniform(T.zb[cB]);
+            zaC[nn] = wave_uniform(T.za[cC]); zbC[nn] = wave_uniform(T.zb[cC]);
+            gzaB[nn] = 0.f; gzbB[nn] = 0.f; gzaC[nn] = 0.f; gzbC[nn] = 0.f;
+        }
 #pragma unroll
         for (int i = 0; i < 4; ++i) {
-            const int row = k * dc + min(i, dc - 1);
+            const int ic = min(i, dc - 1), row = k * dc + ic;
             cwv[i] = i < dc ? (lift ? p.cout_w[i] : 1.f) : 0.f;
+            Dv[i] = p.Dsc[row];
+            bias[i] = p.dt_bias[row];
+            ta[i] = wave_uniform(T.ta[row]); tb[i] = wave_uniform(T.tb[row]);
+            cw[i] = wave_uniform(T.cw[ic]); cb[i] = wave_uniform(T.cb[ic]);
+            gta[i] = 0.f; gtb[i] = 0.f; gcw[i] = 0.f; gcb[i] = 0.f; accD[i] = 0.f;
 #pragma unroll
             for (int nn = 0; nn < NPG; ++nn) {
                 Av[i][nn] = -__expf(p.A_logs[row * kChN + n0 + nn]);
@@ -350,39 +358,37 @@
         for (int c = 0; c < nchunk; ++c) {
             const int u0 = c * 128 + 2 * lane;
             const bool v0 = u0 < L, v1 = u0 + 1 < L, v2 = u0 + 2 < L;
-            const int c0 = min(u0, L - 1), c1 = min(u0 + 1, L - 1), c2 = min(u0 + 2, L - 1);
-            const int l0 = k ? c0 : L - 1 - c0, l1 = k ? c1 : L - 1 - c1, l2 = k ? c2 : L - 1 - c2;
-            ScanOps nxt;
-            if (c + 1 < nchunk) fetch_ops(c + 1, nxt);
-            float (&B0)[NPG] = cur.B0, (&B1)[NPG] = cur.B1, (&C0)[NPG] = cur.C0, (&C1)[NPG] = cur.C1;
-            f32x4 (&hq0)[4] = cur.hq0, (&hq1)[4] = cur.hq1, (&hq2)[4] = cur.hq2;
+            const int c0 = min(u0, L - 1), c1 = min(u0 + 1, L - 1);
+            const int l0 = k ? c0 : L - 1 - c0, l1 = k ? c1 : L - 1 - c1;
+            const float p0 = pc0, p1 = pc1;
+            if (c + 1 < nchunk) fetch_pooled(c + 1, pc0, pc1);
+            float B0[NPG], B1[NPG];
+#pragma unroll
+            for (int nn = 0; nn < NPG; ++nn) { B0[nn] = __builtin_fmaf(zaB[nn], p0, zbB[nn]); B1[nn] = __builtin_fmaf(zaB[nn], p1, zbB[nn]); }
             const float dys0 = v0 ? dys[l0] : 0.f, dys1 = v1 ? dys[l1] : 0.f;
-            float dB0[NPG], dB1[NPG], dC0[NPG], dC1[NPG], ddl0[4], ddl1[4], du0[4], du1[4];
-#pragma unroll
-            for (int nn = 0; nn < NPG; ++nn) { dB0[nn] = 0.f; dB1[nn] = 0.f; dC0[nn] = 0.f; dC1[nn] = 0.f; }
+            float dp0 = 0.f, dp1 = 0.f;
 #pragma unroll
             for (int i = 0; i < 4; ++i) {
-                ddl0[i] = 0.f; ddl1[i] = 0.f; du0[i] = 0.f; du1[i] = 0.f;
                 if (i < dc) {
-                    const int row = k * dc + i;
-                    float dl0, dl1;
-                    if constexpr (use_lds) { dl0 = dlsL[row * L + l0]; dl1 = dlsL[row * L + l1]; }
-                    else {
-                        float e;
-                        const float bias = p.dt_bias[row];
-                        dl0 = softplus_thr(db[row * L + l0] + bias, e);
-                        dl1 = softplus_thr(db[row * L + l1] + bias, e);
-                    }
+                    const bool last = i + 1 == dc, wrap_same = last && (i & 1) == 0;
+                    if (!last) fetch_row(c, i + 1, hq[(i + 1) & 1]);
+                    else if (!wrap_same && c + 1 < nchunk) fetch_row(c + 1, 0, hq[0]);
+                    const RowOps hr = hq[i & 1];
+                    float sg0, sg1;
+                    float dl0 = chan_delta(ta[i], tb[i], bias[i], p0, sg0), dl1 = chan_delta(ta[i], tb[i], bias[i], p1, sg1);
                     dl0 = v0 ? dl0 : 0.f;
                     dl1 = v1 ? dl1 : 0.f;
-                    const float us0 = seq[i * L + l0], us1 = seq[i * L + l1];
+                    const float us0 = __builtin_fmaf(cw[i], p0, cb[i]), us1 = __builtin_fmaf(cw[i], p1, cb[i]);
                     const float dy0 = cwv[i] * dys0, dy1 = cwv[i] * dys1;
+                    const float up0 = us0 * p0, up1 = us1 * p1, dyp0 = dy0 * p0, dyp1 = dy1 * p1;
+                    float ddl0 = 0.f, ddl1 = 0.f, du0 = 0.f, du1 = 0.f;
+                    float sB0 = 0.f, sB1 = 0.f, sC0 = 0.f, sC1 = 0.f;
                     float a0[NPG], a1[NPG], al0[NPG], g0[NPG], g1[NPG], P[NPG], h[NPG];
 #pragma unroll
                     for (int nn = 0; nn < NPG; ++nn) {
                         a0[nn] = exp2_hw(dl0 * Av[i][nn] * kLog2e); a1[nn] = exp2_hw(dl1 * Av[i][nn] * kLog2e);
                         al0[nn] = shift_from_prev_lane(a1[nn], carry_a[i][nn], false);
-                        g0[nn] = dy0 * C0[nn]; g1[nn] = dy1 * C1[nn];
+                        g0[nn] = dy0 * __builtin_fmaf(zaC[nn], p0, zbC[nn]); g1[nn] = dy1 * __builtin_fmaf(zaC[nn], p1, zbC[nn]);
                         P[nn] = al0[nn] * a0[nn]; h[nn] = __builtin_fmaf(a0[nn], g0[nn], g1[nn]);
                     }
                     segment_scan4_64(P, h);
@@ -394,41 +400,57 @@
                         const float dh0 = __builtin_fmaf(al0[nn], din, g0[nn]), dh1 = __builtin_fmaf(a0[nn], dh0, g1[nn]);
                         carry[i][nn] = __int_as_float(__builtin_amdgcn_readlane(__float_as_int(dh1), 63));
                         carry_a[i][nn] = __int_as_float(__builtin_amdgcn_readlane(__float_as_int(a1[nn]), 63));
-                        const float h0 = hq0[i][nn], h1 = hq1[i][nn];
-                        const float hp0 = v1 ? h1 : 0.f, hp1 = v2 ? hq2[i][nn] : 0.f;
-                        dC0[nn] = __builtin_fmaf(dy0, h0, dC0[nn]);
-                        dC1[nn] = __builtin_fmaf(dy1, h1, dC1[nn]);
-                        dB0[nn] = __builtin_fmaf(dh0 * dl0, us0, dB0[nn]);
-                        dB1[nn] = __builtin_fmaf(dh1 * dl1, us1, dB1[nn]);
-                        ddl0[i] = __builtin_fmaf(dh0, __builtin_fmaf(A * a0[nn], hp0, B0[nn] * us0), ddl0[i]);
-                        ddl1[i] = __builtin_fmaf(dh1, __builtin_fmaf(A * a1[nn], hp1, B1[nn] * us1), ddl1[i]);
-                        du0[i] = __builtin_fmaf(dh0 * dl0, B0[nn], du0[i]);
-                        du1[i] = __builtin_fmaf(dh1 * dl1, B1[nn], du1[i]);
-                        accA[i][nn] = __builtin_fmaf(dh0 * dl0 * a0[nn], hp0, __builtin_fmaf(dh1 * dl1 * a1[nn], hp1, accA[i][nn]));
+                        const float h0 = hr.h0[nn], h1 = hr.h1[nn];
+                        const float hp0 = v1 ? h1 : 0.f, hp1 = v2 ? hr.h2[nn] : 0.f;
+                        const float x0 = dh0 * dl0, x1 = dh1 * dl1;
+                        sB0 = __builtin_fmaf(zaB[nn], x0, sB0); sB1 = __builtin_fmaf(zaB[nn], x1, sB1);
+                        sC0 = __builtin_fmaf(zaC[nn], h0, sC0); sC1 = __builtin_fmaf(zaC[nn], h1, sC1);
+                        gzaB[nn] = __builtin_fmaf(x0, up0, __builtin_fmaf(x1, up1, gzaB[nn]));
+                        gzbB[nn] = __builtin_fmaf(x0, us0, __builtin_fmaf(x1, us1, gzbB[nn]));
+                        gzaC[nn] = __builtin_fmaf(dyp0, h0, __builtin_fmaf(dyp1, h1, gzaC[nn]));
+                        gzbC[nn] = __builtin_fmaf(dy0, h0, __builtin_fmaf(dy1, h1, gzbC[nn]));
+                        ddl0 = __builtin_fmaf(dh0, __builtin_fmaf(A * a0[nn], hp0, B0[nn] * us0), ddl0);
+                        ddl1 = __builtin_fmaf(dh1, __builtin_fmaf(A * a1[nn], hp1, B1[nn] * us1), ddl1);
+                        du0 = __builtin_fmaf(x0, B0[nn], du0);
+                        du1 = __builtin_fmaf(x1, B1[nn], du1);
+                        accA[i][nn] = __builtin_fmaf(x0 * a0[nn], hp0, __builtin_fmaf(x1 * a1[nn], hp1, accA[i][nn]));
                     }
+                    if (wrap_same && c + 1 < nchunk) fetch_row(c + 1, 0, hq[0]);
+                    if (ng == 0) {
+                        du0 = __builtin_fmaf(dy0, Dv[i], du0); du1 = __builtin_fmaf(dy1, Dv[i], du1);
+                        accD[i] = __builtin_fmaf(dy0, us0, __builtin_fmaf(dy1, us1, accD[i]));
+                    }
+                    const float gd0 = v0 ? ddl0 * sg0 : 0.f, gd1 = v1 ? ddl1 * sg1 : 0.f;
+                    dp0 = __builtin_fmaf(ta[i], gd0, __builtin_fmaf(cw[i], du0, dp0));
+                    dp1 = __builtin_fmaf(ta[i], gd1, __builtin_fmaf(cw[i], du1, dp1));
+                    dp0 = __builtin_fmaf(us0, sB0, __builtin_fmaf(dy0, sC0, dp0));
+                    dp1 = __builtin_fmaf(us1, sB1, __builtin_fmaf(dy1, sC1, dp1));
+                    gta[i] = __builtin_fmaf(gd0, p0, __builtin_fmaf(gd1, p1, gta[i]));
+                    gtb[i] += gd0 + gd1;
+                    gcw[i] = __builtin_fmaf(du0, p0, __builtin_fmaf(du1, p1, gcw[i]));
+                    gcb[i] += du0 + du1;
                 }
             }
-            {
-                float *dz0 = dzb + (k * L + l0) * Cc + Rc + n0, *dz1 = dzb + (k * L + l1) * Cc + Rc + n0;
-#pragma unroll
-                for (int nn = 0; nn < NPG; ++nn) {
-                    if (v0) { dz0[nn] = dB0[nn]; dz0[kChN + nn] = dC0[nn]; }
-                    if (v1) { dz1[nn] = dB1[nn]; dz1[kChN + nn] = dC1[nn]; }
-                }
-            }
-#pragma unroll
-            for (int i = 0; i < 4; ++i) {
-                if (i < dc) {
-                    const int o = (ng * 2 * dc + k * dc + i) * L;
-                    if (v0) { dpl[o + l0] = ddl0[i]; dpu[o + l0] = du0[i]; }
-                    if (v1) { dpl[o + l1] = ddl1[i]; dpu[o + l1] = du1[i]; }
-                }
-            }
-            if (c + 1 < nchunk) cur = nxt;
+            if (v0) dpp[wave * L + l0] = dp0;
+            if (v1) dpp[wave * L + l1] = dp1;
+        }
+        float *cg = cgw + wave * kChCg;
+#pragma unroll
+        for (int nn = 0; nn < NPG; ++nn) {
+            const float t0 = segment_sum_to_last<64>(gzaB[nn]), t1 = segment_sum_to_last<64>(gzbB[nn]);
+            const float t2 = segment_sum_to_last<64>(gzaC[nn]), t3 = segment_sum_to_last<64>(gzbC[nn]);
+            if (lane == 63) { cg[nn] = t0; cg[4 + nn] = t1; cg[8 + nn] = t2; cg[12 + nn] = t3; }
         }
 #pragma unroll
         for (int i = 0; i < 4; ++i) {
             if (i < dc) {
+                const float t0 = segment_sum_to_last<64>(gta[i]), t1 = segment_sum_to_last<64>(gtb[i]);
+                const float t2 = segment_sum_to_last<64>(gcw[i]), t3 = segment_sum_to_last<64>(gcb[i]);
+                const float tD = segment_sum_to_last<64>(accD[i]);
+                if (lane == 63) {
+                    cg[16 + i] = t0; cg[20 + i] = t1; cg[24 + i] = t2; cg[28 + i] = t3;
+                    if (ng == 0) gp[sl.dD + k * dc + i] = tD;
+                }
 #pragma unroll
                 for (int nn = 0; nn < NPG; ++nn) {
                     const float tA = segment_sum_to_last<64>(accA[i][nn]);
@@ -436,105 +458,76 @@
                 }
             }
         }
-        __syncthreads();
-        if (wave < 2 * dc) {
-            const int row = wave, i = row % dc;
-            const float Dr = p.Dsc[row], cw = lift ? p.cout_w[i] : 1.f, bias = p.dt_bias[row];
-            float sB = 0.f, sD = 0.f;
-            for (int l = lane; l < L; l += 64) {
-                const int o = row * L + l, st = 2 * dc * L;
-                const float tl = ((dpl[o] + dpl[st + o]) + dpl[2 * st + o]) + dpl[3 * st + o];
-                const float tu = ((dpu[o] + dpu[st + o]) + dpu[2 * st + o]) + dpu[3 * st + o];
-                float sg;
-                if constexpr (use_lds) { sg = sgsL[o]; }
-                else {
-                    const float x = db[o] + bias, e = exp2_hw(x * kLog2e);
-                    sg = (x <= 20.f) ? e * __builtin_amdgcn_rcpf(1.f + e) : 1.f;
+    }
+    __syncthreads();
+    auto group_sum = [&](int row, int off) {
+        const float *q = cgw + (row / dc) * GPD * kChCg + off + row % dc;
+        return ((q[0] + q[kChCg]) + q[2 * kChCg]) + q[3 * kChCg];
+    };
+    for (int o = tid; o < 2 * Cc + 2 * dc; o += NT) {
+        if (o < 2 * Cc) {
+            const int k = o / Cc, c = o - k * Cc;
+            float a = 0.f, bb = 0.f;
+            if (c < Rc) {
+                for (int i = 0; i < dc; ++i) {
+                    const float w = p.Wdtc[(k * dc + i) * Rc + c];
+                    a = __builtin_fmaf(w, group_sum(k * dc + i, 16), a);
+                    bb = __builtin_fmaf(w, group_sum(k * dc + i, 20), bb);
                 }
-                const float dy = cw * dys[l], ddt = tl * sg;
-                ddb[o] = ddt;
-                dub[o] = __builtin_fmaf(dy, Dr, tu);
-                sB += ddt;
-                sD = __builtin_fmaf(dy, seq[i * L + l], sD);
-            }
-            const float tB = segment_sum_to_last<64>(sB), tD = segment_sum_to_last<64>(sD);
-            if (lane == 63) { gp[sl.dbias + row] = tB; gp[sl.dD + row] = tD; }
-        }
-        if (wave <= dc) {
-            const int o = wave;
-            float a = 0.f;
+            } else {
+                const int n = (c - Rc) % kChN, isC = (c - Rc) / kChN;
+                const float *q = cgw + (k * GPD + n / NPG) * kChCg + isC * 8 + n % NPG;
+                a = q[0]; bb = q[4];
+            }
+            dza[o] = a; dzb[o] = bb;
+        } else {
+            const int row = o - 2 * Cc;
+            const float a = group_sum(row, 16), bb = group_sum(row, 20);
+            dta[row] = a; dtb[row] = bb;
+            gp[sl.dbias + row] = bb;
+        }
+    }
+    for (int l = tid; l < L; l += NT) {
+        float s = dpp[l];
+#pragma unroll
+        for (int w = 1; w < NW; ++w) s += dpp[w * L + l];
+        dpool[(size_t)b * L + l] = s;
+    }
+    if (wave <= dc) {
+        const int o = wave;
+        float a = 0.f;
+        if (lift) {
+            for (int l = lane; l < L; l += 64)
+                a = o < dc ? __builtin_fmaf(dys[l], yb[o * L + l] + yb[(dc + o) * L + l], a) : a + dys[l];
+        }
+        const float t = segment_sum_to_last<64>(a);
+        if (lane == 63) gp[sl.coutw + o] = t;
+    }
+    __syncthreads();
+    const int n_wdtc = 2 * dc * Rc, n_wxc = 2 * Cc * dc;
+    for (int o = tid; o < n_wdtc + n_wxc; o += NT) {
+        if (o < n_wdtc) {
+            const int row = o / Rc, r = o - row * Rc, col = (row / dc) * Cc + r;
+            gp[sl.wdtc + o] = __builtin_fmaf(dta[row], T.za[col], dtb[row] * T.zb[col]);
+        } else {
+            const int q = o - n_wdtc, i = q % dc, kc = q / dc;
+            gp[sl.wxc + q] = __builtin_fmaf(dza[kc], T.cw[i], dzb[kc] * T.cb[i]);
+        }
+    }
+    {
+        const int i = wave & 3, isb = wave >> 2;
+        if (i < dc) {
+            const float *dz = isb ? dzb : dza;
+            float s = 0.f;
             if (lift) {
-                for (int l = lane; l < L; l += 64)
-                    a = o < dc ? __builtin_fmaf(dys[l], yb[o * L + l] + yb[(dc + o) * L + l], a) : a + dys[l];
-            }
-            const float t = segment_sum_to_last<64>(a);
-            if (lane == 63) gp[sl.coutw + o] = t;
-        }
-    }
-    __syncthreads();
-    {
-        const int ncol = 2 * Rc;
-        const int tpc = ncol >= NT ? 1 : NT / ncol;
-        for (int col = tid % (ncol < NT ? ncol : NT); col < ncol; col += NT) {
-            const int sub = ncol < NT ? tid / ncol : 0;
-            if (sub >= tpc) break;
-            const int k = col / Rc, r = col - k * Rc;
-            float wv[4];
-#pragma unroll
-            for (int i = 0; i < 4; ++i) wv[i] = i < dc ? p.Wdtc[(k * dc + i) * Rc + r] : 0.f;
-#pragma unroll 4
-            for (int l = sub; l < L; l += tpc) {
-                float s = 0.f;
-#pragma unroll
-                for (int i = 0; i < 4; ++i)
-                    if (i < dc) s = __builtin_fmaf(wv[i], ddb[(k * dc + i) * L + l], s);
-                dzb[(k * L + l) * Cc + r] = s;
-            }
-        }
-    }
-    __syncthreads();
-    for (int idx = tid; idx < dc * L; idx += NT) {
-        const int i = idx / L, l = idx - i * L;
-        float s = dub[i * L + l] + dub[(dc + i) * L + l];
-        for (int k = 0; k < 2; ++k) {
-            const float *dz = dzb + (k * L + l) * Cc;
-            const float *wx = sWx + k * Cc * dc + i;
-#pragma unroll 8
-            for (int c = 0; c < Cc; ++c) s = __builtin_fmaf(wx[c * dc], dz[c], s);
-        }
-        dsq[idx] = s;
-    }
-    __syncthreads();
-    for (int l = tid; l < L; l += NT) {
-        float s = 0.f;
-        for (int i = 0; i < dc; ++i) s = lift ? __builtin_fmaf(p.cin_w[i], dsq[i * L + l], s) : s + dsq[i * L + l];
-        dpool[(size_t)b * L + l] = s;
-    }
-    const int n_wdtc = 2 * dc * Rc, n_wxc = 2 * Cc * dc;
-    for (int o = tid; o < n_wdtc + n_wxc + 2 * dc; o += NT) {
-        float s = 0.f;
-        if (o < n_wdtc) {
-            const int row = o / Rc, r = o - row * Rc, k = row / dc;
-            if (stage_zdt) {
-#pragma unroll 8
-                for (int l = 0; l < L; ++l) s = __builtin_fmaf(ddb[row * L + l], zdt[(k * L + l) * Rc + r], s);
-            } else {
-#pragma unroll 8
-                for (int l = 0; l < L; ++l) s = __builtin_fmaf(ddb[row * L + l], zb[(k * L + l) * Cc + r], s);
-            }
-            gp[sl.wdtc + o] = s;
-        } else if (o < n_wdtc + n_wxc) {
-            const int q = o - n_wdtc, i = q % dc, kc = q / dc, k = kc / Cc, c = kc - k * Cc;
-#pragma unroll 8
-            for (int l = 0; l < L; ++l) s = __builtin_fmaf(dzb[(k * L + l) * Cc + c], seq[i * L + l], s);
-            gp[sl.wxc + q] = s;
-        } else {
-            const int q = o - n_wdtc - n_wxc, i = q % dc;
-            if (lift) {
-                if (q < dc) { for (int l = 0; l < L; ++l) s = __builtin_fmaf(dsq[i * L + l], p.pooled[(size_t)b * L + l], s); }
-                else        { for (int l = 0; l < L; ++l) s += dsq[i * L + l]; }
-            }
-            gp[sl.cinw + q] = s;
+                for (int kc = lane; kc < 2 * Cc; kc += 64) s = __builtin_fmaf(p.Wxc[kc * dc + i], dz[kc], s);
+            }
+            const float t = segment_sum_to_last<64>(s);
+            const float *q = cgw + 24 + isb * 4 + i;
+            float d = q[0];
+#pragma unroll
+            for (int w = 1; w < NW; ++w) d += q[w * kChCg];
+            if (lane == 63) gp[sl.cinw + isb * dc + i] = lift ? d + t : 0.f;
         }
     }
 }
@@ -613,54 +606,39 @@
 
 static int chan_check(const oss_chan_params &p) {
     if (p.B <= 0 || p.L <= 0 || p.dc < 1 || p.dc > 4 || p.Rc < 1 || p.Cc != p.Rc + 2 * kChN) return OSS_ERR_SHAPE;
-    if (!p.pooled || !p.Wxc || !p.Wdtc || !p.dt_bias || !p.A_logs || !p.Dsc || !p.cn_w || !p.cn_b || !p.zt || !p.dts || !p.hs ||
-        !p.y || !p.yc || !p.stat || !p.c)
+    if (!p.pooled || !p.Wxc || !p.Wdtc || !p.dt_bias || !p.A_logs || !p.Dsc || !p.cn_w || !p.cn_b || !p.hs || !p.y ||
+        !p.yc || !p.stat || !p.c)
         return OSS_ERR_NULL;
     if ((p.cin_w != nullptr) != (p.cout_w != nullptr)) return OSS_ERR_NULL;
     if (p.cin_w && (!p.cin_b || !p.cout_b)) return OSS_ERR_NULL;
     return 0;
 }
 
+static size_t chan_fwd_lds_floats(const oss_chan_params &p) {
+    return (size_t)(10 * p.dc + 2) * p.L + kChRed + chan_tab_floats(p.dc, p.Cc);
+}
+static size_t chan_bwd_lds_floats(const oss_chan_params &p) {
+    return (size_t)(1 + kChNT / 64) * p.L + kChRed + chan_tab_floats(p.dc, p.Cc) + (kChNT / 64) * kChCg + 4 * (size_t)p.Cc + 4 * p.dc;
+}
+
 int chan_fwd(const oss_chan_params &p, hipStream_t s) {
     if (int e = chan_check(p)) return e;
-    size_t smem = sizeof(float) * ((size_t)(3 * p.dc + 1) * p.L + kChRed + 4 * 2 * (size_t)p.dc * p.L);
+    const size_t smem = sizeof(float) * chan_fwd_lds_floats(p);
     if (smem > kChanLdsMax) return OSS_ERR_SHAPE;
-    const size_t extra = sizeof(float) * (2 * (size_t)p.L * p.Cc + 4 * (size_t)p.dc * p.L);
-    const int use_lds = smem + extra <= kChanLdsMax ? 1 : 0;
-    if (use_lds) smem += extra;
-    if (use_lds) {
-        if (int e = chan_enable_lds(reinterpret_cast<const void *>(oss_chan_fwd_kernel<true, kChNT>), smem)) return e;
-        hipLaunchKernelGGL((oss_chan_fwd_kernel<true, kChNT>), dim3(p.B), dim3(kChNT), smem, s, p);
-    } else {
-        if (int e = chan_enable_lds(reinterpret_cast<const void *>(oss_chan_fwd_kernel<false, kChNT>), smem)) return e;
-        hipLaunchKernelGGL((oss_chan_fwd_kernel<false, kChNT>), dim3(p.B), dim3(kChNT), smem, s, p);
-    }
+    if (int e = chan_enable_lds(reinterpret_cast<const void *>(oss_chan_fwd_kernel<kChNT>), smem)) return e;
+    hipLaunchKernelGGL((oss_chan_fwd_kernel<kChNT>), dim3(p.B), dim3(kChNT), smem, s, p);
     return (int)hipGetLastError();
 }
 
 int chan_bwd(const oss_chan_params &p, const float *gc, float *dpool, float *gsum, float *scratch, hipStream_t s) {
     if (int e = chan_check(p)) return e;
     if (!gc || !dpool || !gsum || !scratch) return OSS_ERR_NULL;
-    size_t smem = sizeof(float) * ((size_t)(2 * p.dc + 1) * p.L + kChRed + 2 * 4 * 2 * (size_t)p.dc * p.L + 2 * (size_t)p.Cc * p.dc);
-    if (smem > kChanLdsMax) return OSS_ERR_SHAPE;
-    const size_t zdt_bytes = sizeof(float) * 2 * (size_t)p.L * p.Rc;
-    const int stage_zdt = smem + zdt_bytes <= kChanLdsMax ? 1 : 0;
-    if (stage_zdt) smem += zdt_bytes;
-    const size_t extra = sizeof(float) * (2 * (size_t)p.L * p.Cc + 8 * (size_t)p.dc * p.L);
-    const int use_lds = smem + extra <= kChanLdsMax ? 1 : 0;
-    if (use_lds) smem += extra;
-    if (use_lds) {
-        if (int e = chan_enable_lds(reinterpret_cast<const void *>(oss_chan_bwd_kernel<true, kChNT>), smem)) return e;
-    } else {
-        if (int e = chan_enable_lds(reinterpret_cast<const void *>(oss_chan_bwd_kernel<false, kChNT>), smem)) return e;
-    }
+    const size_t smem = sizeof(float) * chan_bwd_lds_floats(p);
+    if (smem > kChanLdsMax || sizeof(float) * chan_fwd_lds_floats(p) > kChanLdsMax) return OSS_ERR_SHAPE;
+    if (int e = chan_enable_lds(reinterpret_cast<const void *>(oss_chan_bwd_kernel<kChNT>), smem)) return e;
     const size_t np = chan_grad_floats(p.L, p.dc, p.Rc, p.Cc);
     float *gpart = scratch;
-    float *dzt = gpart + (size_t)p.B * np;
-    float *ddts = dzt + (size_t)p.B * 2 * p.L * p.Cc;
-    float *dug = ddts + (size_t)p.B * 2 * p.dc * p.L;
-    if (use_lds) hipLaunchKernelGGL((oss_chan_bwd_kernel<true, kChNT>), dim3(p.B), dim3(kChNT), smem, s, p, gc, dpool, gpart, dzt, ddts, dug, stage_zdt);
-    else         hipLaunchKernelGGL((oss_chan_bwd_kernel<false, kChNT>), dim3(p.B), dim3(kChNT), smem, s, p, gc, dpool, gpart, dzt, ddts, dug, stage_zdt);
+    hipLaunchKernelGGL((oss_chan_bwd_kernel<kChNT>), dim3(p.B), dim3(kChNT), smem, s, p, gc, dpool, gpart);
     if (defer_finish())
         defer_sum(gpart, p.B, np, np, gsum, np, nullptr);
     else
@@ -668,9 +646,7 @@
     return (int)hipGetLastError();
 }
 
-size_t chan_bwd_scratch_floats(int B, int L, int dc, int Rc, int Cc) {
-    return (size_t)B * (chan_grad_floats(L, dc, Rc, Cc) + 2 * (size_t)L * Cc + 4 * (size_t)dc * L);
-}
+size_t chan_bwd_scratch_floats(int B, int L, int dc, int Rc, int Cc) { return (size_t)B * chan_grad_floats(L, dc, Rc, Cc); }
 
 int rowsum(oss_dtype io, const void *a, const void *bmul, float *out, int B, int C, int P, int64_t asb, int64_t asc, int64_t bsb,
            int64_t bsc, float alpha, hipStream_t s) {
diff --git a/vmambair_amd/ops/channel.py b/vmambair_amd/ops/channel.py
--- a/vmambair_amd/ops/channel.py
+++ b/vmambair_amd/ops/channel.py
@@ -11,18 +11,19 @@
 
 
 def chan_supported(dc: int, n_state: int, d_inner: int) -> bool:
-    lds_bwd = 4 * ((18 * dc + 1) * d_inner + 2 * dc * (dc + 32 + 8) + 8)
-    return n_state == 16 and 1 <= dc <= 4 and lds_bwd <= 160 * 1024
+    rank = max(6, -(-d_inner // 16))
+    lds_fwd = 4 * ((10 * dc + 2) * d_inner + 4 * (rank + 32) + 6 * dc + 8)
+    return n_state == 16 and 1 <= dc <= 4 and lds_fwd <= 160 * 1024
 
 
 def _chan_params(B, L, pooled, prm, saved, c):
     cin_w, cin_b, Wxc, Wdtc, dt_bias, A_logs, Dsc, cout_w, cout_b, cn_w, cn_b = prm
-    zt, dts, hs, y, yc, stat = saved
+    hs, y, yc, stat = saved
     P = _capi.ChanParams()
     P.B, P.L, P.dc, P.Rc, P.Cc = B, L, Wdtc.shape[1], Wdtc.shape[2], Wxc.shape[1]
     for name, t in (("pooled", pooled), ("cin_w", cin_w), ("cin_b", cin_b), ("Wxc", Wxc), ("Wdtc", Wdtc), ("dt_bias", dt_bias),
                     ("A_logs", A_logs), ("Dsc", Dsc), ("cout_w", cout_w), ("cout_b", cout_b), ("cn_w", cn_w), ("cn_b", cn_b),
-                    ("zt", zt), ("dts", dts), ("hs", hs), ("y", y), ("yc", yc), ("stat", stat), ("c", c)):
+                    ("hs", hs), ("y", y), ("yc", yc), ("stat", stat), ("c", c)):
         setattr(P, name, _ptr(t))
     P.pool_part, P.n_part, P.pool_scale = None, 0, 0.0
     return P
@@ -42,11 +43,12 @@
     dev = y2.device
     f = dict(dtype=torch.float32, device=dev)
     pooled, c = torch.empty((B, d), **f), torch.empty((B, d), **f)
-    saved = (torch.empty((B, 2, d, Cc), **f), torch.empty((B, 2 * dc, d), **f), torch.empty((B, 2 * dc, d, 16), **f),
-             torch.empty((B, 2 * dc, d), **f), torch.empty((B, d), **f), torch.empty((B, 2), **f))
+    unused = (torch.empty((0,), **f), torch.empty((0,), **f))
+    saved = (torch.empty((B, 2 * dc, d, 16), **f), torch.empty((B, 2 * dc, d), **f), torch.empty((B, d), **f),
+             torch.empty((B, 2), **f))
     out = torch.empty((B, d, H, W), dtype=y2.dtype, device=dev)
     if y2.numel() == 0:
-        return [out, c, pooled, *saved]
+        return [out, c, pooled, *unused, *saved]
     lib = _capi.load()
     with torch.cuda.device(dev):
         st = torch.cuda.current_stream().cuda_stream
@@ -62,7 +64,7 @@
         _capi.check(lib.oss_row_affine(_DT[y2.dtype], y2.data_ptr(), c.data_ptr() if mul_mode else None,
                                        None if mul_mode else c.data_ptr(), out.data_ptr(), B, d, H * W, y2.stride(0),
                                        y2.stride(1), 1.0, st), "oss_row_affine")
-    return [out, c, pooled, *saved]
+    return [out, c, pooled, *unused, *saved]
 
 
 def chan_gate_bwd(g: torch.Tensor, y2: torch.Tensor, c: torch.Tensor, pooled: torch.Tensor, zt: torch.Tensor, dts: torch.Tensor,
@@ -87,7 +89,7 @@
         st = torch.cuda.current_stream().cuda_stream
         _capi.check(lib.oss_rowsum(_DT[y2.dtype], g.data_ptr(), y2.data_ptr() if mul_mode else None, gc.data_ptr(), B, d, H * W,
                                    g.stride(0), g.stride(1), y2.stride(0), y2.stride(1), 1.0, st), "oss_rowsum")
-        _capi.check(lib.oss_chan_bwd(_chan_params(B, d, pooled, prm, (zt, dts, hs, y, yc, stat), c), gc.data_ptr(),
+        _capi.check(lib.oss_chan_bwd(_chan_params(B, d, pooled, prm, (hs, y, yc, stat), c), gc.data_ptr(),
                                      dpool.data_ptr(), grads.data_ptr(), scratch.data_ptr(), st), "oss_chan_bwd")
         _keep(scratch, grads)
         if fold:
```

Measured after the change: 254.4 images/s (median of 6 runs). 1.3% higher.
